# krzyz/topo-renderer

Hardware: AMD Instinct MI355X
Metric: panorama Mpix/s (higher is better)
Workload: dtype f32; 1 GPU; c4: 10x10 deg COP90-shaped mosaic (100 tiles of 1200x1200 f32), 16384x4096 panorama = 8 sectors of 2048x4096, view_mode 0; frames_in_flight=1

## Files before the change

topo-renderer_amd/__init__.py:

```python
from __future__ import annotations

import ctypes as C
import math
import os
import subprocess

import numpy as np

from . import panorama, synth

_HERE = os.path.dirname(os.path.abspath(__file__))
LIB_PATH = os.environ.get("TOPO_HIP_LIB") or os.path.join(_HERE, "libtopo_hip.so")
HEADER_PATH = os.path.join(os.path.dirname(_HERE), "include", "topo_hip.h")
TEST_HEADER_PATH = os.path.join(os.path.dirname(_HERE), "include", "topo_hip_test.h")

TOPO_OK = 0
TOPO_ERR_INVALID, TOPO_ERR_UNSUPPORTED, TOPO_ERR_HIP, TOPO_ERR_NOT_FOUND, TOPO_ERR_CAPACITY = -1, -2, -3, -4, -5
FORMAT_RGBA8_UNORM_SRGB, FORMAT_BGRA8_UNORM_SRGB, FORMAT_RGBA8_UNORM, FORMAT_BGRA8_UNORM = 1, 2, 3, 4
TIMING_SLOTS = 9
TIMING_NAMES = ("clear", "cull", "raster", "occlusion", "raster_big", "resolve", "total", "load", "load_tables")

NEAR, FAR = 50.0, 500000.0
N_SECTORS = 8
HORIZON_SKY, HORIZON_INCOMPLETE = -1, -2
HORIZON_DTYPE = np.dtype([("row", "<i4"), ("depth", "<f4"), ("lat_deg", "<i4"), ("lon_deg", "<i4"), ("cell_x", "<u4"), ("cell_y", "<u4"),
                          ("fan", "<u4"), ("_reserved", "<u4")])


class TopoError(RuntimeError):
    def __init__(self, code, msg):
        super().__init__(f"topo_hip error {code}: {msg}")
        self.code = code


def build(verbose: bool = False) -> str:
    subprocess.check_call(["make", "-C", os.path.join(_HERE, "csrc"), "all"] + ([] if verbose else ["-s"]))
    return LIB_PATH


_lib = None


def _preload_torch_hip_runtime():
    import importlib.util
    try:
        spec = importlib.util.find_spec("torch")
    except (ImportError, ValueError):
        spec = None
    if spec and spec.submodule_search_locations:
        cand = os.path.join(list(spec.submodule_search_locations)[0], "lib", "libamdhip64.so")
        if os.path.exists(cand):
            C.CDLL(cand, mode=C.RTLD_GLOBAL)


def lib():
    global _lib
    if _lib is None:
        if not os.path.exists(LIB_PATH):
            raise ImportError(f"{LIB_PATH} is missing -- run `python -c 'import __graft_entry__ as g; g.build()'` "
                              "(there is no Python/CPU fallback for the render path)")
        _preload_torch_hip_runtime()
        L = C.CDLL(LIB_PATH)
        vp, u32, i32, f32, sz = C.c_void_p, C.c_uint32, C.c_int32, C.c_float, C.c_size_t
        sigs = {
            "topo_create": (C.c_int, [C.POINTER(vp), C.c_int, u32, u32, u32]),
            "topo_destroy": (None, [vp]),
            "topo_last_error": (C.c_char_p, [vp]),
            "topo_add_terrain": (C.c_int, [vp, i32, i32, vp, u32, u32, vp, vp, vp]),
            "topo_add_terrain_device": (C.c_int, [vp, i32, i32, vp, u32, u32, vp, vp, vp]),
            "topo_unload_terrain": (C.c_int, [vp, i32, i32]),
            "topo_update": (C.c_int, [vp, u32, u32, vp, vp]),
            "topo_render": (C.c_int, [vp, vp, sz, vp, sz]),
            "topo_recompute_normals": (C.c_int, [vp]),
            "topo_render_views_device": (C.c_int, [vp, u32, vp, u32, u32, vp, sz, sz, vp, sz, sz]),
            "topo_set_stream": (C.c_int, [vp, vp]),
            "topo_synchronize": (C.c_int, [vp]),
            "topo_set_normals_lds_rows": (C.c_int, [vp, C.c_int]),
            "topo_debug_set_queue_caps": (C.c_int, [vp, u32, u32]),
            "topo_debug_far_phase_launched": (C.c_int, [vp, vp]),
            "topo_pin_host_buffer": (C.c_int, [vp, vp, sz]),
            "topo_unpin_host_buffer": (C.c_int, [vp, vp]),
            "topo_get_timings": (C.c_int, [vp, vp]),
            "topo_get_timing_history": (C.c_int, [vp, C.c_uint32, vp, vp]),
            "topo_get_counters": (C.c_int, [vp, vp]),
            "topo_set_occlusion_split": (C.c_int, [vp, f32]),
            "topo_set_timing_slots": (C.c_int, [vp, u32]),
            "topo_read_normals": (C.c_int, [vp, i32, i32, vp]),
            "topo_read_tile_tables": (C.c_int, [vp, i32, i32, vp, vp, vp, vp]),
            "topo_probe_sincos": (C.c_int, [vp, vp, vp, vp, sz]),
            "topo_probe_div": (C.c_int, [vp, i32, vp, vp, vp, sz]),
            "topo_set_pipeline_depth": (C.c_int, [vp, i32]),
            "topo_join": (C.c_int, [vp]),
            "topo_frame_status": (C.c_int, [vp, vp]),
            "topo_overlay_lines": (C.c_int, [vp, vp, u32, vp, u32, f32, vp, sz]),
            "topo_overlay_lines_device": (C.c_int, [vp, vp, u32, vp, u32, f32, vp, sz]),
            "topo_overlay_glyphs": (C.c_int, [vp, vp, u32, C.c_float, vp, u32, u32, vp, sz]),
            "topo_overlay_glyphs_device": (C.c_int, [vp, vp, u32, C.c_float, vp, u32, u32, vp, sz]),
            "topo_change_location_plan": (None, [f32, f32, f32, vp, u32, vp, u32, vp, vp, u32, vp]),
            "topo_change_location": (C.c_int, [vp, f32, f32, f32, vp, u32, vp, vp]),
            "topo_comm_unique_id": (C.c_int, [vp]),
            "topo_comm_init": (C.c_int, [C.POINTER(vp), C.c_int, vp, C.c_int, C.c_int]),
            "topo_comm_from_nccl": (C.c_int, [C.POINTER(vp), vp, C.c_int, C.c_int]),
            "topo_comm_destroy": (None, [vp]),
            "topo_panorama_sector_range": (None, [C.c_int, C.c_int, vp, vp]),
            "topo_panorama_slots": (u32, [C.c_int, u32, u32, vp, u32]),
            "topo_render_panorama": (C.c_int, [vp, vp, vp, f32, f32, u32, u32, f32, f32, i32, vp, vp]),
            "topo_render_batch": (C.c_int, [vp, u32, vp, vp, vp, f32, u32, u32, i32, vp, vp]),
            "topo_visible_peaks": (C.c_int, [vp, u32, vp, vp, vp]),
            "topo_visible_peaks_device": (C.c_int, [vp, vp, u32, u32, vp, sz, u32, vp, vp, vp]),
            "topo_camera_uniforms": (None, [vp, f32, f32, f32, f32, f32, f32, f32, i32, vp]),
            "topo_terrain_uniforms": (None, [vp, vp, vp, u32, u32, vp]),
            "topo_geometry_transform": (None, [f32, f32, f32, vp]),
            "topo_dist_from_depth": (f32, [f32]),
            "topo_pad_256": (u32, [u32]),
            "topo_synth_tile": (None, [i32, i32, u32, u32, u32, vp]),
            "topo_locations_range": (u32, [f32, f32, f32, vp, u32]),
            "topo_coordinate_transform": (C.c_int, [vp, u32, vp, u32, vp, vp, vp, vp]),
            "topo_geotiff_info": (C.c_int, [vp, sz, vp, vp, vp, vp, vp]),
            "topo_sector_fov_y": (f32, [u32, u32, u32]),
            "topo_panorama_uniforms": (None, [vp, f32, f32, u32, u32, f32, f32, i32, u32, vp]),
            "topo_render_device": (C.c_int, [vp, vp, sz, vp, sz]),
            "topo_geotiff_decode": (C.c_int, [vp, vp, sz, vp, sz]),
            "topo_add_terrain_geotiff": (C.c_int, [vp, i32, i32, vp, sz]),
            "topo_to_model": (None, [vp, vp, vp, f32, f32, vp]),
            "topo_to_raster": (None, [vp, vp, vp, f32, f32, vp]),
            "topo_height_value_at": (C.c_int, [vp, u32, u32, vp, vp, vp, C.c_double, C.c_double, vp]),
            "topo_viewshed_enable": (C.c_int, [vp, i32]),
            "topo_viewshed_reset": (C.c_int, [vp]),
            "topo_viewshed_read": (C.c_int, [vp, i32, i32, vp, sz, vp]),
            "topo_debug_viewshed_stats": (C.c_int, [vp, vp]),
            "topo_horizon_shape": (C.c_int, [vp, vp, vp, vp]),
            "topo_horizon_read": (C.c_int, [vp, u32, u32, vp, sz]),
            "topo_horizon_device": (C.c_int, [vp, u32, u32, vp, sz]),
            "topo_pixel_angles": (None, [vp, u32, u32, u32, vp, vp]),
        }
        for name, (res, args) in sigs.items():
            fn = getattr(L, name)
            fn.restype = res
            fn.argtypes = args
        L._topo_symbols = tuple(sigs)
        _lib = L
    return _lib


def _p(a):
    return a.ctypes.data_as(C.c_void_p)



def camera_uniforms(eye, yaw, pitch, fov_y, width, height, sun_theta_deg, sun_phi_deg, view_mode=0) -> np.ndarray:
    out = np.zeros(40, dtype=np.float32)
    e = np.ascontiguousarray(eye, dtype=np.float32)
    lib().topo_camera_uniforms(_p(e), yaw, pitch, fov_y, width, height, sun_theta_deg, sun_phi_deg, view_mode, _p(out))
    return out


def terrain_uniforms(raster_point, model_point, pixel_scale, w, h) -> np.ndarray:
    out = np.zeros(24, dtype=np.float32)
    rp, mp, ps = (np.ascontiguousarray(a, dtype=np.float32) for a in (raster_point, model_point, pixel_scale))
    lib().topo_terrain_uniforms(_p(rp), _p(mp), _p(ps), w, h, _p(out))
    return out


def geometry_transform(h, lon_deg, lat_deg) -> np.ndarray:
    out = np.zeros(3, dtype=np.float32)
    lib().topo_geometry_transform(h, lon_deg, lat_deg, _p(out))
    return out


def dist_from_depth(d: float) -> float:
    return float(lib().topo_dist_from_depth(d))


def pad_256(n: int) -> int:
    return int(lib().topo_pad_256(n))


def synth_tile(lat_deg, lon_deg, w=1200, h=1200, seed=synth.SEED_DEFAULT) -> np.ndarray:
    out = np.empty((h, w), dtype=np.float32)
    lib().topo_synth_tile(lat_deg, lon_deg, w, h, seed & 0xFFFFFFFF, _p(out))
    return out


def locations_range(latitude: float, longitude: float, range_dist: float = 100_000.0):
    buf = np.zeros((4096, 2), np.int32)
    n = int(lib().topo_locations_range(latitude, longitude, range_dist, _p(buf), 4096))
    return [(int(a), int(b)) for a, b in buf[:min(n, 4096)]]


def change_location_plan(latitude: float, longitude: float, loaded, range_dist: float = 100_000.0):
    ld = np.ascontiguousarray(np.array(list(loaded), dtype=np.int32).reshape(-1, 2))
    un, rq = np.zeros((4096, 2), np.int32), np.zeros((4096, 2), np.int32)
    nu, nr = C.c_uint32(), C.c_uint32()
    lib().topo_change_location_plan(latitude, longitude, range_dist, _p(ld) if len(ld) else None, len(ld), _p(un), 4096, C.byref(nu), _p(rq), 4096, C.byref(nr))
    return [(int(a), int(b)) for a, b in un[:nu.value]], [(int(a), int(b)) for a, b in rq[:nr.value]]


class CoordinateTransform:

    def __init__(self, raster_point, model_point, pixel_scale):
        self.raster_point = np.asarray(raster_point, np.float32)
        self.model_point = np.asarray(model_point, np.float32)
        self.pixel_scale = np.asarray(pixel_scale, np.float32)

    @classmethod
    def from_geo_tag_data(cls, pixel_scale_data, tie_points_data, model_transformation_data=None):
        arr = lambda v: None if v is None else np.ascontiguousarray(v, dtype=np.float64)
        ps, tp, mt = arr(pixel_scale_data), arr(tie_points_data), arr(model_transformation_data)
        rp, mp, sc = (np.zeros(2, np.float32) for _ in range(3))
        ptr = lambda a: None if a is None else _p(a)
        rc = lib().topo_coordinate_transform(ptr(ps), 0 if ps is None else ps.size, ptr(tp), 0 if tp is None else tp.size, ptr(mt),
                                             _p(rp), _p(mp), _p(sc))
        if rc != 0:
            raise TopoError(rc, "IncorrectGeoTags" if rc == -2 else "IncorrectGeoTagData")
        return cls(rp, mp, sc)

    def to_model(self, x, y):
        out = np.zeros(2, np.float32)
        lib().topo_to_model(_p(self.raster_point), _p(self.model_point), _p(self.pixel_scale), x, y, _p(out))
        return float(out[0]), float(out[1])

    def to_raster(self, lon, lat):
        out = np.zeros(2, np.float32)
        lib().topo_to_raster(_p(self.raster_point), _p(self.model_point), _p(self.pixel_scale), lon, lat, _p(out))
        return float(out[0]), float(out[1])

    def height_value_at(self, heights: np.ndarray, longitude: float, latitude: float):
        hts = np.ascontiguousarray(heights, dtype=np.float32)
        h, w = hts.shape
        out = np.zeros(1, np.float32)
        rc = lib().topo_height_value_at(_p(hts), w, h, _p(self.raster_point), _p(self.model_point), _p(self.pixel_scale),
                                        float(longitude), float(latitude), _p(out))
        return None if rc != 0 else float(out[0])


def geotiff_info(data: bytes):
    buf = np.frombuffer(data, np.uint8)
    w, h = C.c_uint32(), C.c_uint32()
    rp, mp, sc = (np.zeros(2, np.float32) for _ in range(3))
    rc = lib().topo_geotiff_info(_p(buf), buf.size, C.byref(w), C.byref(h), _p(rp), _p(mp), _p(sc))
    if rc != 0:
        raise TopoError(rc, "GeoTIFF container or geo tags not usable")
    return int(w.value), int(h.value), CoordinateTransform(rp, mp, sc)


def pixel_angles(view_uniforms, width: int, height: int, xy) -> np.ndarray:
    u = np.ascontiguousarray(view_uniforms).view(np.uint8)
    if u.nbytes != 160:
        raise ValueError("uniforms must be 160 bytes")
    pts = np.ascontiguousarray(xy, dtype=np.float32).reshape(-1, 2)
    out = np.zeros((len(pts), 2), np.float64)
    lib().topo_pixel_angles(_p(u), width, height, len(pts), _p(pts), _p(out))
    return out


def post_uniforms(width, height, pixelize_n=100.0) -> np.ndarray:
    return np.array([width, height, pixelize_n, 0.0], dtype=np.float32)


def sector_fov_y(sector_w: int, sector_h: int, n_sectors: int = N_SECTORS) -> float:
    return 2.0 * math.atan(math.tan(math.pi / n_sectors) * sector_h / sector_w)


def panorama_uniforms(eye, yaw0, sector_w, sector_h, sun_theta_deg, sun_phi_deg, view_mode=0,
                      n_sectors: int = N_SECTORS, pitch: float = 0.0):
    out = np.zeros((n_sectors, 40), dtype=np.float32)
    e = np.ascontiguousarray(eye, dtype=np.float32)
    lib().topo_panorama_uniforms(_p(e), yaw0, pitch, sector_w, sector_h, sun_theta_deg, sun_phi_deg, view_mode, n_sectors, _p(out))
    return [out[k].copy() for k in range(n_sectors)]



def comm_unique_id() -> np.ndarray:
    out = np.zeros(128, np.uint8)
    rc = lib().topo_comm_unique_id(_p(out))
    if rc != TOPO_OK:
        raise TopoError(rc, lib().topo_last_error(None).decode())
    return out


class Comm:

    def __init__(self, rank: int = 0, world: int = 1, unique_id=None, device: int = 0, nccl_comm: int = 0):
        h = C.c_void_p()
        if nccl_comm:
            rc = lib().topo_comm_from_nccl(C.byref(h), C.c_void_p(nccl_comm), rank, world)
        else:
            uid = None if unique_id is None else np.ascontiguousarray(unique_id, dtype=np.uint8)
            rc = lib().topo_comm_init(C.byref(h), device, None if uid is None else _p(uid), rank, world)
        if rc != TOPO_OK:
            raise TopoError(rc, lib().topo_last_error(None).decode())
        self._h, self.rank, self.world = h, rank, world

    def close(self):
        if getattr(self, "_h", None):
            lib().topo_comm_destroy(self._h)
            self._h = None

    def __del__(self):
        try:
            self.close()
        except Exception:
            pass


def panorama_slots(world: int, sector_w: int, sector_h: int):
    n = lib().topo_panorama_slots(world, sector_w, sector_h, None, 0)
    out = np.zeros((max(1, n), 3), np.uint32)
    lib().topo_panorama_slots(world, sector_w, sector_h, _p(out), n)
    return [tuple(int(v) for v in row) for row in out[:n]]


def panorama_sector_range(rank: int, world: int):
    a, b = C.c_uint32(), C.c_uint32()
    lib().topo_panorama_sector_range(rank, world, C.byref(a), C.byref(b))
    return range(a.value, a.value + b.value)



class TerrainRenderer:

    def __init__(self, width: int, height: int, device: int = 0, color_format: int = FORMAT_RGBA8_UNORM_SRGB):
        h = C.c_void_p()
        rc = lib().topo_create(C.byref(h), device, width, height, color_format)
        if rc != TOPO_OK:
            raise TopoError(rc, lib().topo_last_error(None).decode())
        self._h = h
        self.size = (width, height)
        self.tile_size = None

    def close(self):
        if getattr(self, "_h", None):
            lib().topo_destroy(self._h)
            self._h = None

    def __del__(self):
        try:
            self.close()
        except Exception:
            pass

    def _check(self, rc):
        if rc != TOPO_OK:
            raise TopoError(rc, lib().topo_last_error(self._h).decode())

    def add_terrain(self, lat_deg, lon_deg, heights, raster_point, model_point, pixel_scale):
        hts = np.ascontiguousarray(heights, dtype=np.float32)
        h, w = hts.shape
        rp, mp, ps = (np.ascontiguousarray(a, dtype=np.float32) for a in (raster_point, model_point, pixel_scale))
        self._check(lib().topo_add_terrain(self._h, lat_deg, lon_deg, _p(hts), w, h, _p(rp), _p(mp), _p(ps)))
        self.tile_size = (w, h)

    def add_terrain_device(self, lat_deg, lon_deg, heights_ptr: int, w, h, raster_point, model_point, pixel_scale):
        rp, mp, ps = (np.ascontiguousarray(a, dtype=np.float32) for a in (raster_point, model_point, pixel_scale))
        self._check(lib().topo_add_terrain_device(self._h, lat_deg, lon_deg, C.c_void_p(heights_ptr), w, h, _p(rp), _p(mp), _p(ps)))
        self.tile_size = (w, h)

    def unload_terrain(self, lat_deg, lon_deg):
        self._check(lib().topo_unload_terrain(self._h, lat_deg, lon_deg))

    def update(self, width, height, uniforms: np.ndarray, post: np.ndarray):
        u = np.ascontiguousarray(uniforms).view(np.uint8)
        pu = np.ascontiguousarray(post, dtype=np.float32)
        if u.nbytes != 160 or pu.nbytes != 16:
            raise ValueError("uniforms must be 160 bytes and post uniforms 16 bytes")
        self._check(lib().topo_update(self._h, width, height, _p(u), _p(pu)))
        self.size = (width, height)

    def render(self, want_depth=True, padded_depth=False):
        w, h = self.size
        rgba = np.empty((h, w, 4), np.uint8)
        if not want_depth:
            self._check(lib().topo_render(self._h, _p(rgba), w * 4, None, 0))
            return rgba, None
        pitch = pad_256(4 * w) if padded_depth else 4 * w
        depth = np.zeros((h, pitch // 4), np.float32)
        self._check(lib().topo_render(self._h, _p(rgba), w * 4, _p(depth), pitch))
        return rgba, (depth if padded_depth else depth[:, :w])

    def render_into(self, rgba: np.ndarray, depth: np.ndarray = None):
        self._check(lib().topo_render(self._h, _p(rgba), rgba.strides[0], _p(depth) if depth is not None else None,
                                      depth.strides[0] if depth is not None else 0))

    def pin_host_buffer(self, a: np.ndarray):
        self._check(lib().topo_pin_host_buffer(self._h, _p(a), a.nbytes))

    def unpin_host_buffer(self, a: np.ndarray):
        self._check(lib().topo_unpin_host_buffer(self._h, _p(a)))

    def decode_geotiff(self, data: bytes) -> np.ndarray:
        w, h, _ = geotiff_info(data)
        buf = np.frombuffer(data, np.uint8)
        out = np.empty((h, w), np.float32)
        self._check(lib().topo_geotiff_decode(self._h, _p(buf), buf.size, _p(out), out.size))
        return out

    def add_terrain_geotiff(self, lat_deg: int, lon_deg: int, data: bytes):
        buf = np.frombuffer(data, np.uint8)
        self._check(lib().topo_add_terrain_geotiff(self._h, lat_deg, lon_deg, _p(buf), buf.size))
        w, h, _ = geotiff_info(data)
        self.tile_size = (w, h)

    def render_device(self, rgba_ptr: int, rgba_pitch: int, depth_ptr: int = 0, depth_pitch: int = 0):
        self._check(lib().topo_render_device(self._h, C.c_void_p(rgba_ptr), rgba_pitch, C.c_void_p(depth_ptr) if depth_ptr else None, depth_pitch))

    def recompute_normals(self):
        self._check(lib().topo_recompute_normals(self._h))

    def overlay_lines(self, vertices, indices, rgba: np.ndarray, line_width: float = 0.5) -> np.ndarray:
        v = np.ascontiguousarray(vertices)
        ix = np.ascontiguousarray(indices, dtype=np.uint32)
        assert rgba.dtype == np.uint8 and rgba.flags.c_contiguous
        self._check(lib().topo_overlay_lines(self._h, _p(v), v.nbytes // 32, _p(ix), ix.size, line_width, _p(rgba), rgba.strides[0]))
        return rgba

    def overlay_lines_device(self, vertices, indices, rgba_ptr: int, rgba_pitch: int, line_width: float = 0.5):
        v = np.ascontiguousarray(vertices)
        ix = np.ascontiguousarray(indices, dtype=np.uint32)
        self._check(lib().topo_overlay_lines_device(self._h, _p(v), v.nbytes // 32, _p(ix), ix.size, line_width, C.c_void_p(rgba_ptr), rgba_pitch))

    def overlay_glyphs(self, glyphs, atlas: np.ndarray, rgba: np.ndarray, depth: float = 100.0 / 4096.0) -> np.ndarray:
        g = np.ascontiguousarray(glyphs)
        a = np.ascontiguousarray(atlas, dtype=np.uint8)
        assert rgba.dtype == np.uint8 and rgba.flags.c_contiguous
        self._check(lib().topo_overlay_glyphs(self._h, _p(g), g.nbytes // 28, depth, _p(a), a.shape[1], a.shape[0], _p(rgba), rgba.strides[0]))
        return rgba

    def overlay_glyphs_device(self, glyphs, atlas: np.ndarray, rgba_ptr: int, rgba_pitch: int, depth: float = 100.0 / 4096.0):
        g = np.ascontiguousarray(glyphs)
        a = np.ascontiguousarray(atlas, dtype=np.uint8)
        self._check(lib().topo_overlay_glyphs_device(self._h, _p(g), g.nbytes // 28, depth, _p(a), a.shape[1], a.shape[0], C.c_void_p(rgba_ptr), rgba_pitch))

    def change_location(self, latitude: float, longitude: float, range_dist: float = 100_000.0):
        rq = np.zeros((4096, 2), np.int32)
        nr, nu = C.c_uint32(), C.c_uint32()
        self._check(lib().topo_change_location(self._h, latitude, longitude, range_dist, _p(rq), 4096, C.byref(nr), C.byref(nu)))
        return [(int(a), int(b)) for a, b in rq[:nr.value]], int(nu.value)

    def render_panorama(self, comm, eye, yaw0, sector_w, sector_h, sun_theta_deg, sun_phi_deg, strip_ptr: int, depth_ptr: int = 0,
                        view_mode: int = 0, pitch: float = 0.0):
        e = np.ascontiguousarray(eye, dtype=np.float32)
        self._check(lib().topo_render_panorama(self._h, comm._h if comm is not None else None, _p(e), yaw0, pitch, sector_w, sector_h,
                                               sun_theta_deg, sun_phi_deg, view_mode, C.c_void_p(strip_ptr),
                                               C.c_void_p(depth_ptr) if depth_ptr else None))

    def render_batch(self, eyes, yaw0s, suns_theta_phi_deg, sector_w, sector_h, rgba_ptr: int, depth_ptr: int = 0, view_mode: int = 0,
                     pitch: float = 0.0):
        e = np.ascontiguousarray(eyes, dtype=np.float32).reshape(-1, 3)
        y = np.ascontiguousarray(yaw0s, dtype=np.float32).reshape(-1)
        sn = np.ascontiguousarray(suns_theta_phi_deg, dtype=np.float32).reshape(-1, 2)
        assert len(e) == len(y) == len(sn)
        self._check(lib().topo_render_batch(self._h, len(e), _p(e), _p(y), _p(sn), pitch, sector_w, sector_h, view_mode,
                                            C.c_void_p(rgba_ptr), C.c_void_p(depth_ptr) if depth_ptr else None))

    def render_views_device(self, uniforms_list, width, height, rgba_ptr: int, rgba_view_stride: int, rgba_pitch: int,
                            depth_ptr: int = 0, depth_view_stride: int = 0, depth_pitch: int = 0):
        if isinstance(uniforms_list, np.ndarray) and uniforms_list.dtype == np.uint8 and uniforms_list.ndim == 2:
            us = np.ascontiguousarray(uniforms_list)
            assert us.shape[1] == 160
        else:
            us = np.ascontiguousarray(np.stack([np.ascontiguousarray(u).view(np.uint8).reshape(160) for u in uniforms_list]))
        self._check(lib().topo_render_views_device(self._h, len(us), _p(us), width, height,
                                                   C.c_void_p(rgba_ptr), rgba_view_stride, rgba_pitch,
                                                   C.c_void_p(depth_ptr) if depth_ptr else None, depth_view_stride, depth_pitch))

    def set_stream(self, hip_stream: int):
        self._check(lib().topo_set_stream(self._h, C.c_void_p(hip_stream) if hip_stream else None))

    def set_pipeline_depth(self, depth: int):
        self._check(lib().topo_set_pipeline_depth(self._h, depth))

    def join(self):
        self._check(lib().topo_join(self._h))

    def synchronize(self):
        self._check(lib().topo_synchronize(self._h))

    def frame_status(self) -> dict:
        out = np.zeros(4, np.uint32)
        self._check(lib().topo_frame_status(self._h, _p(out)))
        return {"status": int(out[0]), "big_overflow": bool(out[0] & 1), "rare_overflow": bool(out[0] & 2), "bounds_violation": bool(out[0] & 4),
                "bounds_site": int(out[1]), "bounds_value": int(out[2]) | (int(out[3]) << 32)}

    def set_normals_lds_rows(self, rows: int):
        self._check(lib().topo_set_normals_lds_rows(self._h, rows))

    def debug_set_queue_caps(self, big_cap: int, rare_cap: int):
        self._check(lib().topo_debug_set_queue_caps(self._h, big_cap, rare_cap))

    def debug_far_phase_launched(self) -> bool:
        out = np.zeros(1, np.int32)
        self._check(lib().topo_debug_far_phase_launched(self._h, _p(out)))
        return bool(out[0])

    def timings(self) -> dict:
        out = np.zeros(TIMING_SLOTS, np.float32)
        self._check(lib().topo_get_timings(self._h, _p(out)))
        return {k: float(v) for k, v in zip(TIMING_NAMES, out) if k != "_"}

    def timing_history(self, n_frames: int) -> list:
        out, n = np.zeros((max(1, n_frames), 7), np.float32), C.c_uint32(0)
        self._check(lib().topo_get_timing_history(self._h, n_frames, _p(out), C.byref(n)))
        return [{k: float(v) for k, v in zip(TIMING_NAMES[:7], row)} for row in out[:n.value]]

    def counters(self) -> dict:
        out = np.zeros(6, np.uint32)
        self._check(lib().topo_get_counters(self._h, _p(out)))
        return {"blocks_rastered": int(out[0]) + int(out[5]), "big_items": int(out[1]), "status": int(out[2]), "rare_items": int(out[3]),
                "near_blocks": int(out[0]), "far_tested": int(out[4]), "far_survived": int(out[5])}

    def set_timing_slots(self, names=None, total=True):
        mask = 0x3F if names is None else sum(1 << TIMING_NAMES.index(n) for n in names)
        if not total:
            mask |= 0x80
        self._check(lib().topo_set_timing_slots(self._h, mask))

    def set_occlusion_split(self, metres: float):
        self._check(lib().topo_set_occlusion_split(self._h, metres))

    def read_tile_tables(self, lat_deg, lon_deg) -> dict:
        w, h = self.tile_size
        n = C.c_uint32(0)
        self._check(lib().topo_read_tile_tables(self._h, lat_deg, lon_deg, None, None, None, C.byref(n)))
        minmax, trig, bounds = np.empty((n.value, 2), np.float32), np.empty((w + h, 2), np.float32), np.empty(n.value * 17, np.float64)
        self._check(lib().topo_read_tile_tables(self._h, lat_deg, lon_deg, _p(minmax), _p(trig), _p(bounds), C.byref(n)))
        return {"minmax": minmax, "trig": trig, "bounds": bounds}

    def read_normals(self, lat_deg, lon_deg) -> np.ndarray:
        w, h = self.tile_size
        out = np.empty((h, w, 4), np.uint8)
        self._check(lib().topo_read_normals(self._h, lat_deg, lon_deg, _p(out)))
        return out

    def visible_peaks(self, peaks_xyz: np.ndarray):
        pk = np.ascontiguousarray(peaks_xyz, dtype=np.float32).reshape(-1, 3)
        n = pk.shape[0]
        vis = np.zeros(n, np.uint8)
        xy = np.zeros((n, 2), np.uint32)
        self._check(lib().topo_visible_peaks(self._h, n, _p(pk), _p(vis), _p(xy)))
        return vis.astype(bool), xy

    def visible_peaks_device(self, uniforms, width, height, depth_ptr, depth_pitch, n, peaks_ptr, visible_ptr, xy_ptr):
        u = np.ascontiguousarray(uniforms).view(np.uint8)
        self._check(lib().topo_visible_peaks_device(self._h, _p(u), width, height, C.c_void_p(depth_ptr), depth_pitch, n,
                                                    C.c_void_p(peaks_ptr), C.c_void_p(visible_ptr), C.c_void_p(xy_ptr)))

    def viewshed_enable(self, on: bool = True):
        self._check(lib().topo_viewshed_enable(self._h, 1 if on else 0))

    def viewshed_reset(self):
        self._check(lib().topo_viewshed_reset(self._h))

    def viewshed(self, lat_deg, lon_deg) -> np.ndarray:
        if self.tile_size is None:
            raise TopoError(TOPO_ERR_NOT_FOUND, "no tile loaded")
        w, h = self.tile_size
        out = np.zeros((h - 1, w - 1), np.uint8)
        n = C.c_uint64(0)
        self._check(lib().topo_viewshed_read(self._h, lat_deg, lon_deg, _p(out), w - 1, C.byref(n)))
        if int(out.sum()) != n.value:
            raise TopoError(TOPO_ERR_INVALID, f"viewshed count {n.value} differs from the mask's {int(out.sum())} cells")
        return out.astype(bool)

    def debug_viewshed_stats(self) -> dict:
        out = np.zeros(3, np.uint64)
        self._check(lib().topo_debug_viewshed_stats(self._h, _p(out)))
        return {"terrain_keys": int(out[0]), "updates": int(out[1]), "atomics": int(out[2])}

    def horizon_shape(self):
        n, w, h = C.c_uint32(), C.c_uint32(), C.c_uint32()
        self._check(lib().topo_horizon_shape(self._h, C.byref(n), C.byref(w), C.byref(h)))
        return int(n.value), int(w.value), int(h.value)

    def horizon(self, first_view: int = 0, n_views: int = None) -> np.ndarray:
        total, w, _ = self.horizon_shape()
        n = total - first_view if n_views is None else n_views
        out = np.zeros((max(n, 0), w), HORIZON_DTYPE)
        self._check(lib().topo_horizon_read(self._h, first_view, n, _p(out) if out.size else None, w))
        return out

    def horizon_device(self, out_ptr: int, first_view: int = 0, n_views: int = None, view_stride: int = None):
        total, w, _ = self.horizon_shape()
        n = total - first_view if n_views is None else n_views
        self._check(lib().topo_horizon_device(self._h, first_view, n, C.c_void_p(out_ptr), w if view_stride is None else view_stride))

    def probe_div(self, kind: int, x: np.ndarray, y: np.ndarray) -> np.ndarray:
        x = np.ascontiguousarray(x, dtype=np.float32)
        y = np.ascontiguousarray(y, dtype=np.float32)
        out = np.empty_like(x)
        self._check(lib().topo_probe_div(self._h, kind, _p(x), _p(y), _p(out), x.size))
        return out

    def probe_sincos(self, x: np.ndarray):
        x = np.ascontiguousarray(x, dtype=np.float32)
        s, c = np.empty_like(x), np.empty_like(x)
        self._check(lib().topo_probe_sincos(self._h, _p(x), _p(s), _p(c), x.size))
        return s, c
```

topo-renderer_amd/csrc/host_math.cpp:

```cpp
#include "host_math.hpp"

#include <algorithm>
#include <cmath>
#include <cstdlib>
#include <cstring>

#include "topo_math.h"

namespace topo {

namespace {

inline float rs_to_radians(float d) { return d * 0.017453292519943295f; }

struct V3 { float x, y, z; };
inline float vdot(V3 a, V3 b) { return (a.x * b.x + a.y * b.y) + a.z * b.z; }
inline V3 vcross(V3 a, V3 b) { return {a.y * b.z - a.z * b.y, a.z * b.x - a.x * b.z, a.x * b.y - a.y * b.x}; }
inline V3 vnormalize(V3 v) {
    const float r = 1.0f / sqrtf(vdot(v, v));
    return {v.x * r, v.y * r, v.z * r};
}

void euler_xyz_ex_a0(float b, float c, float m[9] ) {
    const float si = sinf(0.0f), ci = cosf(0.0f);
    const float sj = sinf(b), cj = cosf(b), sh = sinf(c), ch = cosf(c);
    const float cc = ci * ch, cs = ci * sh, sc = si * ch, ss = si * sh;
    m[0] = cj * ch;       m[1] = cj * sh;       m[2] = -sj;
    m[3] = sj * sc - cs;  m[4] = sj * ss + cc;  m[5] = cj * si;
    m[6] = sj * cc + ss;  m[7] = sj * cs - sc;  m[8] = cj * ci;
}

}

void terrain_rotation(float model_lon_deg, float model_lat_deg, float rot[9]) {
    euler_xyz_ex_a0(rs_to_radians(90.0f - model_lat_deg), rs_to_radians(model_lon_deg), rot);
}

void geometry_transform(float h, float lon_deg, float lat_deg, float out[3]) {
    const float r = kR0 + h;
    const float lon = rs_to_radians(lon_deg), lat = rs_to_radians(lat_deg);
    out[0] = r * cosf(lat) * cosf(lon);
    out[1] = r * cosf(lat) * sinf(lon);
    out[2] = r * sinf(lat);
}

void pixel_angles(const topo_uniforms* view, uint32_t w, uint32_t h, uint32_t n, const float* xy, double* az_el) {
    const float* f = view->camera_proj;
    double m[4][4], inv[4][8];
    for (int r = 0; r < 4; ++r)
        for (int c = 0; c < 4; ++c) m[r][c] = f[4 * c + r];
    for (int r = 0; r < 4; ++r)
        for (int c = 0; c < 8; ++c) inv[r][c] = c < 4 ? m[r][c] : (c - 4 == r ? 1.0 : 0.0);
    for (int c = 0; c < 4; ++c) {
        int piv = c;
        for (int r = c + 1; r < 4; ++r)
            if (std::fabs(inv[r][c]) > std::fabs(inv[piv][c])) piv = r;
        for (int k = 0; k < 8; ++k) std::swap(inv[c][k], inv[piv][k]);
        const double d = inv[c][c];
        for (int k = 0; k < 8; ++k) inv[c][k] /= d;
        for (int r = 0; r < 4; ++r)
            if (r != c) {
                const double s = inv[r][c];
                for (int k = 0; k < 8; ++k) inv[r][k] -= s * inv[c][k];
            }
    }
    auto unproject = [&](double nx, double ny, double nz, double out[3]) {
        double p[4];
        for (int r = 0; r < 4; ++r) p[r] = inv[r][4] * nx + inv[r][5] * ny + inv[r][6] * nz + inv[r][7];
        for (int k = 0; k < 3; ++k) out[k] = p[k] / p[3];
    };
    const double ex = view->camera_pos[0], ey = view->camera_pos[1], ez = view->camera_pos[2];
    const double el = std::sqrt(ex * ex + ey * ey + ez * ez);
    const double up[3] = {ex / el, ey / el, ez / el};
    const double eh = std::hypot(up[0], up[1]);
    const double east[3] = {eh > 0.0 ? -up[1] / eh : 0.0, eh > 0.0 ? up[0] / eh : 1.0, 0.0};
    const double north[3] = {up[1] * east[2] - up[2] * east[1], up[2] * east[0] - up[0] * east[2], up[0] * east[1] - up[1] * east[0]};
    const double kDeg = 180.0 / 3.14159265358979323846;
    for (uint32_t i = 0; i < n; ++i) {
        const double nx = 2.0 * xy[2 * i] / w - 1.0, ny = 1.0 - 2.0 * xy[2 * i + 1] / h;
        double p0[3], p1[3];
        unproject(nx, ny, 0.0, p0);
        unproject(nx, ny, 1.0, p1);
        const double d[3] = {p1[0] - p0[0], p1[1] - p0[1], p1[2] - p0[2]};
        const double de = d[0] * east[0] + d[1] * east[1] + d[2] * east[2];
        const double dn = d[0] * north[0] + d[1] * north[1] + d[2] * north[2];
        const double du = d[0] * up[0] + d[1] * up[1] + d[2] * up[2];
        double az = std::atan2(de, dn) * kDeg;
        if (az < 0.0) az += 360.0;
        az_el[2 * i] = az;
        az_el[2 * i + 1] = std::atan2(du, std::hypot(de, dn)) * kDeg;
    }
}

void camera_uniforms(const float eye_in[3], float yaw, float pitch, float fov_y, float width, float height,
                     float sun_theta_deg, float sun_phi_deg, int32_t view_mode, topo_uniforms* out) {
    memset(out, 0, sizeof *out);
    const V3 eye = {eye_in[0], eye_in[1], eye_in[2]};
    const V3 up = vnormalize(eye);
    const V3 from = {0.0f, -1.0f, 0.0f};
    float qx, qy, qz, qw;
    const float d = vdot(from, up);
    const float one_minus_eps = 1.0f - 2.0f * 1.1920929e-7f;
    if (d > one_minus_eps) {
        qx = qy = qz = 0.0f; qw = 1.0f;
    } else if (d < -one_minus_eps) {
        const float sign = copysignf(1.0f, from.z);
        const float a = -1.0f / (sign + from.z);
        const float b = from.x * from.y * a;
        const V3 axis = {b, sign + from.y * from.y * a, -from.y};
        const float s = sinf(3.14159265358979323846f * 0.5f), c = cosf(3.14159265358979323846f * 0.5f);
        qx = axis.x * s; qy = axis.y * s; qz = axis.z * s; qw = c;
    } else {
        const V3 c = vcross(from, up);
        const float w = 1.0f + d;
        const float l2 = (c.x * c.x + c.z * c.z) + (c.y * c.y + w * w);
        const float r = 1.0f / sqrtf(l2);
        qx = c.x * r; qy = c.y * r; qz = c.z * r; qw = w * r;
    }
    const V3 v = {cosf(yaw) * cosf(pitch), sinf(pitch), sinf(yaw) * cosf(pitch)};
    const V3 b = {qx, qy, qz};
    const float b2 = vdot(b, b);
    const float k0 = qw * qw - b2, k1 = vdot(v, b) * 2.0f, k2 = qw * 2.0f;
    const V3 bxv = vcross(b, v);
    const V3 f = {(v.x * k0 + b.x * k1) + bxv.x * k2, (v.y * k0 + b.y * k1) + bxv.y * k2, (v.z * k0 + b.z * k1) + bxv.z * k2};
    const V3 s = vnormalize(vcross(f, up));
    const V3 u = vcross(s, f);
    const float view[16] = {s.x, u.x, -f.x, 0.0f, s.y, u.y, -f.y, 0.0f, s.z, u.z, -f.z, 0.0f,
                            -vdot(eye, s), -vdot(eye, u), vdot(eye, f), 1.0f};
    const float aspect = width / height;
    const float sf = sinf(0.5f * fov_y), cf = cosf(0.5f * fov_y);
    const float hh = cf / sf, ww = hh / aspect, r = kFar / (kNear - kFar);
    const float proj[16] = {ww, 0, 0, 0, 0, hh, 0, 0, 0, 0, r, -1.0f, 0, 0, r * kNear, 0};
    for (int c = 0; c < 4; ++c)
        for (int rr = 0; rr < 4; ++rr) {
            float t = proj[rr] * view[c * 4 + 0];
            t = t + proj[4 + rr] * view[c * 4 + 1];
            t = t + proj[8 + rr] * view[c * 4 + 2];
            t = t + proj[12 + rr] * view[c * 4 + 3];
            out->camera_proj[c * 4 + rr] = t;
        }
    for (int c = 0; c < 3; ++c)
        for (int rr = 0; rr < 3; ++rr) out->normal_proj[c * 4 + rr] = view[c * 4 + rr];
    out->normal_proj[15] = 1.0f;
    out->camera_pos[0] = eye.x; out->camera_pos[1] = eye.y; out->camera_pos[2] = eye.z; out->camera_pos[3] = 0.0f;
    float m3[9];
    euler_xyz_ex_a0(rs_to_radians(90.0f - sun_phi_deg), rs_to_radians(sun_theta_deg), m3);
    out->sun_direction[0] = m3[6]; out->sun_direction[1] = m3[7]; out->sun_direction[2] = m3[8];
    out->view_mode = view_mode;
}

void panorama_uniforms(const float eye[3], float yaw0, float pitch, uint32_t sector_w, uint32_t sector_h, float sun_theta_deg, float sun_phi_deg,
                       int32_t view_mode, uint32_t n_sectors, topo_uniforms* out) {
    const double kPi = 3.14159265358979323846;
    const double fov = 2.0 * atan(tan(kPi / (double)n_sectors) * (double)sector_h / (double)sector_w);
    for (uint32_t k = 0; k < n_sectors; ++k)
        camera_uniforms(eye, (float)((double)yaw0 - (double)k * (2.0 * kPi / (double)n_sectors)), pitch, (float)fov, (float)sector_w,
                        (float)sector_h, sun_theta_deg, sun_phi_deg, view_mode, out + k);
}

uint32_t locations_range(float latitude, float longitude, float range_dist, int32_t* out, uint32_t cap) {
    int c_lat = (int)floorf(latitude);
    c_lat = c_lat < -90 ? c_lat : -90;
    c_lat = c_lat > 89 ? c_lat : 89;
    const int c_lon = ((int)(floorf(longitude) + 540.0f)) % 360 - 180;
    const float lat_cos = cosf(rs_to_radians(latitude));
    const float arc_factor = 0.5f * range_dist / kR0;
    const float arc_factor_sin = sinf(arc_factor);
    const float afs_sq = arc_factor_sin * arc_factor_sin;
    const float R2D = 57.29577951308232f;
    const float dlon = acosf(1.0f - afs_sq / lat_cos / lat_cos) * R2D;
    const float dlat = acosf(1.0f - afs_sq) * R2D;
    int lat_start = (int)floorf(latitude - dlat);
    lat_start = lat_start > -90 ? lat_start : -90;
    int lat_end = (int)floorf(latitude + dlat);
    lat_end = lat_end < 89 ? lat_end : 89;
    const int lon_start = (int)floorf(longitude - dlon), lon_end = (int)floorf(longitude + dlon);
    struct Item { int lat, lon, k0, k1; };
    std::vector<Item> v;
    for (int la = lat_start; la <= lat_end; ++la)
        for (int lo = lon_start; lo <= lon_end; ++lo) v.push_back({la, lo, std::abs(la - c_lat), std::abs(lo - c_lon)});
    std::stable_sort(v.begin(), v.end(), [](const Item& a, const Item& b) { return a.k0 != b.k0 ? a.k0 < b.k0 : a.k1 < b.k1; });
    uint32_t n = 0;
    for (const Item& it : v) {
        if (n < cap && out) { out[2 * n] = it.lat; out[2 * n + 1] = (it.lon + 540) % 360 - 180; }
        ++n;
    }
    return n;
}

void change_location_plan(float latitude, float longitude, float range_dist, const int32_t* loaded, uint32_t n_loaded,
                          std::vector<std::pair<int32_t, int32_t>>& unload, std::vector<std::pair<int32_t, int32_t>>& request) {
    const uint32_t n = locations_range(latitude, longitude, range_dist, nullptr, 0);
    std::vector<int32_t> want(2 * (size_t)n);
    locations_range(latitude, longitude, range_dist, want.data(), n);
    std::vector<bool> have(n, false);
    unload.clear();
    request.clear();
    for (uint32_t i = 0; i < n_loaded; ++i) {
        bool in_new = false;
        for (uint32_t k = 0; k < n; ++k)
            if (want[2 * k] == loaded[2 * i] && want[2 * k + 1] == loaded[2 * i + 1]) { in_new = true; have[k] = true; }
        if (!in_new) unload.emplace_back(loaded[2 * i], loaded[2 * i + 1]);
    }
    for (uint32_t k = 0; k < n; ++k) {
        bool dup = false;
        for (uint32_t j = 0; j < k && !dup; ++j) dup = want[2 * j] == want[2 * k] && want[2 * j + 1] == want[2 * k + 1];
        if (!have[k] && !dup) request.emplace_back(want[2 * k], want[2 * k + 1]);
    }
}

namespace {
inline float synth_hash(int64_t ix, int64_t iy, uint32_t seed) {
    uint32_t h = ((uint32_t)ix * 0x9E3779B1u) ^ ((uint32_t)iy * 0x85EBCA77u) ^ (seed * 0xC2B2AE3Du);
    h ^= h >> 15; h *= 0x2C1B3C6Du; h ^= h >> 12; h *= 0x297A2D39u; h ^= h >> 15;
    return (float)(h >> 8) * (1.0f / 16777216.0f);
}
}

void synth_tile(int32_t lat, int32_t lon, uint32_t w, uint32_t h, uint32_t seed, float* out) {
    static const int wl[5] = {512, 256, 128, 64, 32};
    static const float amp[5] = {1.0f, 0.5f, 0.25f, 0.125f, 0.0625f};
    const float norm = (float)(3000.0 / 1.9375);
    for (uint32_t y = 0; y < h; ++y) {
        const int64_t gy = (int64_t)(89 - lat) * h + y;
        for (uint32_t x = 0; x < w; ++x) {
            const int64_t gx = ((int64_t)lon + 180) * w + x;
            float acc = 0.0f;
            for (int o = 0; o < 5; ++o) {
                const int64_t cx = gx / wl[o], cy = gy / wl[o];
                const float fx = (float)(gx % wl[o]) / (float)wl[o], fy = (float)(gy % wl[o]) / (float)wl[o];
                const float ux = fx * fx * (3.0f - 2.0f * fx), uy = fy * fy * (3.0f - 2.0f * fy);
                const uint32_t s = seed + (uint32_t)o;
                const float v00 = synth_hash(cx, cy, s), v10 = synth_hash(cx + 1, cy, s);
                const float v01 = synth_hash(cx, cy + 1, s), v11 = synth_hash(cx + 1, cy + 1, s);
                const float a = v00 + ux * (v10 - v00), b = v01 + ux * (v11 - v01);
                const float v = a + uy * (b - a);
                acc = acc + amp[o] * v;
            }
            out[(size_t)y * w + x] = acc * norm;
        }
    }
}

}
```

topo-renderer_amd/csrc/host_math.hpp:

```cpp
#pragma once

#include <cstdint>
#include <utility>
#include <vector>

#include "../../include/topo_hip.h"

namespace topo {

void camera_uniforms(const float eye[3], float yaw, float pitch, float fov_y, float width, float height,
                     float sun_theta_deg, float sun_phi_deg, int32_t view_mode, topo_uniforms* out);
void panorama_uniforms(const float eye[3], float yaw0, float pitch, uint32_t sector_w, uint32_t sector_h, float sun_theta_deg, float sun_phi_deg,
                       int32_t view_mode, uint32_t n_sectors, topo_uniforms* out);
void geometry_transform(float h, float lon_deg, float lat_deg, float out[3]);
void pixel_angles(const topo_uniforms* view, uint32_t w, uint32_t h, uint32_t n, const float* xy, double* az_el);
void terrain_rotation(float model_lon_deg, float model_lat_deg, float rot3x3_colmajor[9]);
uint32_t locations_range(float latitude, float longitude, float range_dist, int32_t* out_lat_lon, uint32_t cap);
void change_location_plan(float latitude, float longitude, float range_dist, const int32_t* loaded, uint32_t n_loaded,
                          std::vector<std::pair<int32_t, int32_t>>& unload, std::vector<std::pair<int32_t, int32_t>>& request);
void synth_tile(int32_t lat, int32_t lon, uint32_t w, uint32_t h, uint32_t seed, float* out);

}
```

topo-renderer_amd/csrc/kernels_frame.h:

```cpp
#pragma once

#include "kernels_common.h"

namespace topo {
namespace {

__device__ __forceinline__ void clear_body(uint64_t* __restrict__ vis, uint8_t* __restrict__ dirty, size_t n, uint32_t* __restrict__ counters,
                                           uint32_t* __restrict__ zero, uint32_t block, uint32_t n_blocks) {
    if (block == 0)
        for (uint32_t i = threadIdx.x; i < kCounterWords; i += 256) zero[i] = 0;
    const uint32_t lane = threadIdx.x & 63;
    const size_t nseg = (n + 63) >> 6, wave = (size_t)block * 4 + (threadIdx.x >> 6), nwave = (size_t)n_blocks * 4;
    for (size_t g = wave * 64; g < nseg; g += nwave * 64) {
        const bool mine = g + lane < nseg && dirty[g + lane] != 0;
        uint64_t todo = __ballot(mine);
        if (mine) dirty[g + lane] = 0;
        while (todo) {
            const size_t seg = g + (size_t)__builtin_ctzll(todo);
            todo &= todo - 1;
            if (TOPO_CHK(counters, seg * 64 + lane < ((n + 63) & ~(size_t)63), 3u, seg * 64 + lane))
                vis[seg * 64 + lane] = kVisClear;
        }
    }
}
__global__ __launch_bounds__(256) void k_clear(uint64_t* __restrict__ vis, uint8_t* __restrict__ dirty, size_t n, uint32_t* __restrict__ counters,
                                               uint32_t* __restrict__ zero) {
    clear_body(vis, dirty, n, counters, zero, blockIdx.x, gridDim.x);
}


__device__ __forceinline__ void clip_plane(const float* m, int pl, double out[5]) {
    double a, b, cc, d;
    const int row = pl >> 1;
    const double sgn = (pl & 1) ? -1.0 : 1.0;
    if (pl == 4) {
        a = m[2]; b = m[6]; cc = m[10]; d = m[14];
    } else {
        a = (double)m[3] + sgn * (double)m[row];
        b = (double)m[7] + sgn * (double)m[4 + row];
        cc = (double)m[11] + sgn * (double)m[8 + row];
        d = (double)m[15] + sgn * (double)m[12 + row];
    }
    out[0] = a; out[1] = b; out[2] = cc; out[3] = d;
    out[4] = sqrt(a * a + b * b + cc * cc);
}

__device__ __forceinline__ void emit_near(const FrameParams& P, uint32_t view, uint32_t rank, uint32_t blk) {
    if (P.split_m > 0.0f) {
        const uint32_t by = blk / P.bx_count;
        const uint32_t cell_rows = min(kBCY, P.tile_h - 1 - by * kBCY);
        const uint32_t strip = P.near_strip, n = (cell_rows + strip - 1) / strip;
        const uint32_t base = atomicAdd(&P.counters[kCtrWork], n);
        for (uint32_t k = 0; k < n; ++k)
            if (base + k < P.near_cap && TOPO_CHK(P.counters, blk < (1u << 24) && strip * k < 16u, 4u, blk))
                P.work[base + k] = WorkItem{(view << 16) | rank, blk | ((strip * k) << 24) | (min(strip, cell_rows - strip * k) << 28)};
        return;
    }
    const uint32_t slot = atomicAdd(&P.counters[kCtrWork], 1u);
    if (slot < P.near_cap) P.work[slot] = WorkItem{(view << 16) | rank, blk};
}

__device__ __forceinline__ void cull_body(const FrameParams& P, uint32_t block) {
    const uint32_t blocks_per_tile = P.bx_count * P.by_count;
    const size_t total = (size_t)P.n_views * P.n_tiles * blocks_per_tile;
    const size_t gid0 = (size_t)block * blockDim.x, gid = gid0 + threadIdx.x;
    __shared__ double s_plane[2][6][5];
    __shared__ uint32_t s_far[256], s_nfar;
    const uint32_t view0 = (uint32_t)(gid0 / ((size_t)blocks_per_tile * P.n_tiles));
    if (threadIdx.x < 12 && view0 + threadIdx.x / 6 < P.n_views) clip_plane(P.views[view0 + threadIdx.x / 6].proj, threadIdx.x % 6, s_plane[threadIdx.x / 6][threadIdx.x % 6]);
    if (threadIdx.x == 0) s_nfar = 0;
    __syncthreads();
    if (gid < total) {
        const uint32_t blk = (uint32_t)(gid % blocks_per_tile);
        const uint32_t rank = (uint32_t)((gid / blocks_per_tile) % P.n_tiles);
        const uint32_t view = (uint32_t)(gid / ((size_t)blocks_per_tile * P.n_tiles));
        const TileDev& t = P.tiles[rank];
        const double hmin = (double)t.block_minmax[2 * blk], hmax = (double)t.block_minmax[2 * blk + 1];
        const double* bs = t.block_bounds + (size_t)blk * 4;
        const double c[3] = {bs[0], bs[1], bs[2]}, radius = bs[3];
        const float* m = P.views[view].proj;
        bool keep = true;
        for (int pl = 0; pl < 6 && keep; ++pl) {
            double own[5];
            const double* q = s_plane[view - view0 < 2 ? view - view0 : 0][pl];
            if (view - view0 >= 2) {
                clip_plane(m, pl, own);
                q = own;
            }
            const double dist = q[0] * c[0] + q[1] * c[1] + q[2] * c[2] + q[3];
            if (dist < -radius * q[4]) keep = false;
        }
        const bool sane = hmin <= hmax;
        if (!sane) keep = true;
        if (keep) {
            const double wn = sqrt((double)m[3] * m[3] + (double)m[7] * m[7] + (double)m[11] * m[11]);
            const double w_near = ((double)m[3] * c[0] + (double)m[7] * c[1] + (double)m[11] * c[2] + (double)m[15]) - radius * wn;
            const double sagitta = t.block_bounds[(size_t)blocks_per_tile * 16 + blk];
            if (sane && P.split_m > 0.0f && w_near > (double)P.split_m && sagitta <= 1.0) {
                const uint32_t fslot = atomicAdd(&s_nfar, 1u);
                if (TOPO_CHK(P.counters, fslot < 256u, 5u, fslot)) s_far[fslot] = threadIdx.x;
            }
            else emit_near(P, view, rank, blk);
        }
    }
    __syncthreads();
    for (uint32_t i = threadIdx.x; i < s_nfar; i += blockDim.x) {
        const size_t g = gid0 + s_far[i];
        const uint32_t blk = (uint32_t)(g % blocks_per_tile);
        const uint32_t rank = (uint32_t)((g / blocks_per_tile) % P.n_tiles);
        const uint32_t view = (uint32_t)(g / ((size_t)blocks_per_tile * P.n_tiles));
        const TileDev& t = P.tiles[rank];
        const double hmin = (double)t.block_minmax[2 * blk], hmax = (double)t.block_minmax[2 * blk + 1];
        const double* bb = t.block_bounds + (size_t)blocks_per_tile * 4 + (size_t)blk * 12;
        const float* m = P.views[view].proj;
        double bxlo = 1e30, bxhi = -1e30, bylo = 1e30, byhi = -1e30, wmin = 1e30, zclip_at_wmin = 0.0;
        const double hs[2] = {hmin - 1.0, hmax + 2.0 + t.block_bounds[(size_t)blocks_per_tile * 16 + blk]};
#pragma unroll 1
        for (int k = 0; k < 8; ++k) {
            const double R = (double)kR0 + (k < 4 ? hs[0] : hs[1]);
            const double px = R * bb[3 * (k & 3)], py = R * bb[3 * (k & 3) + 1], pz = R * bb[3 * (k & 3) + 2];
            const double cx = (double)m[0] * px + (double)m[4] * py + (double)m[8] * pz + (double)m[12];
            const double cy = (double)m[1] * px + (double)m[5] * py + (double)m[9] * pz + (double)m[13];
            const double cz = (double)m[2] * px + (double)m[6] * py + (double)m[10] * pz + (double)m[14];
            const double cw = (double)m[3] * px + (double)m[7] * py + (double)m[11] * pz + (double)m[15];
            const double icw = 1.0 / cw;
            const double sx = (cx * icw * 0.5 + 0.5) * (double)P.W, sy = (0.5 - cy * icw * 0.5) * (double)P.H;
            bxlo = sx < bxlo ? sx : bxlo; bxhi = sx > bxhi ? sx : bxhi;
            bylo = sy < bylo ? sy : bylo; byhi = sy > byhi ? sy : byhi;
            if (cw < wmin) { wmin = cw; zclip_at_wmin = cz; }
        }
        const double zmin = (zclip_at_wmin - 8.0) / wmin;
        if (!(wmin > 1000.0 && zmin > 0.0 && zmin < 1.0)) {
            emit_near(P, view, rank, blk);
            continue;
        }
        const int32_t ix0 = max((int32_t)floor(bxlo) - 2, 0), ix1 = min((int32_t)ceil(bxhi) + 2, P.W - 1);
        const int32_t iy0 = max((int32_t)floor(bylo) - 2, 0), iy1 = min((int32_t)ceil(byhi) + 2, P.H - 1);
        if (ix0 > ix1 || iy0 > iy1) continue;
        float zf = (float)zmin;
        if ((double)zf > zmin) zf = bits_f(f_bits(zf) - 1u);
        const uint32_t q = block % kFarLists, slot = atomicAdd(&P.counters[far_list_counter(q)], 1u);
        if (TOPO_CHK(P.counters, slot < P.far_sub_cap, 5u, slot)) {
            FarItem fi;
            fi.view_rank = (view << 16) | rank; fi.block = blk;
            fi.x0 = (uint16_t)ix0; fi.x1 = (uint16_t)ix1; fi.y0 = (uint16_t)iy0; fi.y1 = (uint16_t)iy1;
            fi.zmin_bits = f_bits(zf);
            P.far[(size_t)q * P.far_sub_cap + slot] = fi;
        }
    }
}

__global__ __launch_bounds__(256) void k_cull(FrameParams P) { cull_body(P, blockIdx.x); }
struct ClearCullArgs {
    FrameParams P;
    uint32_t n_cull_blocks, n_clear_blocks;
    uint32_t* zero;
    ViewPack pack;
    uint32_t pack_words;
};
__global__ __launch_bounds__(256) void k_clear_cull(FrameParams P, uint32_t n_cull_blocks, uint32_t n_clear_blocks, uint32_t* __restrict__ zero, ViewPack pack,
                                                    uint32_t pack_words) {
    if (pack_words) {
        const auto src = kernarg<uint32_t>(offsetof(ClearCullArgs, pack));
        if (blockIdx.x == 0 && threadIdx.x < pack_words) const_cast<uint32_t*>(reinterpret_cast<const uint32_t*>(P.views))[threadIdx.x] = src[threadIdx.x];
        P.views = (const ViewDev*)(const void*)src;
    }
    const uint32_t total = n_cull_blocks + n_clear_blocks;
    const uint32_t before = (uint32_t)((uint64_t)blockIdx.x * n_clear_blocks / total), upto = (uint32_t)((uint64_t)(blockIdx.x + 1u) * n_clear_blocks / total);
    if (upto > before) clear_body(P.vis, P.dirty, (size_t)P.n_views * P.W * P.H, P.counters, zero, before, n_clear_blocks);
    else cull_body(P, blockIdx.x - before);
}

#ifndef TOPO_OCC_ROWS
#define TOPO_OCC_ROWS 4
#endif
constexpr uint32_t kOccRows = TOPO_OCC_ROWS;
__global__ __launch_bounds__(256) void k_occlusion(FrameParams P) {
    if (blockIdx.x == 0 && threadIdx.x == 0) {
        P.counters[kCtrBigStart] = P.counters[kCtrBig];
        P.counters[kCtrRareStart] = P.counters[kCtrRare];
    }
    const uint32_t lane = threadIdx.x & 63;
    const uint32_t wave_global = blockIdx.x * 4 + __builtin_amdgcn_readfirstlane(threadIdx.x >> 6), wave_count = gridDim.x * 4;
    static_assert(kFarLists == 64, "one sub-list per lane");
    uint32_t incl = min(P.counters[far_list_counter(lane)], P.far_sub_cap);
#pragma unroll
    for (int o = 1; o < 64; o <<= 1) {
        const uint32_t up = (uint32_t)__shfl_up((int)incl, o);
        if ((int)lane >= o) incl += up;
    }
    const uint32_t count = (uint32_t)__shfl((int)incl, 63);
    if (blockIdx.x == 0 && threadIdx.x == 0) P.counters[kCtrFarTested] = count;
    auto entry = [&](uint32_t g) -> const FarItem& {
        const uint32_t q = (uint32_t)__popcll(__ballot(incl <= g));
        const uint32_t start = q ? (uint32_t)__shfl((int)incl, (int)q - 1) : 0u;
        return P.far[(size_t)q * P.far_sub_cap + (g - start)];
    };
    if (count == 0) return;
    FarItem fi_next = entry(wave_global < count ? wave_global : 0u);
    for (uint32_t item = wave_global; item < count; item += wave_count) {
        const FarItem fi = fi_next;
        fi_next = entry(item + wave_count < count ? item + wave_count : item);
        const uint64_t* vis = P.vis + (size_t)(fi.view_rank >> 16) * P.W * P.H;
        bool visible = false;
        for (uint32_t x = fi.x0; x <= fi.x1 && !visible; x += 64) {
            const uint32_t px = min(x + lane, (uint32_t)fi.x1);
            for (uint32_t y = fi.y0; y <= fi.y1; y += kOccRows) {
                uint32_t d[kOccRows];
#pragma unroll
                for (uint32_t k = 0; k < kOccRows; ++k) {
                    const size_t at = (size_t)min(y + k, (uint32_t)fi.y1) * P.W + px;
                    d[k] = TOPO_CHK(P.counters, at < (size_t)P.W * P.H && (fi.view_rank >> 16) < P.n_views, 6u, at) ? (uint32_t)(vis[at] >> 32) : 0u;
                }
                bool open = false;
#pragma unroll
                for (uint32_t k = 0; k < kOccRows; ++k) open |= d[k] >= fi.zmin_bits;
                if (__any(open)) { visible = true; break; }
            }
        }
        if (visible && lane == 0) {
            const uint32_t blk = fi.block, by = blk / P.bx_count;
            const uint32_t cell_rows = min(kBCY, P.tile_h - 1 - by * kBCY);
            const uint32_t strip = P.near_strip, n = (cell_rows + strip - 1) / strip;
            const uint32_t base = atomicAdd(&P.counters[kCtrFarSurvived], n);
            for (uint32_t k = 0; k < n; ++k)
                if (base + k < P.near_cap)
                    P.work2[base + k] = WorkItem{fi.view_rank, blk | ((strip * k) << 24) | (min(strip, cell_rows - strip * k) << 28)};
        }
    }
}



__device__ __forceinline__ void raster_box(const TriSetup& ts, const Vis& vis, int32_t W, uint32_t id,
                                           int32_t px0, int32_t px1, int32_t py0, int32_t py1) {
    for (int32_t py = py0; py <= py1; ++py)
        for (int32_t px = px0; px <= px1; ++px) {
            float z, b[3];
            if (triangle_pixel(ts, px, py, z, b)) vis_min(vis, (size_t)py * W + px, vis_key(z, id));
        }
}

__device__ bool enqueue_big(const FrameParams& P, uint32_t view, uint32_t id, const SVert& s0, const SVert& s1, const SVert& s2,
                            int32_t px0, int32_t px1, int32_t py0, int32_t py1) {
    const int32_t rx0 = px0 >> 6, rx1 = px1 >> 6, ry0 = py0 >> 6, ry1 = py1 >> 6;
    const uint32_t n = (uint32_t)((rx1 - rx0 + 1) * (ry1 - ry0 + 1));
    const uint32_t base = atomicAdd(&P.counters[kCtrBig], n);
    BigItem it;
    it.view = view;
    it.id = id;
    it.X[0] = s0.X; it.X[1] = s1.X; it.X[2] = s2.X;
    it.Y[0] = s0.Y; it.Y[1] = s1.Y; it.Y[2] = s2.Y;
    it.z[0] = s0.z; it.z[1] = s1.z; it.z[2] = s2.z;
    if (base >= P.big_cap || n > P.big_cap - base) {
        atomicOr(&P.counters[kCtrStatus], kStatusBigOverflow);
        it.id = kNoTri;
        it.region = 0;
        for (uint32_t k = base; k < P.big_cap && k - base < n; ++k) P.big[k] = it;
        return false;
    }
    uint32_t k = base;
    for (int32_t ry = ry0; ry <= ry1; ++ry)
        for (int32_t rx = rx0; rx <= rx1; ++rx) {
            it.region = ((uint32_t)ry << 16) | (uint32_t)rx;
            if (TOPO_CHK(P.counters, k < P.big_cap && rx >= 0 && ry >= 0 && rx * 64 < P.W && ry * 64 < P.H, 7u, k)) P.big[k] = it;
            ++k;
        }
    return true;
}

__device__ __forceinline__ void enqueue_rare(const FrameParams& P, uint32_t view, uint32_t draw) {
    const uint32_t slot = atomicAdd(&P.counters[kCtrRare], 1u);
    if (slot < P.rare_cap) P.rare[slot] = RareItem{view, draw};
    else atomicOr(&P.counters[kCtrStatus], kStatusRareOverflow);
}

#ifndef TOPO_FRAG_CAP
#define TOPO_FRAG_CAP 128
#endif
constexpr uint32_t kFragCap = TOPO_FRAG_CAP;
struct FragList {
    uint32_t count;
    uint32_t pix[kFragCap];
    uint64_t key[kFragCap];
};

#ifndef TOPO_INLANE_ROWS
#define TOPO_INLANE_ROWS 5
#endif
#ifndef TOPO_INLANE_COLS
#define TOPO_INLANE_COLS 24
#endif
constexpr int32_t kInlaneRows = TOPO_INLANE_ROWS, kInlaneCols = TOPO_INLANE_COLS;

__device__ __forceinline__ void frag_push(FragList& fl, const Vis& vis, uint32_t pix, uint64_t key) {
    const uint32_t slot = atomicAdd(&fl.count, 1u);
    if (slot < kFragCap) {
        fl.pix[slot] = pix;
        fl.key[slot] = key;
    } else {
        vis_min(vis, pix, key);
    }
}

constexpr uint32_t kTriCap = 128;
struct TriList {
    int32_t X0[kTriCap], Y0[kTriCap], X1[kTriCap], Y1[kTriCap], X2[kTriCap], Y2[kTriCap];
    float z0[kTriCap], z1[kTriCap], z2[kTriCap];
    uint32_t id[kTriCap];
};

__device__ __forceinline__ bool classify_small(const FrameParams& P, const SVert& s0, const SVert& s1, const SVert& s2, uint32_t view,
                                               uint32_t id) {
    const int32_t X0 = s0.X, Y0 = s0.Y, X1 = s1.X, Y1 = s1.Y, X2 = s2.X, Y2 = s2.Y;
    const int32_t mnx = min(X0, min(X1, X2)), mxx = max(X0, max(X1, X2));
    const int32_t mny = min(Y0, min(Y1, Y2)), mxy = max(Y0, max(Y1, Y2));
    if ((mxx - mnx) >= (1 << 14) || (mxy - mny) >= (1 << 14)) {
        enqueue_rare(P, view, id >> 1);
        return false;
    }
    const int32_t area2 = __mul24(X1 - X0, Y2 - Y0) - __mul24(Y1 - Y0, X2 - X0);
    if (area2 >= 0) return false;
    const int32_t px0 = max((mnx + 127) >> 8, 0), px1 = min((mxx - 128) >> 8, P.W - 1);
    const int32_t py0 = max((mny + 127) >> 8, 0), py1 = min((mxy - 128) >> 8, P.H - 1);
    if (px0 > px1 || py0 > py1) return false;
    if (py1 - py0 >= kInlaneRows || px1 - px0 >= kInlaneCols) {
        if (!enqueue_big(P, view, id, s0, s1, s2, px0, px1, py0, py1)) enqueue_rare(P, view, id >> 1);
        return false;
    }
    return true;
}


__device__ __forceinline__ uint32_t tri_push(TriList& tl, uint32_t n, bool push, const SVert& s0, const SVert& s1, const SVert& s2,
                                             uint32_t id, uint32_t* vis_counters) {
    const uint64_t mask = __ballot(push);
    if (push) {
        const uint32_t slot = n + __popcll(mask & ((1ull << (threadIdx.x & 63)) - 1ull));
        if (!TOPO_CHK(vis_counters, slot < kTriCap, 8u, slot)) return n;
        tl.X0[slot] = s0.X; tl.Y0[slot] = s0.Y; tl.X1[slot] = s1.X; tl.Y1[slot] = s1.Y; tl.X2[slot] = s2.X; tl.Y2[slot] = s2.Y;
        tl.z0[slot] = s0.z; tl.z1[slot] = s1.z; tl.z2[slot] = s2.z;
        tl.id[slot] = id;
    }
    return n + (uint32_t)__popcll(mask);
}

__device__ __forceinline__ uint32_t tri_drain(TriList& tl, FragList& fl, const Vis& vis, int32_t W, int32_t H, uint32_t n,
                                              bool flush) {
    const uint32_t lane = threadIdx.x & 63;
    const uint32_t take = min(n, 64u), base = n - take;
    if (lane < take) {
        const uint32_t e = base + lane;
        raster_rows(W, H, tl.X0[e], tl.Y0[e], tl.X1[e], tl.Y1[e], tl.X2[e], tl.Y2[e], tl.z0[e], tl.z1[e], tl.z2[e], tl.id[e],
                    [&](uint32_t pix, uint64_t key) { frag_push(fl, vis, pix, key); });
    }
    const uint32_t nfrag = min(fl.count, kFragCap);
    if (nfrag >= 64 || (flush && nfrag > 0)) {
        for (uint32_t f = lane; f < nfrag; f += 64) vis_min(vis, fl.pix[f], fl.key[f]);
        if (lane == 0) fl.count = 0;
    }
    return base;
}

__device__ __forceinline__ SVert shfl_down1(const SVert& v) {
    SVert o;
    o.X = __shfl_down(v.X, 1);
    o.Y = __shfl_down(v.Y, 1);
    o.z = __shfl_down(v.z, 1);
    o.flag = __shfl_down(v.flag, 1);
    return o;
}

#ifndef TOPO_RASTER_WAVES
#define TOPO_RASTER_WAVES 5
#endif
__global__ __launch_bounds__(256, TOPO_RASTER_WAVES) void k_raster(FrameParams P, int phase) {
    __shared__ FragList s_fl[4];
    __shared__ TriList s_tl[4];
    const WorkItem* __restrict__ work = phase == 0 ? P.work : P.work2;
    uint32_t count = P.counters[phase == 0 ? kCtrWork : kCtrFarSurvived];
    const uint32_t cap = P.near_cap;
    if (count > cap) count = cap;
    const uint32_t lane = threadIdx.x & 63, wave = __builtin_amdgcn_readfirstlane(threadIdx.x >> 6);
    FragList& fl = s_fl[wave];
    TriList& tl = s_tl[wave];
    uint32_t ntri = 0;
    const uint32_t wave_global = blockIdx.x * 4 + wave, wave_count = gridDim.x * 4;
    for (uint32_t item = wave_global; item < count; item += wave_count) {
        const auto wi_c = const_space(work + item);
        const WorkItem wi = {wi_c->view_rank, wi_c->block};
        const uint32_t view_idx = wi.view_rank >> 16, rank = wi.view_rank & 0xFFFFu;
        TileDev t;
        {
            const auto tc = const_space(P.tiles + rank);
            t.heights = tc->heights;
            t.raster_x = tc->raster_x; t.raster_y = tc->raster_y;
            t.model_x = tc->model_x; t.model_y = tc->model_y;
            t.scale_x = tc->scale_x; t.scale_y = tc->scale_y;
        }
        const auto view_proj = const_space(P.views[view_idx].proj);
        const uint32_t blk_id = wi.block & 0xFFFFFFu, strip_first = (wi.block >> 24) & 15u, strip_rows = wi.block >> 28;
        const uint32_t bx = blk_id % P.bx_count, by = blk_id / P.bx_count;
        const uint32_t x0 = bx * kBCX, y0 = by * kBCY + strip_first;
        const uint32_t nrows = min(strip_rows ? strip_rows + 1 : kVY, P.tile_h - y0);
        const uint32_t ncx = min(kBCX, P.tile_w - 1 - x0);
        const uint32_t vx = x0 + lane;
        const bool vcol = lane < kVX && vx < P.tile_w;
        const Vis vis = view_vis(P, view_idx);
        float proj[16];
#pragma unroll
        for (int q = 0; q < 16; ++q) proj[q] = view_proj[q];
        if (lane == 0) fl.count = 0;
        float slo, clo, lat_s = 0.0f, lat_c = 0.0f;
        sincos_f(vertex_lon(t, vcol ? vx : x0), slo, clo);
        if (lane < nrows) sincos_f(vertex_lat(t, y0 + lane), lat_s, lat_c);
        const auto hcol = TOPO_GLOBAL_F32(t.heights) + (size_t)y0 * P.tile_w + (vcol ? vx : x0);
        (void)TOPO_CHK(P.counters, rank < P.n_tiles && view_idx < P.n_views && y0 + nrows <= P.tile_h && (vcol ? vx : x0) < P.tile_w && nrows >= 1u, 9u,
                       ((uint64_t)y0 << 32) | x0);
        float h0 = hcol[0];
        float h1 = nrows > 1 ? hcol[(size_t)1 * P.tile_w] : 0.0f;
        float h2 = nrows > 2 ? hcol[(size_t)2 * P.tile_w] : 0.0f;
        float h3 = nrows > 3 ? hcol[(size_t)3 * P.tile_w] : 0.0f;
        SVert prev;
        prev.X = 0; prev.Y = 0; prev.z = 0.0f; prev.flag = kVtxNear;
        for (uint32_t r = 0; r < nrows; ++r) {
            const float h = h0;
            h0 = h1; h1 = h2; h2 = h3;
            if (r + 4 < nrows) h3 = hcol[(size_t)(r + 4) * P.tile_w];
            const float sla = __shfl(lat_s, (int)r), cla = __shfl(lat_c, (int)r);
            SVert cur;
            cur.X = 0; cur.Y = 0; cur.z = 0.0f; cur.flag = kVtxNear;
            if (vcol) {
                const f3 p = world_from_sincos(h, sla, cla, slo, clo);
                float clip[4];
                mat4_point(proj, p.x, p.y, p.z, clip);
                clip_to_screen(clip, (float)P.W, (float)P.H, cur);
            }
            if (r > 0) {
                const SVert cc = shfl_down1(prev), d = shfl_down1(cur);
                bool live = lane < ncx;
                if (live && (prev.flag | cur.flag | cc.flag | d.flag) == kVtxOk) {
                    const int32_t qx0 = min(min(prev.X, cur.X), min(cc.X, d.X)), qx1 = max(max(prev.X, cur.X), max(cc.X, d.X));
                    const int32_t qy0 = min(min(prev.Y, cur.Y), min(cc.Y, d.Y)), qy1 = max(max(prev.Y, cur.Y), max(cc.Y, d.Y));
                    const int32_t bx0 = max((qx0 + 127) >> 8, 0), bx1 = min((qx1 - 128) >> 8, P.W - 1);
                    const int32_t by0 = max((qy0 + 127) >> 8, 0), by1 = min((qy1 - 128) >> 8, P.H - 1);
                    live = bx0 <= bx1 && by0 <= by1;
                }
                const SVert &a = prev, &b = cur;
                const uint32_t i = x0 + lane, j = y0 + r - 1;
                const bool even = ((i + j) & 1u) == 0;
                const uint32_t tri0 = (i * (P.tile_h - 1) + j) * 2;
#pragma unroll
                for (uint32_t k = 0; k < 2; ++k) {
                    const SVert& s0 = k == 0 ? a : d;
                    const SVert& s1 = k == 0 ? b : cc;
                    const SVert& s2 = k == 0 ? (even ? d : cc) : (even ? a : b);
                    const uint32_t draw = rank * P.tris_per_tile + tri0 + k;
                    bool push = false;
                    if (live) {
                        const int fg = s0.flag | s1.flag | s2.flag;
                        if (fg == kVtxOk) {
                            push = classify_small(P, s0, s1, s2, view_idx, draw << 1);
                        } else if (fg & kVtxNear) {
                            const int nnear = (s0.flag == kVtxNear) + (s1.flag == kVtxNear) + (s2.flag == kVtxNear);
                            if (nnear != 3) enqueue_rare(P, view_idx, draw);
                        }
                    }
                    ntri = tri_push(tl, ntri, push, s0, s1, s2, draw << 1, P.counters);
                    if (ntri >= 64) ntri = tri_drain(tl, fl, vis, P.W, P.H, ntri, false);
                }
            }
            prev = cur;
        }
// ... 130 lines not shown
```

topo-renderer_amd/csrc/terrain_renderer.cpp:

```cpp
#include "terrain_renderer.hpp"

#include "geotiff.hpp"

#include <algorithm>
#include <atomic>
#include <thread>
#include <cmath>
#include <cstdio>
#include <cstring>

namespace topo {

namespace {

struct Switches {
    static int env(const char* name, int unset) { return getenv(name) ? atoi(getenv(name)) : unset; }
    const bool views_by_copy = env("TOPO_VIEWS_BY_COPY", 0) != 0;
    const bool views_in_cull = env("TOPO_VIEWS_IN_CULL", 1) != 0;
    const bool status_by_copy = env("TOPO_STATUS_BY_COPY", 0) != 0;
    const bool far_skip = env("TOPO_FAR_SKIP", 1) != 0;
    const bool events_by_marker = env("TOPO_EVENTS_BY_MARKER", 0) != 0;
    const bool fuse_clear_cull = env("TOPO_FUSE_CLEAR_CULL", 1) != 0;
    const int near_strip = env("TOPO_NEAR_STRIP", 0);
};
const Switches& switches() { static const Switches s; return s; }

bool is_linear(uint32_t format) { return format == TOPO_FORMAT_RGBA8_UNORM || format == TOPO_FORMAT_BGRA8_UNORM; }
bool is_bgra(uint32_t format) { return format == TOPO_FORMAT_BGRA8_UNORM_SRGB || format == TOPO_FORMAT_BGRA8_UNORM; }

constexpr int kTimingSlots = 6;
constexpr uint32_t kStagesOfSlot[kTimingSlots] = {1u << kStClear, 1u << kStCull, (1u << kStRasterNear) | (1u << kStRasterFar), 1u << kStOcclusion,
                                                  (1u << kStRareBigNear) | (1u << kStRareBigFar), 1u << kStResolve};
constexpr uint32_t stage_events(int stage) { return 3u << stage; }
constexpr uint32_t kLastEvent = 1u << kNumStages, kTotalEvents = 1u | kLastEvent;

}

int TerrainRenderer::fail(int code, const std::string& msg) {
    err_ = msg;
    return code;
}

int TerrainRenderer::hip_fail(hipError_t e, const char* what) {
    err_ = std::string(what) + ": " + hipGetErrorString(e);
    return TOPO_ERR_HIP;
}

int TerrainRenderer::bind_device() {
    TOPO_HIP_TRY(hipSetDevice(device_));
    return TOPO_OK;
}

int TerrainRenderer::create(TerrainRenderer** out, int device, uint32_t w, uint32_t h, uint32_t format, std::string* err) {
    *out = nullptr;
    if (w == 0 || h == 0) { *err = "target size must be non-zero"; return TOPO_ERR_INVALID; }
    if (format < TOPO_FORMAT_RGBA8_UNORM_SRGB || format > TOPO_FORMAT_BGRA8_UNORM) {
        *err = "colour format must be Rgba8UnormSrgb, Bgra8UnormSrgb, Rgba8Unorm or Bgra8Unorm";
        return TOPO_ERR_UNSUPPORTED;
    }
    int count = 0;
    hipError_t e = hipGetDeviceCount(&count);
    if (e != hipSuccess || count == 0) {
        *err = std::string("no HIP device: ") + (e != hipSuccess ? hipGetErrorString(e) : "device count is 0") +
               " (this library has no CPU fallback)";
        return TOPO_ERR_HIP;
    }
    if (device < 0 || device >= count) { *err = "hip_device out of range"; return TOPO_ERR_INVALID; }
    TerrainRenderer* r = new TerrainRenderer();
    r->device_ = device;
    r->W_ = w;
    r->H_ = h;
    r->format_ = format;
    if (r->init() != TOPO_OK) {
        *err = "HIP initialisation failed: " + r->err_;
        delete r;
        return TOPO_ERR_HIP;
    }
    *out = r;
    return TOPO_OK;
}

int TerrainRenderer::init() {
    TOPO_HIP_TRY(hipSetDevice(device_));
    TOPO_HIP_TRY(hipStreamCreate(&own_stream_.h));
    stream_ = own_stream_;
    for (auto& e : load_ev_) TOPO_HIP_TRY(hipEventCreate(&e.h));
    return init_ctx(ctx_[0], false);
}

TerrainRenderer::~TerrainRenderer() {
    (void)hipSetDevice(device_);
    if (stream_) (void)hipStreamSynchronize(stream_);
    for (auto& c : ctx_)
        if (c.stream) (void)hipStreamSynchronize(c.stream);
}

int TerrainRenderer::ensure(hipStream_t s, DeviceBuffer& b, size_t need) {
    if (need <= b.cap) return TOPO_OK;
    if (b.p) {
        TOPO_HIP_TRY(hipStreamSynchronize(s));
        TOPO_HIP_TRY(hipFree(b.p));
        b.p = nullptr;
        b.cap = 0;
    }
    TOPO_HIP_TRY(hipMalloc(&b.p, need));
    b.cap = need;
    return TOPO_OK;
}

int TerrainRenderer::ensure_pinned(PinnedBuffer& b, size_t need) {
    if (need <= b.cap) return TOPO_OK;
    b.reset();
    TOPO_HIP_TRY(hipHostMalloc(&b.p, need));
    b.cap = need;
    return TOPO_OK;
}

int TerrainRenderer::wait_all() {
    if (int rc = join()) return rc;
    TOPO_HIP_TRY(hipStreamSynchronize(stream_));
    return TOPO_OK;
}

Tile* TerrainRenderer::find(int lat, int lon) {
    auto it = tiles_.find(geo_key(lat, lon));
    return it == tiles_.end() ? nullptr : &it->second;
}

void TerrainRenderer::collect_jobs(const Tile& nt, const std::map<GeoKey, uint32_t>& rank, std::vector<EdgeJob>& edges,
                                   std::vector<CornerJob>& corners) {
    const int lat = nt.lat, lon = nt.lon;
    const uint32_t NONE = 0xFFFFFFFFu;
    auto loaded = [&](int la, int lo) -> uint32_t {
        Tile* t = find(la, lo);
        return (t && t != &nt && t->seq < nt.seq) ? rank.at(geo_key(la, lo)) : NONE;
    };
    const uint32_t me = rank.at(geo_key(lat, lon));
    const uint32_t left = loaded(lat, lon - 1), right = loaded(lat, lon + 1);
    const uint32_t top = loaded(lat + 1, lon), bottom = loaded(lat - 1, lon);
    const uint32_t top_left = loaded(lat + 1, lon - 1), top_right = loaded(lat + 1, lon + 1);
    const uint32_t bottom_left = loaded(lat - 1, lon - 1), bottom_right = loaded(lat - 1, lon + 1);
    if (left != NONE) edges.push_back(EdgeJob{left, me, me, 0});
    if (right != NONE) edges.push_back(EdgeJob{me, right, me, 0});
    if (top != NONE) edges.push_back(EdgeJob{top, me, me, 1});
    if (bottom != NONE) edges.push_back(EdgeJob{me, bottom, me, 1});
    if (top_left != NONE && top != NONE && left != NONE) corners.push_back(CornerJob{top_left, top, left, me, me});
    if (top != NONE && top_right != NONE && right != NONE) corners.push_back(CornerJob{top, top_right, me, right, me});
    if (left != NONE && bottom_left != NONE && bottom != NONE) corners.push_back(CornerJob{left, me, bottom_left, bottom, me});
    if (right != NONE && bottom != NONE && bottom_right != NONE) corners.push_back(CornerJob{me, right, bottom, bottom_right, me});
}

int TerrainRenderer::upload_seam_jobs(const std::vector<EdgeJob>& edges, const std::vector<CornerJob>& corners) {
    if (!edges.empty()) {
        if (int rc = ensure(stream_, d_edge_jobs_, edges.size() * sizeof(EdgeJob))) return rc;
        TOPO_HIP_TRY(hipMemcpyAsync(d_edge_jobs_.p, edges.data(), edges.size() * sizeof(EdgeJob), hipMemcpyHostToDevice, stream_));
    }
    if (!corners.empty()) {
        if (int rc = ensure(stream_, d_corner_jobs_, corners.size() * sizeof(CornerJob))) return rc;
        TOPO_HIP_TRY(hipMemcpyAsync(d_corner_jobs_.p, corners.data(), corners.size() * sizeof(CornerJob), hipMemcpyHostToDevice, stream_));
    }
    return TOPO_OK;
}
void TerrainRenderer::launch_seam_jobs(size_t n_edges, size_t n_corners) {
    launch_normals_border(d_tiles_.as<const TileDev>(), d_edge_jobs_.as<const EdgeJob>(), (uint32_t)n_edges, d_corner_jobs_.as<const CornerJob>(), (uint32_t)n_corners,
                          tile_w_, tile_h_, stream_);
}
int TerrainRenderer::run_seam_jobs(const std::vector<EdgeJob>& edges, const std::vector<CornerJob>& corners) {
    if (int rc = upload_seam_jobs(edges, corners)) return rc;
    launch_seam_jobs(edges.size(), corners.size());
    return TOPO_OK;
}

std::map<GeoKey, uint32_t> TerrainRenderer::ranks() const {
    std::map<GeoKey, uint32_t> r;
    uint32_t i = 0;
    for (const auto& kv : tiles_) r[kv.first] = i++;
    return r;
}

int TerrainRenderer::add_terrain(int32_t lat, int32_t lon, const float* heights, bool on_device, uint32_t w, uint32_t h,
                                 const float rp[2], const float mp[2], const float ps[2]) {
    if (!heights || !rp || !mp || !ps) return fail(TOPO_ERR_INVALID, "null argument");
    if (w < 3 || h < 3) return fail(TOPO_ERR_INVALID, "tile must be at least 3x3");
    if (w > 32768 || h > 32768) return fail(TOPO_ERR_INVALID, "tile too large");
    if (!tiles_.empty() && (w != tile_w_ || h != tile_h_))
        return fail(TOPO_ERR_INVALID, "mixed tile sizes are rejected (the reference caches one mesh: render_buffer.rs:12-15)");
    if (int rc = join()) return rc;
    const uint64_t tris = 2ull * (w - 1) * (h - 1);
    const size_t n_after = tiles_.size() + (find(lat, lon) ? 0 : 1);
    if (tris * n_after >= (1ull << 31) || n_after > 0xFFFFu) return fail(TOPO_ERR_CAPACITY, "draw-order id space exhausted");
    tile_w_ = w;
    tile_h_ = h;
    const size_t texels = (size_t)w * h;
    const uint32_t bxc = (w - 1 + kBCX - 1) / kBCX, byc = (h - 1 + kBCY - 1) / kBCY;
    Tile t;
    t.lat = lat;
    t.lon = lon;
    t.seq = next_seq_++;
    const size_t tile_floats = (size_t)bxc * byc * 2 + 2 * ((size_t)w + h);
    auto up256 = [](size_t n) { return (n + 255) & ~(size_t)255; };
    const size_t off_normals = up256(texels * 4), off_tables = off_normals + up256(texels * 4), off_bounds = off_tables + up256(tile_floats * sizeof(float));
    if (int rc = ensure(stream_, t.pool, off_bounds + (size_t)bxc * byc * 17 * sizeof(double))) return rc;
    t.d_heights = t.pool.as<float>();
    t.d_normals = reinterpret_cast<uint32_t*>(t.pool.as<uint8_t>() + off_normals);
    t.d_minmax = reinterpret_cast<float*>(t.pool.as<uint8_t>() + off_tables);
    if (const hipError_t e = hipMemcpyAsync(t.d_heights, heights, texels * 4, on_device ? hipMemcpyDeviceToDevice : hipMemcpyHostToDevice, stream_))
        return hip_fail(e, "tile upload");
    if (vs_ever_)
        if (int rc = alloc_mask(t)) return rc;
    t.dev.heights = t.d_heights;
    t.dev.normals = t.d_normals;
    t.dev.block_minmax = t.d_minmax;
    t.dev.trig_lon = t.d_minmax + (size_t)bxc * byc * 2;
    t.dev.trig_lat = t.dev.trig_lon + 2 * (size_t)w;
    t.dev.block_bounds = reinterpret_cast<const double*>(t.pool.as<uint8_t>() + off_bounds);
    t.dev.raster_x = rp[0]; t.dev.raster_y = rp[1];
    t.dev.model_x = mp[0]; t.dev.model_y = mp[1];
    t.dev.scale_x = ps[0]; t.dev.scale_y = ps[1];
    terrain_rotation(mp[0], mp[1], t.dev.rot);
    struct Retired {
        Tile tile;
        hipStream_t stream;
        ~Retired() { if (tile.pool.p) (void)hipStreamSynchronize(stream); }
    } old{Tile{}, stream_};
    if (Tile* ex = find(lat, lon)) { old.tile = std::move(*ex); tiles_.erase(geo_key(lat, lon)); }
    Tile& nt = tiles_[geo_key(lat, lon)] = std::move(t);
    table_dirty_ = true;
    ++tile_gen_;
    if (int rc = upload_tile_table()) return rc;
    {
        const std::map<GeoKey, uint32_t> rk = ranks();
        std::vector<EdgeJob> edges;
        std::vector<CornerJob> corners;
        collect_jobs(nt, rk, edges, corners);
        launch_load_kernels(rk.at(geo_key(lat, lon)), 1, nullptr);
        if (int rc = run_seam_jobs(edges, corners)) return rc;
    }
    TOPO_HIP_TRY(hipStreamSynchronize(stream_));
    {
        std::vector<double> sph((size_t)bxc * byc * 4);
        TOPO_HIP_TRY(hipMemcpy(sph.data(), nt.dev.block_bounds, sph.size() * sizeof(double), hipMemcpyDeviceToHost));
        double c[3] = {0.0, 0.0, 0.0}, r2 = 0.0;
        bool finite = true;
        for (size_t i = 0; i < sph.size(); i += 4) {
            finite = finite && std::isfinite(sph[i]) && std::isfinite(sph[i + 1]) && std::isfinite(sph[i + 2]) && std::isfinite(sph[i + 3]);
            for (int k = 0; k < 3; ++k) c[k] += sph[i + k];
        }
        for (int k = 0; k < 3; ++k) c[k] /= (double)(sph.size() / 4);
        for (size_t i = 0; i < sph.size() && finite; i += 4) {
            const double dx = sph[i] - c[0], dy = sph[i + 1] - c[1], dz = sph[i + 2] - c[2];
            r2 = std::max(r2, dx * dx + dy * dy + dz * dz);
        }
        nt.centres[0] = c[0]; nt.centres[1] = c[1]; nt.centres[2] = c[2];
        nt.centres[3] = finite ? std::sqrt(r2) : -1.0;
    }
    TOPO_HIP_TRY(hipGetLastError());
    return TOPO_OK;
}

void TerrainRenderer::launch_load_kernels(uint32_t first, uint32_t count, hipEvent_t mid) {
    const TileDev* tiles = d_tiles_.as<const TileDev>();
    if (normals_tables_fused(tile_w_, tile_h_, lds_rows_)) {
        launch_trig_tables(tiles, first, count, tile_w_, tile_h_, stream_);
        if (mid) (void)hipEventRecord(mid, stream_);
        launch_normals_tables(tiles, first, count, tile_w_, tile_h_, stream_);
        launch_block_bounds(tiles, first, count, tile_w_, tile_h_, stream_);
    } else {
        launch_block_tables(tiles, first, count, tile_w_, tile_h_, stream_);
        if (mid) (void)hipEventRecord(mid, stream_);
        launch_normals_interior(tiles, first, count, tile_w_, tile_h_, lds_rows_, stream_);
    }
}

int TerrainRenderer::unload_terrain(int32_t lat, int32_t lon) {
    Tile* t = find(lat, lon);
    if (!t) return TOPO_OK;
    if (int rc = wait_all()) return rc;
    tiles_.erase(geo_key(lat, lon));
    table_dirty_ = true;
    ++tile_gen_;
    return TOPO_OK;
}

int TerrainRenderer::recompute_normals() {
    if (int rc = join()) return rc;
    std::vector<Tile*> order;
    for (auto& kv : tiles_) order.push_back(&kv.second);
    std::sort(order.begin(), order.end(), [](Tile* a, Tile* b) { return a->seq < b->seq; });
    if (int rc = upload_tile_table()) return rc;
    const std::map<GeoKey, uint32_t> rk = ranks();
    std::vector<EdgeJob> edges;
    std::vector<CornerJob> corners;
    for (Tile* t : order) collect_jobs(*t, rk, edges, corners);
    if (int rc = ensure(stream_, d_edge_jobs_, (edges.size() + 1) * sizeof(EdgeJob))) return rc;
    if (int rc = ensure(stream_, d_corner_jobs_, (corners.size() + 1) * sizeof(CornerJob))) return rc;
    if (int rc = upload_seam_jobs(edges, corners)) return rc;
    TOPO_HIP_TRY(hipEventRecord(load_ev_[0], stream_));
    launch_load_kernels(0, (uint32_t)order.size(), load_ev_[2]);
    launch_seam_jobs(edges.size(), corners.size());
    TOPO_HIP_TRY(hipEventRecord(load_ev_[1], stream_));
    TOPO_HIP_TRY(hipStreamSynchronize(stream_));
    load_timed_ = true;
    TOPO_HIP_TRY(hipGetLastError());
    return TOPO_OK;
}

int TerrainRenderer::update(uint32_t w, uint32_t h, const topo_uniforms* u, const topo_post_uniforms* pu) {
    if (!u || !pu) return fail(TOPO_ERR_INVALID, "null argument");
    if (w == 0 || h == 0) return fail(TOPO_ERR_INVALID, "target size must be non-zero");
    if (pu->pixelize_n < 99.99999f && !(pu->pixelize_n >= 1.0f)) return fail(TOPO_ERR_INVALID, "pixelize_n must be at least 1");
    if (pu->pixelize_n < 99.99999f && !(pu->viewport[0] >= 1.0f && pu->viewport[1] >= 1.0f)) return fail(TOPO_ERR_INVALID, "viewport must be at least 1 x 1");
    W_ = w;
    H_ = h;
    uniforms_ = *u;
    post_ = *pu;
    have_uniforms_ = true;
    return TOPO_OK;
}

int TerrainRenderer::upload_tile_table() {
    if (!table_dirty_) return TOPO_OK;
    std::vector<TileDev> table;
    for (auto& kv : tiles_) table.push_back(kv.second.dev);
    if (!table.empty()) {
        if (int rc = ensure(stream_, d_tiles_, table.size() * sizeof(TileDev))) return rc;
        TOPO_HIP_TRY(hipStreamSynchronize(stream_));
        TOPO_HIP_TRY(hipMemcpy(d_tiles_.p, table.data(), table.size() * sizeof(TileDev), hipMemcpyHostToDevice));
        if (vs_ever_) {
            std::vector<uint32_t*> masks;
            for (auto& kv : tiles_) masks.push_back(kv.second.mask.as<uint32_t>());
            if (int rc = ensure(stream_, d_vs_table_, masks.size() * sizeof(uint32_t*))) return rc;
            TOPO_HIP_TRY(hipMemcpy(d_vs_table_.p, masks.data(), masks.size() * sizeof(uint32_t*), hipMemcpyHostToDevice));
        }
    }
    table_dirty_ = false;
    return TOPO_OK;
}

int TerrainRenderer::init_ctx(FrameCtx& c, bool own_stream) {
    for (auto& f : c.timed_frames)
        for (auto& e : f.ev)
            if (!e) TOPO_HIP_TRY(hipEventCreate(&e.h));
    if (!c.done) TOPO_HIP_TRY(hipEventCreateWithFlags(&c.done.h, hipEventDisableTiming));
    if (own_stream && !c.stream) TOPO_HIP_TRY(hipStreamCreateWithFlags(&c.stream.h, hipStreamNonBlocking));
    return TOPO_OK;
}

int TerrainRenderer::join() {
    if (int rc = bind_device()) return rc;
    for (auto& c : ctx_)
        if (c.pending) {
            if (c.last_stream) TOPO_HIP_TRY(hipStreamSynchronize(c.last_stream));
            c.pending = false;
        }
    return TOPO_OK;
}

bool TerrainRenderer::fold_frames(FrameCtx& c, uint64_t end) {
    bool overflow = false;
    for (; c.checked < end; ++c.checked) {
        const uint32_t* w = c.status_words(c.checked);
        last_status_[0] |= w[kCtrStatus];
        if (w[kCtrStatus] & kStatusBounds) record_bounds(w);
        overflow |= (w[kCtrStatus] & kStatusRareOverflow) != 0;
    }
    return overflow;
}

void TerrainRenderer::record_bounds(const uint32_t* w) {
    last_status_[0] |= kStatusBounds;
    last_status_[1] = w[kCtrBoundsTag]; last_status_[2] = w[kCtrBoundsLo]; last_status_[3] = w[kCtrBoundsHi];
}

bool TerrainRenderer::fold_idle() {
    bool overflow = false;
    for (auto& c : ctx_)
        if (!c.pending && c.h_status.p) overflow |= fold_frames(c);
    return overflow;
}

bool TerrainRenderer::fold_latest(FrameCtx& c, bool retry) {
    overflow_pending_ |= fold_frames(c, c.submitted - 1);
    const bool overflow = (c.latest_status()[kCtrStatus] & kStatusRareOverflow) != 0;
    if (overflow && retry) ++c.checked;
    else (void)fold_frames(c);
    return overflow;
}

int TerrainRenderer::check_frames() {
    const bool overflow = fold_idle() | overflow_pending_;
    overflow_pending_ = false;
    if (overflow) return fail(TOPO_ERR_CAPACITY, "rare-triangle queue overflowed: a frame is incomplete (raise the queue capacity or render fewer views per submission)");
    return TOPO_OK;
}

int TerrainRenderer::set_pipeline_depth(int depth) {
    if (depth < 1 || depth > kMaxPipeline) return fail(TOPO_ERR_INVALID, "pipeline depth must be 1..4");
    if (int rc = wait_all()) return rc;
    for (int i = 0; i < depth; ++i)
        if (int rc = init_ctx(ctx_[i], depth > 1)) return rc;
    pipeline_depth_ = depth;
    next_ctx_ = last_ctx_ = 0;
    return TOPO_OK;
}

static const char* submission_error(uint32_t n, uint32_t w, uint32_t h) {
    if (n > 0xFFFFu) return "too many views";
    if (w == 0 || h == 0 || w > 65536 || h > 65536) return "bad target size";
    return nullptr;
}

int TerrainRenderer::render_views_device(uint32_t n, const topo_uniforms* views, uint32_t w, uint32_t h, const OutputParams& out) {
    if (n == 0 || !views || !out.rgba) return fail(TOPO_ERR_INVALID, "null/empty argument");
    if (const char* e = submission_error(n, w, h)) return fail(TOPO_ERR_INVALID, e);
    if (int rc = bind_device()) return rc;
    if (table_dirty_)
        if (int rc = join()) return rc;
    if (int rc = upload_tile_table()) return rc;
    FrameCtx& c = ctx_[next_ctx_];
    last_ctx_ = next_ctx_;
    next_ctx_ = (next_ctx_ + 1) % pipeline_depth_;
    if (pipeline_depth_ == 1) return render_frame(c, stream_, n, views, w, h, out);
    TOPO_HIP_TRY(hipEventRecord(c.done, stream_));
    TOPO_HIP_TRY(hipStreamWaitEvent(c.stream, c.done, 0));
    return render_frame(c, c.stream, n, views, w, h, out);
}

static bool far_phase_empty(const topo_uniforms* views, uint32_t n, const std::map<GeoKey, Tile>& tiles, float* split_m) {
    double bound = 0.0;
    for (uint32_t i = 0; i < n && bound >= 0.0; ++i) {
        const float* m = views[i].camera_proj;
        const double wn = std::sqrt((double)m[3] * m[3] + (double)m[7] * m[7] + (double)m[11] * m[11]);
        for (const auto& kv : tiles) {
            const double* s = kv.second.centres;
            const double w_far = (double)m[3] * s[0] + (double)m[7] * s[1] + (double)m[11] * s[2] + (double)m[15] + s[3] * wn;
            if (!(s[3] >= 0.0) || !(w_far < 1e30)) { bound = -1.0; break; }
            bound = std::max(bound, w_far);
        }
    }
    if (!(bound >= 0.0 && bound + 2.0 < (double)*split_m * (4.0 / 3.0))) return false;
    *split_m = std::max(*split_m, (float)(bound + 2.0));
    return true;
}

static bool fused_clear_cull(const FrameParams& p) { return switches().fuse_clear_cull && p.n_tiles != 0; }

int TerrainRenderer::render_frame(FrameCtx& c, hipStream_t stream, uint32_t n, const topo_uniforms* views, uint32_t w, uint32_t h,
                                  const OutputParams& out, const ResolveSlot* slots, uint32_t n_slots,
                                  const std::function<int(uint32_t, hipStream_t)>* after_slot) {
    if (n == 0) return fail(TOPO_ERR_INVALID, "null/empty argument");
    if (const char* e = submission_error(n, w, h)) return fail(TOPO_ERR_INVALID, e);
    latest_ctx_ = -1;
    FrameParams p{};
    if (int rc = grow_frame_buffers(c, stream, n, w, h, p)) return rc;
    ViewPack pack{};
    bool pack_in_cull = false;
    if (int rc = stage_views(c, stream, views, p, pack, &pack_in_cull)) return rc;
    fill_params(c, p);
    last_blocks_tested_ = p.work_cap;
    last_far_phase_ = p.split_m > 0.0f && !(switches().far_skip && far_phase_empty(views, n, tiles_, &p.split_m));
    if (int rc = queue_frame(c, stream, p, pack_in_cull ? &pack : nullptr, last_far_phase_, out, slots, n_slots, after_slot)) return rc;
    record_submission(c, p);
    TOPO_HIP_TRY(hipGetLastError());
    return TOPO_OK;
}

int TerrainRenderer::grow_frame_buffers(FrameCtx& c, hipStream_t stream, uint32_t n, uint32_t w, uint32_t h, FrameParams& p) {
    p.n_views = n;
    p.n_tiles = (uint32_t)tiles_.size();
    p.W = (int32_t)w;
    p.H = (int32_t)h;
    p.bx_count = p.n_tiles ? (tile_w_ - 1 + kBCX - 1) / kBCX : 0;
    p.by_count = p.n_tiles ? (tile_h_ - 1 + kBCY - 1) / kBCY : 0;
    const size_t pixels = (size_t)n * w * h;
    const size_t work_cap = (size_t)n * p.n_tiles * p.bx_count * p.by_count;
    p.big_cap = big_cap_cfg_ ? big_cap_cfg_ : (1u << 22);
    p.rare_cap = rare_cap_cfg_ ? rare_cap_cfg_ : (rare_cap_auto_ ? (uint32_t)rare_cap_auto_ : (1u << 22));
    if (work_cap >= (1ull << 30)) return fail(TOPO_ERR_CAPACITY, "too many raster blocks in one submission");
    if (pixels >= (1ull << 32)) return fail(TOPO_ERR_CAPACITY, "more than 2^32 pixels in one submission");
    const size_t vis_keys = (pixels + 63) & ~(size_t)63;
    if (vis_keys * 8 > c.d_vis.cap) {
        if (int rc = ensure(stream, c.d_vis, vis_keys * 8)) return rc;
        if (int rc = ensure(stream, c.d_dirty, vis_keys / 64 + 64)) return rc;
        TOPO_HIP_TRY(hipMemsetAsync(c.d_dirty.p, 1, c.d_dirty.cap, stream));
    }
    if (int rc = ensure(stream_, d_views_, sizeof(ViewDev) * kMaxViewsPerSlot * kViewSlots)) return rc;
    const int strip_env = switches().near_strip;
    p.near_strip = strip_env >= 1 && strip_env <= 15 ? (uint32_t)strip_env : (work_cap <= 64 * 1024 ? 1u : 2u);
    const size_t near_cap = (size_t)((kBCY + p.near_strip - 1) / p.near_strip) * work_cap;
    if (int rc = ensure(stream, c.d_work, (near_cap ? near_cap : 1) * sizeof(WorkItem))) return rc;
    if (int rc = ensure(stream, c.d_work2, (near_cap ? near_cap : 1) * sizeof(WorkItem))) return rc;
    const size_t far_sub_cap = ((work_cap + 255) / 256 + kFarLists - 1) / kFarLists * 256;
    if (int rc = ensure(stream, c.d_far, (far_sub_cap ? far_sub_cap * kFarLists : 1) * sizeof(FarItem))) return rc;
    if (int rc = ensure(stream, c.d_big, p.big_cap * sizeof(BigItem))) return rc;
    if (int rc = ensure(stream, c.d_rare, p.rare_cap * sizeof(RareItem))) return rc;
    if (!c.d_counters.p) {
        if (int rc = ensure(stream, c.d_counters, 2 * kCounterWords * sizeof(uint32_t))) return rc;
        TOPO_HIP_TRY(hipMemsetAsync(c.d_counters.p, 0, 2 * kCounterWords * sizeof(uint32_t), stream));
    }
    if (int rc = ensure_pinned(c.h_status, kStatusRing * kStatusWords * sizeof(uint32_t))) return rc;
    if (c.submitted - c.checked == kStatusRing) {
        if (c.last_stream) TOPO_HIP_TRY(hipStreamSynchronize(c.last_stream));
        overflow_pending_ |= fold_frames(c);
    }
    c.last_stream = stream;
    c.pending = pipeline_depth_ > 1;
    p.work_cap = (uint32_t)work_cap;
    p.far_sub_cap = (uint32_t)far_sub_cap;
    p.near_cap = (uint32_t)near_cap;
    return TOPO_OK;
}

int TerrainRenderer::stage_views(FrameCtx& c, hipStream_t stream, const topo_uniforms* views, FrameParams& p, ViewPack& pack, bool* pack_in_cull) {
    const uint32_t n = p.n_views;
    if (n > kMaxViewsPerSlot) return fail(TOPO_ERR_INVALID, "too many views in one submission");
    static_assert(kViewSlots % kMaxPipeline == 0, "every frame context has its own share of the slots");
    const int slot = (int)(&c - ctx_) * (kViewSlots / kMaxPipeline) + (int)(c.frames % (kViewSlots / kMaxPipeline));
    ViewDev* d_slot = d_views_.as<ViewDev>() + (size_t)slot * kMaxViewsPerSlot;
    p.views = d_slot;
    auto fill_views = [&](ViewDev* vd) {
        for (uint32_t i = 0; i < n; ++i) {
            memcpy(vd[i].proj, views[i].camera_proj, sizeof vd[i].proj);
            vd[i].cam_x = views[i].camera_pos[0];
            vd[i].cam_y = views[i].camera_pos[1];
            memcpy(vd[i].sun, views[i].sun_direction, sizeof vd[i].sun);
            vd[i].view_mode = views[i].view_mode;
        }
    };
    const bool packed = n <= kPackViews && !switches().views_by_copy;
    *pack_in_cull = packed && fused_clear_cull(p) && switches().views_in_cull;
    if (packed) {
        fill_views(pack.v);
        if (!*pack_in_cull) launch_put_views(pack, n, d_slot, stream);
        return TOPO_OK;
    }
    if (!view_ev_[kViewSlots - 1]) {
        if (int rc = ensure_pinned(h_views_, sizeof(ViewDev) * kMaxViewsPerSlot * kViewSlots)) return rc;
        for (auto& e : view_ev_)
            if (!e) TOPO_HIP_TRY(hipEventCreateWithFlags(&e.h, hipEventDisableTiming));
    }
    if (view_used_[slot]) TOPO_HIP_TRY(hipEventSynchronize(view_ev_[slot]));
    ViewDev* vd = h_views_.as<ViewDev>() + (size_t)slot * kMaxViewsPerSlot;
    fill_views(vd);
    TOPO_HIP_TRY(hipMemcpyAsync(d_slot, vd, n * sizeof(ViewDev), hipMemcpyHostToDevice, stream));
    TOPO_HIP_TRY(hipEventRecord(view_ev_[slot], stream));
    view_used_[slot] = true;
    return TOPO_OK;
}

void TerrainRenderer::fill_params(FrameCtx& c, FrameParams& p) {
    p.tiles = d_tiles_.as<const TileDev>();
    p.vis = c.d_vis.as<uint64_t>();
    p.dirty = c.d_dirty.as<uint8_t>();
    p.work = c.d_work.as<WorkItem>();
    p.counters = c.d_counters.as<uint32_t>() + (c.frames & 1u) * kCounterWords;
#ifdef TOPO_BOUNDS_CHECK
    p.status_out = nullptr;
#else
    p.status_out = switches().status_by_copy ? nullptr : c.status_words(c.submitted);
#endif
    p.big = c.d_big.as<BigItem>();
    p.rare = c.d_rare.as<RareItem>();
    p.far = c.d_far.as<FarItem>();
    p.work2 = c.d_work2.as<WorkItem>();
    p.split_m = occlusion_split_m_;
    p.tile_w = tile_w_;
    p.tile_h = tile_h_;
    p.tris_per_tile = p.n_tiles ? 2u * (tile_w_ - 1) * (tile_h_ - 1) : 8u;
    p.div_tris = fastdiv_make(p.tris_per_tile);
    p.div_hm1 = fastdiv_make(p.n_tiles ? tile_h_ - 1 : 2u);
    p.rblocks_x = ((uint32_t)p.W + kResolveBlockW - 1) / kResolveBlockW;
    p.rblocks_view = p.rblocks_x * (((uint32_t)p.H + kResolveBlockH - 1) / kResolveBlockH);
    p.div_rblocks_x = fastdiv_make(p.rblocks_x > 1 ? p.rblocks_x : 2u);
    p.div_rblocks_view = fastdiv_make(p.rblocks_view > 1 ? p.rblocks_view : 2u);
    float thresh[256];
    for (int i = 0; i < 256; ++i) thresh[i] = bits_f(TOPO_SRGB_THRESH_BITS[i]);
    p.linear_target = is_linear(format_) ? 1u : 0u;
    p.bgra = is_bgra(format_) ? 1u : 0u;
    p.sky_c8 = (p.linear_target ? to_unorm8(0.0f) | (to_unorm8(0.71f) << 8) | (to_unorm8(0.885f) << 16)
                                : srgb_encode(thresh, 0.0f) | (srgb_encode(thresh, 0.71f) << 8) | (srgb_encode(thresh, 0.885f) << 16)) |
               (to_unorm8(1.0f) << 24);
}

int TerrainRenderer::queue_frame(FrameCtx& c, hipStream_t stream, FrameParams& p, const ViewPack* pack_in_cull, bool far_phase, const OutputParams& out,
                                 const ResolveSlot* slots, uint32_t n_slots, const std::function<int(uint32_t, hipStream_t)>* after_slot) {
    const uint32_t n = p.n_views, w = (uint32_t)p.W, h = (uint32_t)p.H;
    uint32_t* const counters_next = c.d_counters.as<uint32_t>() + ((c.frames & 1u) ^ 1u) * kCounterWords;
    uint32_t ev_need = timing_total_ ? kTotalEvents : 0u;
    for (int sl = 0; sl < kTimingSlots; ++sl)
        for (int st = 0; st < kNumStages; ++st)
            if ((timing_slots_ & (1u << sl)) && (kStagesOfSlot[sl] & (1u << st))) ev_need |= stage_events(st);
    const bool pixelize = post_.pixelize_n < 99.99999f;
    const bool own_times = !switches().events_by_marker && !pixelize && (ev_need & ~(kTotalEvents | stage_events(kStResolve))) == 0;
    FrameCtx::TimedFrame& tf = c.timed_frames[c.frames++ % kEvRing];
    tf.recorded = ev_need;
    tf.slots = timing_slots_;
    tf.frame = ++frame_seq_;
    auto mark = [&](int i, bool may_be_own = false) { return (ev_need >> i & 1u) && !(may_be_own && own_times) ? hipEventRecord(tf.ev[i], stream) : hipSuccess; };
    auto own = [&](int i) -> hipEvent_t { return (ev_need >> i & 1u) && own_times ? (hipEvent_t)tf.ev[i] : nullptr; };
    TOPO_HIP_TRY(mark(kStClear, true));
    const hipEvent_t ev_first = own(kStClear);
    const bool fuse = fused_clear_cull(p);
    if (fuse) launch_clear_cull(p, counters_next, stream, ev_first, pack_in_cull, n);
    else launch_clear(p, counters_next, stream, ev_first);
    TOPO_HIP_TRY(mark(kStCull));
    if (!fuse) launch_cull(p, stream);
    TOPO_HIP_TRY(mark(kStRasterNear));
    launch_raster(p, 0, stream);
    TOPO_HIP_TRY(mark(kStRareBigNear));
    launch_raster_rare(p, stream);
    launch_raster_big(p, stream);
    TOPO_HIP_TRY(mark(kStOcclusion));
    if (far_phase) launch_occlusion(p, stream);
    TOPO_HIP_TRY(mark(kStRasterFar));
    if (far_phase) launch_raster(p, 1, stream);
    TOPO_HIP_TRY(mark(kStRareBigFar));
    if (far_phase) {
        launch_raster_rare(p, stream);
        launch_raster_big(p, stream);
    }
    TOPO_HIP_TRY(mark(kStResolve, true));
    const hipEvent_t ev_rstart = own(kStResolve), ev_rstop = own(kNumStages);
    OutputParams kout = out;
    if (pixelize) {
        if (n_slots) return fail(TOPO_ERR_UNSUPPORTED, "the pixelise branch is not available on the slot-by-slot (multi-GPU) path");
        const size_t img = (size_t)w * h * 4;
        if (int rc = ensure(stream, c.d_pre_rgba, img * n)) return rc;
        if (!out.depth)
            if (int rc = ensure(stream, c.d_pre_depth, img * n)) return rc;
        kout.rgba = c.d_pre_rgba.as<uint8_t>();
        kout.rgba_view_stride = img;
        kout.rgba_pitch = (size_t)w * 4;
        if (!out.depth) { kout.depth = c.d_pre_depth.as<float>(); kout.depth_view_stride = img; kout.depth_pitch = (size_t)w * 4; }
        p.post_off = 1;
    }
    if (n_slots == 0) {
        p.rblock_first = 0;
        p.rblock_count = p.rblocks_view * n;
        launch_resolve(p, kout, stream, ev_rstart, ev_rstop);
        if (pixelize)
            launch_post_pixelize(n, (int32_t)w, (int32_t)h, post_.viewport[0] >= 1.0f ? post_.viewport[0] : (float)w, post_.viewport[1] >= 1.0f ? post_.viewport[1] : (float)h,
                                 post_.pixelize_n, c.d_pre_rgba.as<const uint8_t>(), out, kout.depth, kout.depth_view_stride, kout.depth_pitch, p.linear_target, p.bgra, stream);
    } else {
        for (uint32_t i = 0; i < n_slots; ++i) {
            if ((uint64_t)slots[i].block_first + slots[i].block_count > (uint64_t)p.rblocks_view * n) return fail(TOPO_ERR_INVALID, "resolve slot outside the frame");
            p.rblock_first = slots[i].block_first;
            p.rblock_count = slots[i].block_count;
            launch_resolve(p, out, stream, i == 0 ? ev_rstart : nullptr, i + 1 == n_slots ? ev_rstop : nullptr);
            if (after_slot)
                if (int rc = (*after_slot)(i, stream)) return rc;
        }
    }
    if (vs_on_)
        launch_viewshed(p, d_vs_table_.as<uint32_t* const>(), d_vs_stats_.as<unsigned long long>(), stream);
    TOPO_HIP_TRY(mark(kNumStages, true));
    if (!p.status_out) TOPO_HIP_TRY(hipMemcpyAsync(c.status_words(c.submitted), p.counters, kStatusWords * sizeof(uint32_t), hipMemcpyDeviceToHost, stream));
    return TOPO_OK;
}

void TerrainRenderer::record_submission(FrameCtx& c, const FrameParams& p) {
    ++c.submitted;
    c.timed = true;
    c.sub.n_views = p.n_views;
    c.sub.tile_gen = tile_gen_;
    HorizonParams& q = c.sub.query;
    q.vis = p.vis;
    q.dirty = p.dirty;
    q.counters = p.counters;
    q.W = (uint32_t)p.W;
    q.H = (uint32_t)p.H;
    q.n_keys = (size_t)p.n_views * q.W * q.H;
    q.n_tiles = p.n_tiles;
    q.tris_per_tile = p.tris_per_tile;
    q.hm1 = p.n_tiles ? tile_h_ - 1 : 2u;
    q.div_tris = p.div_tris;
    q.div_hm1 = p.div_hm1;
    latest_ctx_ = (int)(&c - ctx_);
}


int TerrainRenderer::alloc_mask(Tile& t) {
    DeviceBuffer m;
    if (int rc = ensure(stream_, m, mask_bytes())) return rc;
    TOPO_HIP_TRY(hipMemsetAsync(m.p, 0, mask_bytes(), stream_));
    t.mask = std::move(m);
    return TOPO_OK;
}

int TerrainRenderer::viewshed_enable(bool on) {
    if (int rc = bind_device()) return rc;
    if (on && !vs_ever_) {
        if (int rc = join()) return rc;
        const size_t stats = (size_t)kViewshedStatSlots * 4 * sizeof(unsigned long long);
        if (!d_vs_stats_.p) {
            if (int rc = ensure(stream_, d_vs_stats_, stats)) return rc;
            TOPO_HIP_TRY(hipMemsetAsync(d_vs_stats_.p, 0, stats, stream_));
        }
        for (auto& kv : tiles_)
            if (!kv.second.mask.p)
                if (int rc = alloc_mask(kv.second)) return rc;
        vs_ever_ = true;
        table_dirty_ = true;
    }
    vs_on_ = on;
    return TOPO_OK;
}

int TerrainRenderer::viewshed_reset() {
    if (int rc = bind_device()) return rc;
    if (!vs_ever_) return TOPO_OK;
    if (int rc = join()) return rc;
    for (auto& kv : tiles_) TOPO_HIP_TRY(hipMemsetAsync(kv.second.mask.p, 0, mask_bytes(), stream_));
    TOPO_HIP_TRY(hipMemsetAsync(d_vs_stats_.p, 0, (size_t)kViewshedStatSlots * 4 * sizeof(unsigned long long), stream_));
    return TOPO_OK;
}

int TerrainRenderer::viewshed_read(int32_t lat, int32_t lon, uint8_t* mask_out, size_t pitch, uint64_t* n_visible) {
    if (!mask_out) return fail(TOPO_ERR_INVALID, "mask_out is null");
    Tile* t = find(lat, lon);
    if (!t) return fail(TOPO_ERR_NOT_FOUND, "no such tile");
    if (!vs_ever_) return fail(TOPO_ERR_INVALID, "viewshed accumulation was never enabled");
    const uint32_t wm1 = tile_w_ - 1, hm1 = tile_h_ - 1;
    if (pitch < wm1) return fail(TOPO_ERR_INVALID, "pitch smaller than a row");
    if (int rc = wait_all()) return rc;
    std::vector<uint32_t> words(mask_bytes() / 4);
    TOPO_HIP_TRY(hipMemcpy(words.data(), t->mask.p, mask_bytes(), hipMemcpyDeviceToHost));
    uint64_t count = 0;
    for (uint32_t x = 0, bit = 0; x < wm1; ++x)
        for (uint32_t y = 0; y < hm1; ++y, ++bit) {
            const uint8_t v = (uint8_t)((words[bit >> 5] >> (bit & 31u)) & 1u);
            mask_out[(size_t)y * pitch + x] = v;
            count += v;
        }
    if (n_visible) *n_visible = count;
    return TOPO_OK;
}

int TerrainRenderer::viewshed_stats(uint64_t out[3]) {
    if (!out) return fail(TOPO_ERR_INVALID, "null argument");
    out[0] = out[1] = out[2] = 0;
    if (!vs_ever_) return TOPO_OK;
    if (int rc = wait_all()) return rc;
    std::vector<unsigned long long> s((size_t)kViewshedStatSlots * 4);
    TOPO_HIP_TRY(hipMemcpy(s.data(), d_vs_stats_.p, s.size() * sizeof(s[0]), hipMemcpyDeviceToHost));
    for (size_t i = 0; i < s.size(); i += 4)
        for (int k = 0; k < 3; ++k) out[k] += s[i + k];
    return TOPO_OK;
}


static_assert(sizeof(HorizonPoint) == sizeof(topo_horizon_point) && sizeof(topo_horizon_point) == 32, "horizon record layout");

int TerrainRenderer::horizon_shape(uint32_t* n_views, uint32_t* w, uint32_t* h) {
    if (!n_views || !w || !h) return fail(TOPO_ERR_INVALID, "null argument");
    if (latest_ctx_ < 0) return fail(TOPO_ERR_INVALID, "no submission to query");
    const FrameCtx::Submission& s = ctx_[latest_ctx_].sub;
    *n_views = s.n_views;
    *w = s.query.W;
    *h = s.query.H;
    return TOPO_OK;
}

int TerrainRenderer::horizon_prepare(uint32_t first, uint32_t n, size_t view_stride, FrameCtx** out_c, hipStream_t* out_s) {
    if (latest_ctx_ < 0) return fail(TOPO_ERR_INVALID, "no submission to query");
    FrameCtx& c = ctx_[latest_ctx_];
    if (c.sub.tile_gen != tile_gen_) return fail(TOPO_ERR_INVALID, "tiles were added or unloaded since the latest submission: its draw order is gone");
    if (n == 0 || first >= c.sub.n_views || n > c.sub.n_views - first) return fail(TOPO_ERR_INVALID, "views outside the latest submission");
    if (view_stride < c.sub.query.W) return fail(TOPO_ERR_INVALID, "view stride smaller than a view's width");
    if (int rc = bind_device()) return rc;
    *out_c = &c;
    *out_s = c.last_stream ? c.last_stream : stream_;
    return TOPO_OK;
}

int TerrainRenderer::horizon_launch(FrameCtx& c, uint32_t first, uint32_t n, HorizonPoint* out, size_t view_stride, hipStream_t s) {
    if (hz_ll_gen_ != tile_gen_) {
        if (int rc = wait_all()) return rc;
        hz_ll_.clear();
        for (const auto& kv : tiles_) {
            hz_ll_.push_back(kv.second.lat);
            hz_ll_.push_back(kv.second.lon);
        }
        if (int rc = ensure(stream_, d_hz_ll_, (hz_ll_.size() + 2) * sizeof(int32_t))) return rc;
        if (!hz_ll_.empty()) TOPO_HIP_TRY(hipMemcpyAsync(d_hz_ll_.p, hz_ll_.data(), hz_ll_.size() * sizeof(int32_t), hipMemcpyHostToDevice, s));
        hz_ll_gen_ = tile_gen_;
    }
#ifdef TOPO_BOUNDS_CHECK
    if (!d_hz_check_.p) {
        if (int rc = ensure(s, d_hz_check_, kStatusWords * sizeof(uint32_t))) return rc;
        TOPO_HIP_TRY(hipMemsetAsync(d_hz_check_.p, 0, kStatusWords * sizeof(uint32_t), s));
    }
#endif
    HorizonParams p = c.sub.query;
    p.check = d_hz_check_.as<uint32_t>();
    p.tile_ll = d_hz_ll_.as<const int32_t>();
    p.out = out;
    p.view_stride = view_stride;
    p.first_view = first;
    p.n_views = n;
    launch_horizon(p, s);
    TOPO_HIP_TRY(hipGetLastError());
    return TOPO_OK;
}

int TerrainRenderer::horizon_fold_check() {
#ifdef TOPO_BOUNDS_CHECK
    if (!d_hz_check_.p) return TOPO_OK;
    uint32_t w[kStatusWords];
    TOPO_HIP_TRY(hipMemcpy(w, d_hz_check_.p, sizeof w, hipMemcpyDeviceToHost));
    if (w[kCtrStatus] & kStatusBounds) {
        record_bounds(w);
        TOPO_HIP_TRY(hipMemset(d_hz_check_.p, 0, sizeof w));
    }
#endif
    return TOPO_OK;
}

int TerrainRenderer::horizon_read(uint32_t first, uint32_t n, topo_horizon_point* out, size_t view_stride) {
    if (!out) return fail(TOPO_ERR_INVALID, "null argument");
    FrameCtx* c = nullptr;
    hipStream_t s = nullptr;
    if (int rc = horizon_prepare(first, n, view_stride, &c, &s)) return rc;
    const size_t row = (size_t)c->sub.query.W * sizeof(HorizonPoint);
    if (int rc = ensure(s, d_hz_out_, row * n)) return rc;
    if (int rc = horizon_launch(*c, first, n, d_hz_out_.as<HorizonPoint>(), c->sub.query.W, s)) return rc;
    TOPO_HIP_TRY(hipMemcpy2DAsync(out, view_stride * sizeof(topo_horizon_point), d_hz_out_.p, row, row, n, hipMemcpyDeviceToHost, s));
    TOPO_HIP_TRY(hipStreamSynchronize(s));
    c->pending = false;
    const bool overflow = fold_latest(*c, false);
    if (int rc = horizon_fold_check()) return rc;
    if (overflow)
        return fail(TOPO_ERR_CAPACITY, "rare-triangle queue overflowed: the latest submission is incomplete, and so is its horizon");
    return TOPO_OK;
}

int TerrainRenderer::horizon_device(uint32_t first, uint32_t n, topo_horizon_point* out_dev, size_t view_stride) {
    if (!out_dev) return fail(TOPO_ERR_INVALID, "null argument");
    if ((uintptr_t)out_dev % 16 != 0) return fail(TOPO_ERR_INVALID, "out_dev must be 16-byte aligned");
    FrameCtx* c = nullptr;
    hipStream_t s = nullptr;
    if (int rc = horizon_prepare(first, n, view_stride, &c, &s)) return rc;
    if (int rc = horizon_launch(*c, first, n, (HorizonPoint*)out_dev, view_stride, s)) return rc;
    if (s != stream_) c->pending = true;
    return TOPO_OK;
}

int TerrainRenderer::render_device(uint8_t* rgba_dev, size_t rgba_pitch, float* depth_dev, size_t depth_pitch) {
    if (!rgba_dev) return fail(TOPO_ERR_INVALID, "rgba_dev is null");
    if (!have_uniforms_) return fail(TOPO_ERR_INVALID, "topo_update has not been called");
    if (rgba_pitch < (size_t)W_ * 4 || (depth_dev && depth_pitch < (size_t)W_ * 4)) return fail(TOPO_ERR_INVALID, "pitch smaller than a row");
    return render_views_device(1, &uniforms_, W_, H_, image_output(rgba_dev, rgba_pitch, depth_dev, depth_pitch, H_));
}

int TerrainRenderer::render(uint8_t* rgba, size_t rgba_pitch, float* depth, size_t depth_pitch) {
    if (!rgba) return fail(TOPO_ERR_INVALID, "rgba_out is null");
    if (!have_uniforms_) return fail(TOPO_ERR_INVALID, "topo_update has not been called");
    if (rgba_pitch < (size_t)W_ * 4 || (depth && depth_pitch < (size_t)W_ * 4)) return fail(TOPO_ERR_INVALID, "pitch smaller than a row");
    if (int rc = bind_device()) return rc;
    const size_t row = (size_t)W_ * 4;
    if (int rc = ensure(stream_, d_out_rgba_, row * H_)) return rc;
    if (depth)
        if (int rc = ensure(stream_, d_out_depth_, row * H_)) return rc;
    const OutputParams o = image_output(d_out_rgba_.as<uint8_t>(), row, depth ? d_out_depth_.as<float>() : nullptr, row, H_);
    if (int rc = wait_all()) return rc;
    overflow_pending_ |= fold_idle();
    for (int attempt = 0;; ++attempt) {
        if (int rc = render_views_device(1, &uniforms_, W_, H_, o)) return rc;
        if (int rc = wait_all()) return rc;
        FrameCtx& fc = ctx_[last_ctx_];
        const bool retry = rare_cap_cfg_ == 0 && attempt < 3;
        if (!fold_latest(fc, retry)) break;
        if (!retry) return fail(TOPO_ERR_CAPACITY, "rare-triangle queue overflowed: frame incomplete");
        const uint32_t wanted = fc.latest_status()[kCtrRare];
        rare_cap_auto_ = (uint64_t)wanted + wanted / 4u + 1024u;
        if (rare_cap_auto_ > (1ull << 28)) return fail(TOPO_ERR_CAPACITY, "rare-triangle queue would exceed 2^28 entries");
    }
    if (int rc = download(rgba, rgba_pitch, d_out_rgba_.as<const uint8_t>(), row)) return rc;
    if (depth)
        if (int rc = download((uint8_t*)depth, depth_pitch, d_out_depth_.as<const uint8_t>(), row)) return rc;
    have_depth_ = depth != nullptr;
    depth_w_ = W_;
    depth_h_ = H_;
    return TOPO_OK;
}

int TerrainRenderer::download(uint8_t* dst, size_t dst_pitch, const uint8_t* src_dev, size_t row) {
    const size_t span = dst_pitch * (H_ - 1) + row;
    for (const auto& pin : pinned_)
        if (dst >= pin.as<uint8_t>() && dst + span <= pin.as<uint8_t>() + pin.cap) {
            TOPO_HIP_TRY(hipMemcpy2DAsync(dst, dst_pitch, src_dev, row, row, H_, hipMemcpyDeviceToHost, stream_));
            TOPO_HIP_TRY(hipStreamSynchronize(stream_));
            return TOPO_OK;
        }
    const size_t total = row * H_;
    if (int rc = ensure_pinned(h_stage_, total)) return rc;
    uint8_t* const stage = h_stage_.as<uint8_t>();
    constexpr int kSlices = 8;
    for (auto& e : stage_ev_)
        if (!e) TOPO_HIP_TRY(hipEventCreateWithFlags(&e.h, hipEventDisableTiming));
    const uint32_t rows_per = (H_ + kSlices - 1) / kSlices;
    int n_slices = 0;
    for (uint32_t r0 = 0; r0 < H_; r0 += rows_per, ++n_slices) {
        const uint32_t rows = std::min(rows_per, H_ - r0);
        TOPO_HIP_TRY(hipMemcpyAsync(stage + (size_t)r0 * row, src_dev + (size_t)r0 * row, (size_t)rows * row, hipMemcpyDeviceToHost, stream_));
        TOPO_HIP_TRY(hipEventRecord(stage_ev_[n_slices], stream_));
    }
    const unsigned hw = std::thread::hardware_concurrency();
    const int n_threads = (int)std::min<size_t>(std::max(1u, std::min(hw ? hw : 4u, 8u)), std::max<size_t>(1, total >> 20));
    std::atomic<int> failed{0};
// ... 410 lines not shown
```

topo-renderer_amd/csrc/terrain_renderer.hpp:

```cpp
#pragma once

#include <hip/hip_runtime.h>

#include <cstdint>
#include <functional>
#include <map>
#include <string>
#include <tuple>
#include <utility>
#include <vector>

#include "../../include/topo_hip.h"
#include "host_math.hpp"
#include "topo_kernels.h"

namespace topo {

constexpr uint32_t kPanoramaSectors = 8;
struct Comm;

using GeoKey = std::tuple<int, int, int, int>;
inline GeoKey geo_key(int lat, int lon) {
    return GeoKey(lat < 0 ? -lat : lat, lat > 0 ? 1 : 0, lon < 0 ? -lon : lon, lon > 0 ? 1 : 0);
}

#define TOPO_HIP_TRY(expr)                                   \
    do {                                                     \
        hipError_t e_ = (expr);                              \
        if (e_ != hipSuccess) return hip_fail(e_, #expr);    \
    } while (0)

template <hipError_t (*Free)(void*)>
struct Block {
    void* p = nullptr;
    size_t cap = 0;
    Block() = default;
    Block(Block&& o) noexcept : p(std::exchange(o.p, nullptr)), cap(std::exchange(o.cap, 0)) {}
    Block& operator=(Block&& o) noexcept { if (this != &o) { reset(); p = std::exchange(o.p, nullptr); cap = std::exchange(o.cap, 0); } return *this; }
    ~Block() { reset(); }
    void reset() { if (p) (void)Free(p); p = nullptr; cap = 0; }
    template <class T> T* as() const { return static_cast<T*>(p); }
};
using DeviceBuffer = Block<hipFree>;
using PinnedBuffer = Block<hipHostFree>;
using HostRegistration = Block<hipHostUnregister>;

template <class H, hipError_t (*Destroy)(H)>
struct Handle {
    H h = nullptr;
    Handle() = default;
    Handle(Handle&& o) noexcept : h(std::exchange(o.h, nullptr)) {}
    Handle& operator=(Handle&& o) noexcept { if (this != &o) { reset(); h = std::exchange(o.h, nullptr); } return *this; }
    ~Handle() { reset(); }
    void reset() { if (h) (void)Destroy(h); h = nullptr; }
    operator H() const { return h; }
};
using Event = Handle<hipEvent_t, hipEventDestroy>;
using Stream = Handle<hipStream_t, hipStreamDestroy>;

inline OutputParams image_output(uint8_t* rgba, size_t rgba_pitch, float* depth, size_t depth_pitch, uint32_t rows) {
    return OutputParams{rgba, rgba_pitch * rows, rgba_pitch, depth, depth_pitch * rows, depth_pitch};
}

struct Tile {
    int lat = 0, lon = 0;
    uint64_t seq = 0;
    DeviceBuffer pool;
    float* d_heights = nullptr;
    uint32_t* d_normals = nullptr;
    float* d_minmax = nullptr;
    double centres[4] = {0.0, 0.0, 0.0, -1.0};
    TileDev dev{};
    DeviceBuffer mask;
};

enum Stage { kStClear, kStCull, kStRasterNear, kStRareBigNear, kStOcclusion, kStRasterFar, kStRareBigFar, kStResolve, kNumStages };

class TerrainRenderer {
   public:
    static int create(TerrainRenderer** out, int device, uint32_t w, uint32_t h, uint32_t format, std::string* err);
    ~TerrainRenderer();

    int add_terrain(int32_t lat, int32_t lon, const float* heights, bool heights_on_device, uint32_t w, uint32_t h,
                    const float rp[2], const float mp[2], const float ps[2]);
    int unload_terrain(int32_t lat, int32_t lon);
    bool last_far_phase() const { return last_far_phase_; }
    int update(uint32_t w, uint32_t h, const topo_uniforms* u, const topo_post_uniforms* pu);
    int render(uint8_t* rgba, size_t rgba_pitch, float* depth, size_t depth_pitch);
    int render_views_device(uint32_t n, const topo_uniforms* views, uint32_t w, uint32_t h, const OutputParams& out);
    int render_device(uint8_t* rgba_dev, size_t rgba_pitch, float* depth_dev, size_t depth_pitch);
    int render_panorama(Comm* comm, const float eye[3], float yaw0, float pitch, uint32_t sector_w, uint32_t sector_h, float sun_theta_deg,
                        float sun_phi_deg, int32_t view_mode, uint8_t* strip_dev, float* depth_dev);
    int render_batch(uint32_t n_viewpoints, const float* eyes, const float* yaw0s, const float* sun_theta_phi_deg, float pitch, uint32_t sector_w,
                     uint32_t sector_h, int32_t view_mode, uint8_t* rgba_dev, float* depth_dev);
    int recompute_normals();
    int overlay_lines_device(const void* vertices, uint32_t n_vertices, const uint32_t* indices, uint32_t n_indices, float line_width, uint8_t* rgba_dev,
                             size_t rgba_pitch);
    int overlay_glyphs(const void* glyphs, uint32_t n_glyphs, float depth, const uint8_t* atlas, uint32_t atlas_w, uint32_t atlas_h, uint8_t* rgba, size_t rgba_pitch);
    int overlay_glyphs_device(const void* glyphs, uint32_t n_glyphs, float depth, const uint8_t* atlas, uint32_t atlas_w, uint32_t atlas_h, uint8_t* rgba_dev,
                              size_t rgba_pitch);
    int overlay_lines(const void* vertices, uint32_t n_vertices, const uint32_t* indices, uint32_t n_indices, float line_width, uint8_t* rgba,
                      size_t rgba_pitch);
    int change_location(float latitude, float longitude, float range_dist, std::vector<std::pair<int32_t, int32_t>>& request, uint32_t* n_unloaded);

    int set_stream(hipStream_t s);
    int synchronize();
    int set_pipeline_depth(int depth);
    int join();
    int join_frames();
    int set_normals_lds_rows(int rows);
    int set_queue_caps(uint32_t big_cap, uint32_t rare_cap);
    int pin_host_buffer(void* p, size_t bytes);
    int unpin_host_buffer(void* p);
    int get_timings(float out[TOPO_TIMING_SLOTS]);
    int get_timing_history(uint32_t n_frames, float* out_ms, uint32_t* n_out);
    int get_counters(uint32_t out[6]);
    int frame_status(uint32_t out[4]);
    int set_occlusion_split(float metres);
    int set_timing_slots(uint32_t mask);
    int read_normals(int32_t lat, int32_t lon, uint8_t* out);
    int read_tile_tables(int32_t lat, int32_t lon, float* minmax_out, float* trig_out, double* bounds_out, uint32_t* n_blocks_out);
    int geotiff_to_device(const uint8_t* bytes, size_t n, DeviceBuffer& heights, uint32_t* w, uint32_t* h, float rp[2], float mp[2], float ps[2]);
    int geotiff_decode(const uint8_t* bytes, size_t n, float* heights_out, size_t capacity);
    int add_terrain_geotiff(int32_t lat, int32_t lon, const uint8_t* bytes, size_t n);
    int probe_sincos(const float* x, float* s, float* c, size_t n);
    int probe_div(int32_t kind, const float* x, const float* y, float* out, size_t n);
    int visible_peaks(uint32_t n, const float* peaks, uint8_t* visible, uint32_t* xy);
    int visible_peaks_device(const topo_uniforms* view, uint32_t w, uint32_t h, const float* depth_dev, size_t depth_pitch,
                             uint32_t n, const float* peaks_dev, uint8_t* visible_dev, uint32_t* xy_dev);

    int viewshed_enable(bool on);
    int viewshed_reset();
    int viewshed_read(int32_t lat, int32_t lon, uint8_t* mask_out, size_t pitch, uint64_t* n_visible);
    int viewshed_stats(uint64_t out[3]);

    int horizon_shape(uint32_t* n_views, uint32_t* w, uint32_t* h);
    int horizon_read(uint32_t first_view, uint32_t n_views, topo_horizon_point* out, size_t view_stride);
    int horizon_device(uint32_t first_view, uint32_t n_views, topo_horizon_point* out_dev, size_t view_stride);

    const char* last_error() const { return err_.c_str(); }

   private:
    TerrainRenderer() = default;
    int init();
    int fail(int code, const std::string& msg);
    int hip_fail(hipError_t e, const char* what);
    int bind_device();
    int ensure(hipStream_t s, DeviceBuffer& b, size_t need);
    int ensure_pinned(PinnedBuffer& b, size_t need);
    int wait_all();
    void collect_jobs(const Tile& nt, const std::map<GeoKey, uint32_t>& rank, std::vector<EdgeJob>& edges,
                      std::vector<CornerJob>& corners);
    int run_seam_jobs(const std::vector<EdgeJob>& edges, const std::vector<CornerJob>& corners);
    int upload_seam_jobs(const std::vector<EdgeJob>& edges, const std::vector<CornerJob>& corners);
    void launch_seam_jobs(size_t n_edges, size_t n_corners);
    void launch_load_kernels(uint32_t first, uint32_t count, hipEvent_t mid);
    std::map<GeoKey, uint32_t> ranks() const;
    Tile* find(int lat, int lon);
    int upload_tile_table();
    int overlay_upload(const void* a, size_t a_bytes, const void* b, size_t b_bytes, uint8_t** b_dev, bool* keys_fresh);
    template <class Draw> int overlay_host_image(uint8_t* rgba, size_t rgba_pitch, Draw draw);
    int alloc_mask(Tile& t);
    size_t mask_bytes() const { return (((size_t)(tile_w_ - 1) * (tile_h_ - 1) + 31) / 32) * 4; }

    int device_ = 0;
    uint32_t W_ = 0, H_ = 0;
    uint32_t format_ = TOPO_FORMAT_RGBA8_UNORM_SRGB;
    uint32_t tile_w_ = 0, tile_h_ = 0;
    topo_uniforms uniforms_{};
    topo_post_uniforms post_{{0.0f, 0.0f}, 100.0f, 0.0f};
    bool have_uniforms_ = false;
    std::map<GeoKey, Tile> tiles_;
    uint64_t next_seq_ = 1;
    bool table_dirty_ = true;
    int lds_rows_ = 0;
    uint32_t big_cap_cfg_ = 0, rare_cap_cfg_ = 0;
    uint64_t rare_cap_auto_ = 0;
    uint32_t timing_slots_ = 0x3Fu;
    bool timing_total_ = true;
    float occlusion_split_m_ = 90000.0f;

    Stream own_stream_;
    hipStream_t stream_ = nullptr;
    static constexpr int kEvRing = 32;
    static constexpr uint64_t kStatusRing = 64;
    uint64_t frame_seq_ = 0;
    Event load_ev_[3];
    bool load_timed_ = false;

    struct FrameCtx {
        Stream stream;
        struct TimedFrame {
            Event ev[kNumStages + 1];
            uint32_t recorded = 0, slots = 0;
            uint64_t frame = 0;
        } timed_frames[kEvRing];
        uint64_t frames = 0;
        Event done;
        hipStream_t last_stream = nullptr;
        bool timed = false, pending = false;
        PinnedBuffer h_status;
        uint64_t submitted = 0, checked = 0;
        uint32_t* status_words(uint64_t frame) const { return h_status.as<uint32_t>() + (frame % kStatusRing) * kStatusWords; }
        const uint32_t* latest_status() const { return status_words(submitted - 1); }
        DeviceBuffer d_vis, d_dirty;
        DeviceBuffer d_work, d_work2, d_far, d_big, d_rare, d_counters;
        DeviceBuffer d_pre_rgba, d_pre_depth;
        struct Submission {
            uint32_t n_views = 0;
            uint64_t tile_gen = 0;
            HorizonParams query{};
        } sub;
    };
    static constexpr int kMaxPipeline = 4;
    FrameCtx ctx_[kMaxPipeline];
    int pipeline_depth_ = 1, next_ctx_ = 0, last_ctx_ = 0;
    int init_ctx(FrameCtx& c, bool own_stream);
    int check_frames();
    uint32_t last_status_[4] = {};
    bool fold_frames(FrameCtx& c, uint64_t end);
    bool fold_frames(FrameCtx& c) { return fold_frames(c, c.submitted); }
    bool fold_idle();
    bool fold_latest(FrameCtx& c, bool retry);
    void record_bounds(const uint32_t* words);
    bool overflow_pending_ = false;
    struct ResolveSlot { uint32_t block_first, block_count; };
    int render_frame(FrameCtx& c, hipStream_t s, uint32_t n, const topo_uniforms* views, uint32_t w, uint32_t h, const OutputParams& out,
                     const ResolveSlot* slots = nullptr, uint32_t n_slots = 0, const std::function<int(uint32_t, hipStream_t)>* after_slot = nullptr);
    int grow_frame_buffers(FrameCtx& c, hipStream_t s, uint32_t n, uint32_t w, uint32_t h, FrameParams& p);
    int stage_views(FrameCtx& c, hipStream_t s, const topo_uniforms* views, FrameParams& p, ViewPack& pack, bool* pack_in_cull);
    void fill_params(FrameCtx& c, FrameParams& p);
    int queue_frame(FrameCtx& c, hipStream_t s, FrameParams& p, const ViewPack* pack_in_cull, bool far_phase, const OutputParams& out, const ResolveSlot* slots,
                    uint32_t n_slots, const std::function<int(uint32_t, hipStream_t)>* after_slot);
    void record_submission(FrameCtx& c, const FrameParams& p);
    int frame_durations(const FrameCtx::TimedFrame& f, float out[7]);

    DeviceBuffer d_tiles_, d_views_, d_edge_jobs_, d_corner_jobs_, d_out_rgba_, d_out_depth_;
    PinnedBuffer h_stage_;
    Event stage_ev_[8];
    std::vector<HostRegistration> pinned_;
    int download(uint8_t* dst, size_t dst_pitch, const uint8_t* src_dev, size_t row);
    static constexpr int kViewSlots = 16;
    static constexpr uint32_t kMaxViewsPerSlot = 64;
    PinnedBuffer h_views_;
    Event view_ev_[kViewSlots];
    bool view_used_[kViewSlots] = {};
    DeviceBuffer d_peaks_;
    DeviceBuffer d_proj_;
    DeviceBuffer d_overlay_geo_;
    DeviceBuffer d_overlay_keys_;
    uint32_t overlay_w_ = 0, overlay_h_ = 0;
    bool have_depth_ = false;
    uint32_t depth_w_ = 0, depth_h_ = 0;
    uint32_t last_blocks_tested_ = 0;
    bool last_far_phase_ = true;
    bool vs_on_ = false, vs_ever_ = false;
    DeviceBuffer d_vs_table_;
    DeviceBuffer d_vs_stats_;
    int latest_ctx_ = -1;
    uint64_t tile_gen_ = 0;
    std::vector<int32_t> hz_ll_;
    uint64_t hz_ll_gen_ = ~0ull;
    DeviceBuffer d_hz_ll_, d_hz_out_;
    DeviceBuffer d_hz_check_;
    int horizon_prepare(uint32_t first_view, uint32_t n_views, size_t view_stride, FrameCtx** c, hipStream_t* s);
    int horizon_launch(FrameCtx& c, uint32_t first_view, uint32_t n_views, HorizonPoint* out, size_t view_stride, hipStream_t s);
    int horizon_fold_check();

    std::string err_;
};

int comm_unique_id(uint8_t out[128], std::string* err);
int comm_init(Comm** out, int device, const uint8_t id128[128], int rank, int world, std::string* err);
int comm_from_nccl(Comm** out, void* nccl_comm, int rank, int world, std::string* err);
void comm_destroy(Comm* c);
void panorama_sector_range(int rank, int world, uint32_t* first, uint32_t* count);
uint32_t panorama_slots(int world, uint32_t sector_w, uint32_t sector_h, topo_panorama_slot* out, uint32_t cap);

}
```

topo-renderer_amd/csrc/topo_capi.cpp:

```cpp
#include <cmath>
#include <cstdint>
#include <cstring>
#include <new>
#include <string>
#include <utility>
#include <vector>

#include "../../include/topo_hip_test.h"
#include "geotiff.hpp"
#include "terrain_renderer.hpp"

struct topo_ctx {
    topo::TerrainRenderer* r = nullptr;
};

namespace {
thread_local std::string g_create_error;
}

#define TOPO_GUARD(ctx)                       \
    if (!(ctx) || !(ctx)->r) return TOPO_ERR_INVALID

extern "C" {

int topo_create(topo_ctx** out, int hip_device, uint32_t width, uint32_t height, uint32_t color_format) {
    if (!out) return TOPO_ERR_INVALID;
    *out = nullptr;
    topo::TerrainRenderer* r = nullptr;
    int rc;
    try {
        rc = topo::TerrainRenderer::create(&r, hip_device, width, height, color_format, &g_create_error);
    } catch (const std::exception& e) {
        g_create_error = e.what();
        return TOPO_ERR_HIP;
    }
    if (rc != TOPO_OK) return rc;
    topo_ctx* c = new (std::nothrow) topo_ctx();
    if (!c) { delete r; return TOPO_ERR_HIP; }
    c->r = r;
    *out = c;
    return TOPO_OK;
}

void topo_destroy(topo_ctx* ctx) {
    if (!ctx) return;
    delete ctx->r;
    delete ctx;
}

const char* topo_last_error(topo_ctx* ctx) {
    if (!ctx || !ctx->r) return g_create_error.c_str();
    return ctx->r->last_error();
}

#define TOPO_CALL(expr)                                         \
    try {                                                       \
        return (expr);                                          \
    } catch (const std::exception&) {                           \
        return TOPO_ERR_HIP;                                    \
    }

int topo_add_terrain(topo_ctx* ctx, int32_t lat, int32_t lon, const float* heights, uint32_t w, uint32_t h,
                     const float rp[2], const float mp[2], const float ps[2]) {
    TOPO_GUARD(ctx);
    TOPO_CALL(ctx->r->add_terrain(lat, lon, heights, false, w, h, rp, mp, ps));
}

int topo_add_terrain_device(topo_ctx* ctx, int32_t lat, int32_t lon, const float* heights_dev, uint32_t w, uint32_t h,
                            const float rp[2], const float mp[2], const float ps[2]) {
    TOPO_GUARD(ctx);
    TOPO_CALL(ctx->r->add_terrain(lat, lon, heights_dev, true, w, h, rp, mp, ps));
}

int topo_unload_terrain(topo_ctx* ctx, int32_t lat, int32_t lon) {
    TOPO_GUARD(ctx);
    TOPO_CALL(ctx->r->unload_terrain(lat, lon));
}

int topo_update(topo_ctx* ctx, uint32_t w, uint32_t h, const topo_uniforms* u, const topo_post_uniforms* pu) {
    TOPO_GUARD(ctx);
    TOPO_CALL(ctx->r->update(w, h, u, pu));
}

int topo_render(topo_ctx* ctx, uint8_t* rgba, size_t rgba_pitch, float* depth, size_t depth_pitch) {
    TOPO_GUARD(ctx);
    TOPO_CALL(ctx->r->render(rgba, rgba_pitch, depth, depth_pitch));
}

int topo_recompute_normals(topo_ctx* ctx) {
    TOPO_GUARD(ctx);
    TOPO_CALL(ctx->r->recompute_normals());
}

int topo_render_views_device(topo_ctx* ctx, uint32_t n_views, const topo_uniforms* views, uint32_t width, uint32_t height,
                             uint8_t* rgba_dev, size_t rgba_view_stride, size_t rgba_pitch, float* depth_dev,
                             size_t depth_view_stride, size_t depth_pitch) {
    TOPO_GUARD(ctx);
    topo::OutputParams o{};
    o.rgba = rgba_dev;
    o.rgba_view_stride = rgba_view_stride;
    o.rgba_pitch = rgba_pitch;
    o.depth = depth_dev;
    o.depth_view_stride = depth_view_stride;
    o.depth_pitch = depth_pitch;
    TOPO_CALL(ctx->r->render_views_device(n_views, views, width, height, o));
}

int topo_set_stream(topo_ctx* ctx, void* hip_stream) {
    TOPO_GUARD(ctx);
    TOPO_CALL(ctx->r->set_stream((hipStream_t)hip_stream));
}

int topo_synchronize(topo_ctx* ctx) {
    TOPO_GUARD(ctx);
    TOPO_CALL(ctx->r->synchronize());
}

int topo_set_normals_lds_rows(topo_ctx* ctx, int rows) {
    TOPO_GUARD(ctx);
    return ctx->r->set_normals_lds_rows(rows);
}

int topo_debug_set_queue_caps(topo_ctx* ctx, uint32_t big_cap, uint32_t rare_cap) {
    TOPO_GUARD(ctx);
    TOPO_CALL(ctx->r->set_queue_caps(big_cap, rare_cap));
}

int topo_debug_far_phase_launched(topo_ctx* ctx, int32_t* out) {
    TOPO_GUARD(ctx);
    if (!out) return TOPO_ERR_INVALID;
    *out = ctx->r->last_far_phase() ? 1 : 0;
    return TOPO_OK;
}

int topo_get_timings(topo_ctx* ctx, float out_ms[TOPO_TIMING_SLOTS]) {
    TOPO_GUARD(ctx);
    TOPO_CALL(ctx->r->get_timings(out_ms));
}

int topo_pin_host_buffer(topo_ctx* ctx, void* buffer, size_t bytes) {
    TOPO_GUARD(ctx);
    TOPO_CALL(ctx->r->pin_host_buffer(buffer, bytes));
}

int topo_unpin_host_buffer(topo_ctx* ctx, void* buffer) {
    TOPO_GUARD(ctx);
    TOPO_CALL(ctx->r->unpin_host_buffer(buffer));
}

int topo_get_timing_history(topo_ctx* ctx, uint32_t n_frames, float* out_ms, uint32_t* n_out) {
    TOPO_GUARD(ctx);
    if (!n_out) return TOPO_ERR_INVALID;
    TOPO_CALL(ctx->r->get_timing_history(n_frames, out_ms, n_out));
}

int topo_set_timing_slots(topo_ctx* ctx, uint32_t slot_mask) {
    TOPO_GUARD(ctx);
    TOPO_CALL(ctx->r->set_timing_slots(slot_mask));
}

int topo_set_occlusion_split(topo_ctx* ctx, float metres) {
    TOPO_GUARD(ctx);
    return ctx->r->set_occlusion_split(metres);
}

int topo_get_counters(topo_ctx* ctx, uint32_t out[6]) {
    TOPO_GUARD(ctx);
    TOPO_CALL(ctx->r->get_counters(out));
}

int topo_read_normals(topo_ctx* ctx, int32_t lat, int32_t lon, uint8_t* out) {
    TOPO_GUARD(ctx);
    TOPO_CALL(ctx->r->read_normals(lat, lon, out));
}

int topo_read_tile_tables(topo_ctx* ctx, int32_t lat, int32_t lon, float* minmax_out, float* trig_out, double* bounds_out, uint32_t* n_blocks_out) {
    TOPO_GUARD(ctx);
    TOPO_CALL(ctx->r->read_tile_tables(lat, lon, minmax_out, trig_out, bounds_out, n_blocks_out));
}

int topo_visible_peaks(topo_ctx* ctx, uint32_t n_peaks, const float* peaks_xyz, uint8_t* visible_out, uint32_t* xy_out) {
    TOPO_GUARD(ctx);
    TOPO_CALL(ctx->r->visible_peaks(n_peaks, peaks_xyz, visible_out, xy_out));
}

int topo_visible_peaks_device(topo_ctx* ctx, const topo_uniforms* view, uint32_t width, uint32_t height, const float* depth_dev,
                              size_t depth_pitch, uint32_t n_peaks, const float* peaks_xyz_dev, uint8_t* visible_dev,
                              uint32_t* xy_dev) {
    TOPO_GUARD(ctx);
    TOPO_CALL(ctx->r->visible_peaks_device(view, width, height, depth_dev, depth_pitch, n_peaks, peaks_xyz_dev, visible_dev, xy_dev));
}

int topo_probe_sincos(topo_ctx* ctx, const float* x, float* s, float* c, size_t n) {
    TOPO_GUARD(ctx);
    TOPO_CALL(ctx->r->probe_sincos(x, s, c, n));
}

int topo_set_pipeline_depth(topo_ctx* ctx, int32_t depth) {
    TOPO_GUARD(ctx);
    TOPO_CALL(ctx->r->set_pipeline_depth(depth));
}

int topo_join(topo_ctx* ctx) {
    TOPO_GUARD(ctx);
    TOPO_CALL(ctx->r->join_frames());
}

struct topo_comm {
    topo::Comm* c = nullptr;
};

int topo_comm_unique_id(uint8_t out_id[TOPO_COMM_ID_BYTES]) {
    if (!out_id) return TOPO_ERR_INVALID;
    try {
        return topo::comm_unique_id(out_id, &g_create_error);
    } catch (const std::exception& e) {
        g_create_error = e.what();
        return TOPO_ERR_HIP;
    }
}

int topo_comm_init(topo_comm** out, int hip_device, const uint8_t id[TOPO_COMM_ID_BYTES], int rank, int world) {
    if (!out || (world > 1 && !id)) return TOPO_ERR_INVALID;
    *out = nullptr;
    topo::Comm* c = nullptr;
    static const uint8_t zero[TOPO_COMM_ID_BYTES] = {};
    int rc;
    try {
        rc = topo::comm_init(&c, hip_device, id ? id : zero, rank, world, &g_create_error);
    } catch (const std::exception& e) {
        g_create_error = e.what();
        return TOPO_ERR_HIP;
    }
    if (rc != TOPO_OK) return rc;
    *out = new topo_comm();
    (*out)->c = c;
    return TOPO_OK;
}

int topo_comm_from_nccl(topo_comm** out, void* nccl_comm, int rank, int world) {
    if (!out) return TOPO_ERR_INVALID;
    *out = nullptr;
    topo::Comm* c = nullptr;
    if (int rc = topo::comm_from_nccl(&c, nccl_comm, rank, world, &g_create_error)) return rc;
    *out = new topo_comm();
    (*out)->c = c;
    return TOPO_OK;
}

void topo_comm_destroy(topo_comm* comm) {
    if (!comm) return;
    topo::comm_destroy(comm->c);
    delete comm;
}

void topo_panorama_sector_range(int rank, int world, uint32_t* first, uint32_t* count) {
    if (first && count && world >= 1 && rank >= 0 && rank < world) topo::panorama_sector_range(rank, world, first, count);
}

uint32_t topo_panorama_slots(int world, uint32_t sector_w, uint32_t sector_h, topo_panorama_slot* out, uint32_t cap) {
    if (world < 1 || topo::kPanoramaSectors % (uint32_t)world != 0 || sector_w == 0 || sector_h == 0) return 0;
    return topo::panorama_slots(world, sector_w, sector_h, out, cap);
}

int topo_render_panorama(topo_ctx* ctx, topo_comm* comm, const float eye[3], float yaw0, float pitch, uint32_t sector_w, uint32_t sector_h,
                         float sun_theta_deg, float sun_phi_deg, int32_t view_mode, uint8_t* strip_dev, float* depth_dev) {
    TOPO_GUARD(ctx);
    TOPO_CALL(ctx->r->render_panorama(comm ? comm->c : nullptr, eye, yaw0, pitch, sector_w, sector_h, sun_theta_deg, sun_phi_deg, view_mode,
                                      strip_dev, depth_dev));
}

int topo_render_batch(topo_ctx* ctx, uint32_t n_viewpoints, const float* eyes_xyz, const float* yaw0, const float* sun_theta_phi_deg,
                      float pitch, uint32_t sector_w, uint32_t sector_h, int32_t view_mode, uint8_t* rgba_dev, float* depth_dev) {
    TOPO_GUARD(ctx);
    TOPO_CALL(ctx->r->render_batch(n_viewpoints, eyes_xyz, yaw0, sun_theta_phi_deg, pitch, sector_w, sector_h, view_mode, rgba_dev, depth_dev));
}

static uint32_t put_pairs(const std::vector<std::pair<int32_t, int32_t>>& v, int32_t* out, uint32_t cap) {
    for (uint32_t i = 0; i < v.size() && i < cap && out; ++i) { out[2 * i] = v[i].first; out[2 * i + 1] = v[i].second; }
    return (uint32_t)v.size();
}

void topo_change_location_plan(float latitude, float longitude, float range_dist, const int32_t* loaded_lat_lon, uint32_t n_loaded,
                               int32_t* unload_out, uint32_t unload_cap, uint32_t* n_unload, int32_t* request_out, uint32_t request_cap,
                               uint32_t* n_request) {
    std::vector<std::pair<int32_t, int32_t>> unload, request;
    topo::change_location_plan(latitude, longitude, range_dist, loaded_lat_lon, loaded_lat_lon ? n_loaded : 0, unload, request);
    const uint32_t nu = put_pairs(unload, unload_out, unload_cap), nr = put_pairs(request, request_out, request_cap);
    if (n_unload) *n_unload = nu;
    if (n_request) *n_request = nr;
}

int topo_change_location(topo_ctx* ctx, float latitude, float longitude, float range_dist, int32_t* request_out, uint32_t request_cap,
                         uint32_t* n_request, uint32_t* n_unloaded) {
    TOPO_GUARD(ctx);
    try {
        std::vector<std::pair<int32_t, int32_t>> request;
        const int rc = ctx->r->change_location(latitude, longitude, range_dist, request, n_unloaded);
        if (rc != TOPO_OK) return rc;
        const uint32_t nr = put_pairs(request, request_out, request_cap);
        if (n_request) *n_request = nr;
        return TOPO_OK;
    } catch (const std::exception&) {
        return TOPO_ERR_HIP;
    }
}

int topo_overlay_lines(topo_ctx* ctx, const topo_overlay_vertex* vertices, uint32_t n_vertices, const uint32_t* indices, uint32_t n_indices,
                       float line_width, uint8_t* rgba, size_t rgba_pitch) {
    TOPO_GUARD(ctx);
    TOPO_CALL(ctx->r->overlay_lines(vertices, n_vertices, indices, n_indices, line_width, rgba, rgba_pitch));
}

int topo_overlay_lines_device(topo_ctx* ctx, const topo_overlay_vertex* vertices, uint32_t n_vertices, const uint32_t* indices, uint32_t n_indices,
                              float line_width, uint8_t* rgba_dev, size_t rgba_pitch) {
    TOPO_GUARD(ctx);
    TOPO_CALL(ctx->r->overlay_lines_device(vertices, n_vertices, indices, n_indices, line_width, rgba_dev, rgba_pitch));
}

int topo_overlay_glyphs(topo_ctx* ctx, const topo_glyph* glyphs, uint32_t n_glyphs, float depth, const uint8_t* atlas_mask, uint32_t atlas_w, uint32_t atlas_h,
                        uint8_t* rgba, size_t rgba_pitch) {
    TOPO_GUARD(ctx);
    TOPO_CALL(ctx->r->overlay_glyphs(glyphs, n_glyphs, depth, atlas_mask, atlas_w, atlas_h, rgba, rgba_pitch));
}

int topo_overlay_glyphs_device(topo_ctx* ctx, const topo_glyph* glyphs, uint32_t n_glyphs, float depth, const uint8_t* atlas_mask, uint32_t atlas_w,
                               uint32_t atlas_h, uint8_t* rgba_dev, size_t rgba_pitch) {
    TOPO_GUARD(ctx);
    TOPO_CALL(ctx->r->overlay_glyphs_device(glyphs, n_glyphs, depth, atlas_mask, atlas_w, atlas_h, rgba_dev, rgba_pitch));
}

int topo_viewshed_enable(topo_ctx* ctx, int32_t on) {
    TOPO_GUARD(ctx);
    TOPO_CALL(ctx->r->viewshed_enable(on != 0));
}

int topo_viewshed_reset(topo_ctx* ctx) {
    TOPO_GUARD(ctx);
    TOPO_CALL(ctx->r->viewshed_reset());
}

int topo_viewshed_read(topo_ctx* ctx, int32_t lat_deg, int32_t lon_deg, uint8_t* mask_out, size_t pitch, uint64_t* n_visible_out) {
    TOPO_GUARD(ctx);
    TOPO_CALL(ctx->r->viewshed_read(lat_deg, lon_deg, mask_out, pitch, n_visible_out));
}

int topo_debug_viewshed_stats(topo_ctx* ctx, uint64_t out[3]) {
    TOPO_GUARD(ctx);
    TOPO_CALL(ctx->r->viewshed_stats(out));
}

int topo_horizon_shape(topo_ctx* ctx, uint32_t* n_views, uint32_t* width, uint32_t* height) {
    TOPO_GUARD(ctx);
    TOPO_CALL(ctx->r->horizon_shape(n_views, width, height));
}

int topo_horizon_read(topo_ctx* ctx, uint32_t first_view, uint32_t n_views, topo_horizon_point* out, size_t view_stride) {
    TOPO_GUARD(ctx);
    TOPO_CALL(ctx->r->horizon_read(first_view, n_views, out, view_stride));
}

int topo_horizon_device(topo_ctx* ctx, uint32_t first_view, uint32_t n_views, topo_horizon_point* out_dev, size_t view_stride) {
    TOPO_GUARD(ctx);
    TOPO_CALL(ctx->r->horizon_device(first_view, n_views, out_dev, view_stride));
}

void topo_pixel_angles(const topo_uniforms* view, uint32_t width, uint32_t height, uint32_t n, const float* xy, double* az_el_out) {
    if (!view || !az_el_out || (n && !xy) || width == 0 || height == 0) return;
    topo::pixel_angles(view, width, height, n, xy, az_el_out);
}

int topo_frame_status(topo_ctx* ctx, uint32_t out[4]) {
    TOPO_GUARD(ctx);
    if (!out) return TOPO_ERR_INVALID;
    TOPO_CALL(ctx->r->frame_status(out));
}

int topo_probe_div(topo_ctx* ctx, int32_t kind, const float* x, const float* y, float* out, size_t n) {
    TOPO_GUARD(ctx);
    TOPO_CALL(ctx->r->probe_div(kind, x, y, out, n));
}

void topo_camera_uniforms(const float eye[3], float yaw, float pitch, float fov_y, float width, float height,
                          float sun_theta_deg, float sun_phi_deg, int32_t view_mode, topo_uniforms* out) {
    topo::camera_uniforms(eye, yaw, pitch, fov_y, width, height, sun_theta_deg, sun_phi_deg, view_mode, out);
}

float topo_sector_fov_y(uint32_t sector_w, uint32_t sector_h, uint32_t n_sectors) {
    return (float)(2.0 * atan(tan(3.14159265358979323846 / (double)n_sectors) * (double)sector_h / (double)sector_w));
}

void topo_panorama_uniforms(const float eye[3], float yaw0, float pitch, uint32_t sector_w, uint32_t sector_h, float sun_theta_deg,
                            float sun_phi_deg, int32_t view_mode, uint32_t n_sectors, topo_uniforms* out) {
    topo::panorama_uniforms(eye, yaw0, pitch, sector_w, sector_h, sun_theta_deg, sun_phi_deg, view_mode, n_sectors, out);
}

int topo_render_device(topo_ctx* ctx, uint8_t* rgba_dev, size_t rgba_pitch, float* depth_dev, size_t depth_pitch) {
    TOPO_GUARD(ctx);
    TOPO_CALL(ctx->r->render_device(rgba_dev, rgba_pitch, depth_dev, depth_pitch));
}

void topo_terrain_uniforms(const float rp[2], const float mp[2], const float ps[2], uint32_t w, uint32_t h, float out[24]) {
    memset(out, 0, 24 * sizeof(float));
    out[0] = rp[0]; out[1] = rp[1]; out[2] = mp[0]; out[3] = mp[1]; out[4] = ps[0]; out[5] = ps[1];
    out[6] = (float)w; out[7] = (float)h;
    float rot[9];
    topo::terrain_rotation(mp[0], mp[1], rot);
    for (int c = 0; c < 3; ++c)
        for (int r = 0; r < 3; ++r) out[8 + c * 4 + r] = rot[c * 3 + r];
    out[8 + 15] = 1.0f;
}

void topo_geometry_transform(float h, float lon_deg, float lat_deg, float out[3]) {
    topo::geometry_transform(h, lon_deg, lat_deg, out);
}

float topo_dist_from_depth(float depth) { return topo::kFar * topo::kNear / (topo::kFar - depth * (topo::kFar - topo::kNear)); }

uint32_t topo_pad_256(uint32_t size) { return ((size - 1) / 256 + 1) * 256; }

int topo_coordinate_transform(const double* pixel_scale, uint32_t n_pixel_scale, const double* tie_points, uint32_t n_tie_points,
                              const double* model_transformation, float rp[2], float mp[2], float ps[2]) {
    if (!rp || !mp || !ps) return TOPO_ERR_INVALID;
    if (model_transformation) return TOPO_ERR_UNSUPPORTED;
    if (!pixel_scale || !tie_points) return TOPO_ERR_UNSUPPORTED;
    if (n_pixel_scale != 3 || n_tie_points != 6) return TOPO_ERR_INVALID;
    rp[0] = (float)tie_points[0]; rp[1] = (float)tie_points[1];
    mp[0] = (float)tie_points[3]; mp[1] = (float)tie_points[4];
    ps[0] = (float)pixel_scale[0]; ps[1] = (float)pixel_scale[1];
    return TOPO_OK;
}

void topo_to_model(const float rp[2], const float mp[2], const float ps[2], float x, float y, float out[2]) {
    out[0] = (x - rp[0]) * ps[0] + mp[0];
    out[1] = (y - rp[1]) * -ps[1] + mp[1];
}

// ... 55 lines not shown
```

topo-renderer_amd/csrc/topo_kernels.h:

```cpp
#pragma once

#include <hip/hip_runtime.h>
#include <hip/hip_ext.h>

#include "topo_pipeline.h"

namespace topo {

constexpr uint32_t kBCX = 60, kBCY = 15;
constexpr uint32_t kVX = kBCX + 1, kVY = kBCY + 1;
#ifndef TOPO_RESOLVE_RPW
#define TOPO_RESOLVE_RPW 8
#endif
constexpr uint32_t kResolveBlockW = 64, kResolveBlockH = 4 * TOPO_RESOLVE_RPW;

struct WorkItem {
    uint32_t view_rank;
    uint32_t block;
};

struct FarItem {
    uint32_t view_rank;
    uint32_t block;
    uint16_t x0, x1, y0, y1;
    uint32_t zmin_bits;
};

struct BigItem {
    uint32_t view;
    uint32_t id;
    uint32_t region;
    int32_t X[3], Y[3];
    float z[3];
};

struct RareItem {
    uint32_t view;
    uint32_t draw;
};

struct FrameParams {
    const TileDev* tiles;
    const ViewDev* views;
    uint64_t* vis;
    uint8_t* dirty;
    WorkItem* work;
    uint32_t* counters;
    uint32_t* status_out;
    BigItem* big;
    RareItem* rare;
    FarItem* far;
    WorkItem* work2;
    uint32_t work_cap, big_cap, rare_cap;
    uint32_t far_sub_cap;
    uint32_t near_cap;
    uint32_t near_strip;
    float split_m;
    uint32_t n_views, n_tiles;
    int32_t W, H;
    uint32_t tile_w, tile_h;
    uint32_t bx_count, by_count;
    uint32_t tris_per_tile;
    FastDiv div_tris, div_hm1;
    uint32_t sky_c8;
    uint32_t linear_target;
    uint32_t bgra;
    uint32_t rblocks_x, rblocks_view;
    uint32_t post_off;
    uint32_t rblock_first, rblock_count;
    FastDiv div_rblocks_x, div_rblocks_view;
};

struct OutputParams {
    uint8_t* rgba;
    size_t rgba_view_stride, rgba_pitch;
    float* depth;
    size_t depth_view_stride, depth_pitch;
};

constexpr uint32_t kStatusBigOverflow = 1u;
constexpr uint32_t kStatusRareOverflow = 2u;
constexpr uint32_t kFarLists = 64;
constexpr uint32_t kStatusWords = 16;
constexpr uint32_t kCounterWords = kStatusWords + 16 * kFarLists;
constexpr uint32_t kStatusBounds = 4u;
constexpr uint32_t kCtrWork = 0, kCtrBig = 1;
constexpr uint32_t kCtrStatus = 2;
constexpr uint32_t kCtrRare = 3;
constexpr uint32_t kCtrFarTested = 4, kCtrFarSurvived = 5;
constexpr uint32_t kCtrBigStart = 6, kCtrRareStart = 7;
constexpr uint32_t kCtrBoundsTag = 8, kCtrBoundsLo = 9, kCtrBoundsHi = 10;
constexpr uint32_t far_list_counter(uint32_t q) { return kStatusWords + 16 * q; }

struct EdgeJob {
    uint32_t lt, rb;
    uint32_t uni;
    uint32_t top_bottom;
};
struct CornerJob {
    uint32_t lt, rt, lb, rb;
    uint32_t uni;
};

void launch_block_tables(const TileDev* tiles, uint32_t first, uint32_t count, uint32_t w, uint32_t h, hipStream_t s);
bool normals_tables_fused(uint32_t w, uint32_t h, int lds_rows);
void launch_trig_tables(const TileDev* tiles, uint32_t first, uint32_t count, uint32_t w, uint32_t h, hipStream_t s);
void launch_normals_tables(const TileDev* tiles, uint32_t first, uint32_t count, uint32_t w, uint32_t h, hipStream_t s);
void launch_block_bounds(const TileDev* tiles, uint32_t first, uint32_t count, uint32_t w, uint32_t h, hipStream_t s);
void launch_normals_interior(const TileDev* tiles, uint32_t first, uint32_t count, uint32_t w, uint32_t h, int lds_rows,
                             hipStream_t s);
void launch_normals_border(const TileDev* tiles, const EdgeJob* edges, uint32_t n_edges, const CornerJob* corners, uint32_t n_corners, uint32_t w,
                           uint32_t h, hipStream_t s);

constexpr uint32_t kPackViews = 8;
struct ViewPack { ViewDev v[kPackViews]; };
void launch_put_views(const ViewPack& pack, uint32_t n, ViewDev* dst, hipStream_t s);
void launch_clear(const FrameParams& p, uint32_t* zero, hipStream_t s, hipEvent_t start = nullptr);
void launch_clear_cull(const FrameParams& p, uint32_t* zero, hipStream_t s, hipEvent_t start = nullptr, const ViewPack* pack = nullptr, uint32_t n_pack_views = 0);
void launch_cull(const FrameParams& p, hipStream_t s);
void launch_raster(const FrameParams& p, int phase, hipStream_t s);
void launch_occlusion(const FrameParams& p, hipStream_t s);
void launch_raster_rare(const FrameParams& p, hipStream_t s);
void launch_raster_big(const FrameParams& p, hipStream_t s);
void launch_resolve(const FrameParams& p, const OutputParams& o, hipStream_t s, hipEvent_t start = nullptr, hipEvent_t stop = nullptr);

constexpr uint32_t kViewshedStatSlots = 1024;
void launch_viewshed(const FrameParams& p, uint32_t* const* masks, unsigned long long* stats, hipStream_t s);

struct HorizonPoint {
    int32_t row;
    float depth;
    int32_t lat, lon;
    uint32_t cell_x, cell_y, fan, reserved;
};
struct HorizonParams {
    const uint64_t* vis;
    const uint8_t* dirty;
    const uint32_t* counters;
    uint32_t* check;
    const int32_t* tile_ll;
    HorizonPoint* out;
    size_t view_stride;
    size_t n_keys;
    uint32_t first_view, n_views;
    uint32_t W, H;
    uint32_t n_tiles, tris_per_tile, hm1;
    FastDiv div_tris, div_hm1;
};
void launch_horizon(const HorizonParams& p, hipStream_t s);

void launch_overlay(const OverlayVertex* verts, const uint32_t* idx, uint32_t n_tris, uint32_t n_verts, float width, int32_t W, int32_t H, uint64_t* keys,
                    bool keys_fresh, uint8_t* rgba, size_t pitch, uint32_t linear_target, uint32_t bgra, hipStream_t s);

void launch_overlay_glyphs(const GlyphInstance* glyphs, uint32_t n_glyphs, float depth, const uint8_t* atlas, uint32_t aw, uint32_t ah, int32_t W, int32_t H,
                           uint64_t* keys, bool keys_fresh, uint8_t* rgba, size_t pitch, uint32_t linear_target, uint32_t bgra, hipStream_t s);
void launch_post_pixelize(uint32_t n_views, int32_t W, int32_t H, float vw, float vh, float pixelize_n, const uint8_t* pre_rgba, const OutputParams& out,
                          const float* depth, size_t depth_view_stride, size_t depth_pitch, uint32_t linear_target, uint32_t bgra, hipStream_t s);
void launch_visible_peaks(const float* proj16_dev, uint32_t w, uint32_t h, const float* depth, size_t depth_pitch, uint32_t n,
                          const float* peaks_xyz, uint8_t* visible, uint32_t* xy, hipStream_t s);

struct TiffSegDev {
    uint64_t byte_off;
    uint32_t row0;
    uint32_t x0, y0, w, h;
    uint32_t pad_;
};
void launch_tiff_rows(uint8_t* bytes, const TiffSegDev* segs, const uint32_t* row_seg, uint32_t n_rows, float* out, uint32_t W, uint32_t H,
                      uint32_t predictor, bool big_endian, hipStream_t s);
void launch_probe_sincos(const float* x, float* s, float* c, size_t n, hipStream_t st);
void launch_probe_div(int kind, const float* x, const float* y, float* out, size_t n, hipStream_t st);

}
```

topo-renderer_amd/csrc/topo_kernels.hip:

```cpp
#include <atomic>

#include "kernels_common.h"
#include "kernels_load.h"
#include "kernels_frame.h"
#include "kernels_resolve.h"
#include "kernels_query.h"
#include "kernels_overlay.h"
#include "kernels_tiff.h"

namespace topo {


template <typename K, typename... Args>
static inline void launch_timed(K kernel, dim3 grid, dim3 block, hipStream_t s, hipEvent_t start, hipEvent_t stop, const Args&... args) {
    if (start || stop) hipExtLaunchKernelGGL(kernel, grid, block, 0, s, start, stop, 0, args...);
    else hipLaunchKernelGGL(kernel, grid, block, 0, s, args...);
}

struct BlockGrid { uint32_t bxc, byc; };
static inline BlockGrid block_grid(uint32_t w, uint32_t h) { return {(w - 1 + kBCX - 1) / kBCX, (h - 1 + kBCY - 1) / kBCY}; }

template <int kSite, typename K>
static unsigned resident_grid(K kernel, unsigned fallback) {
    constexpr int kMaxDev = 64;
    static std::atomic<unsigned> cache[kMaxDev];
    int dev = 0, cus = 0, per_cu = 0;
    if (hipGetDevice(&dev) != hipSuccess || dev < 0 || dev >= kMaxDev) return fallback;
    if (unsigned g = cache[dev].load(std::memory_order_relaxed)) return g;
    if (hipDeviceGetAttribute(&cus, hipDeviceAttributeMultiprocessorCount, dev) != hipSuccess || cus <= 0) return fallback;
    if (hipOccupancyMaxActiveBlocksPerMultiprocessor(&per_cu, kernel, 256, 0) != hipSuccess || per_cu <= 0) return fallback;
    const unsigned g = (unsigned)(cus * per_cu);
    cache[dev].store(g, std::memory_order_relaxed);
    return g;
}


void launch_block_tables(const TileDev* tiles, uint32_t first, uint32_t count, uint32_t w, uint32_t h, hipStream_t s) {
    if (count == 0) return;
    const auto [bxc, byc] = block_grid(w, h);
    const uint32_t runs = (bxc + kTblBlocks - 1) / kTblBlocks * byc;
    hipLaunchKernelGGL(k_block_tables, dim3((runs + 3) / 4, count), dim3(256), 0, s, tiles, first, w, h, bxc, byc);
}

bool normals_tables_fused(uint32_t w, uint32_t h, int lds_rows) {
    static const bool off = getenv("TOPO_LOAD_FUSED") && atoi(getenv("TOPO_LOAD_FUSED")) == 0;
    return !off && lds_rows == 0 && w >= 4 * kBCX && w % (4 * kBCX) == 0 && h >= 3;
}
void launch_trig_tables(const TileDev* tiles, uint32_t first, uint32_t count, uint32_t w, uint32_t h, hipStream_t s) {
    if (count == 0) return;
    hipLaunchKernelGGL(k_trig_tables, dim3((w + h + 255) / 256, count), dim3(256), 0, s, tiles, first, w, h);
}
void launch_normals_tables(const TileDev* tiles, uint32_t first, uint32_t count, uint32_t w, uint32_t h, hipStream_t s) {
    if (count == 0) return;
    const auto [bxc, byc] = block_grid(w, h);
    const uint32_t pieces = (w / (4 * kBCX)) * ((h + kBCY - 1) / kBCY) * count;
    static const int shape = getenv("TOPO_FUSED_SHAPE") ? atoi(getenv("TOPO_FUSED_SHAPE")) : 44;
    const dim3 grid(((pieces + 7) / 8) * 8);
    switch (shape) {
        case 53: hipLaunchKernelGGL((k_normals_rolling<5, 3, true, 5>), grid, dim3(192), 0, s, tiles, first, count, (int)w, (int)h, bxc, byc); break;
        case 35: hipLaunchKernelGGL((k_normals_rolling<3, 5, true, 3>), grid, dim3(320), 0, s, tiles, first, count, (int)w, (int)h, bxc, byc); break;
        case 82: hipLaunchKernelGGL((k_normals_rolling<8, 2, true, 4>), grid, dim3(128), 0, s, tiles, first, count, (int)w, (int)h, bxc, byc); break;
        case 151: hipLaunchKernelGGL((k_normals_rolling<15, 1, true, 5>), grid, dim3(64), 0, s, tiles, first, count, (int)w, (int)h, bxc, byc); break;
        default: hipLaunchKernelGGL((k_normals_rolling<4, 4, true, 4>), grid, dim3(256), 0, s, tiles, first, count, (int)w, (int)h, bxc, byc); break;
    }
}
void launch_block_bounds(const TileDev* tiles, uint32_t first, uint32_t count, uint32_t w, uint32_t h, hipStream_t s) {
    if (count == 0) return;
    const auto [bxc, byc] = block_grid(w, h);
    if (count <= 4) hipLaunchKernelGGL(k_block_bounds<8>, dim3((bxc * byc + 31) / 32, count), dim3(256), 0, s, tiles, first, w, h, bxc, byc);
    else hipLaunchKernelGGL(k_block_bounds<1>, dim3((bxc * byc + 255) / 256, count), dim3(256), 0, s, tiles, first, w, h, bxc, byc);
}

void launch_normals_interior(const TileDev* tiles, uint32_t first, uint32_t count, uint32_t w, uint32_t h, int lds_rows,
                             hipStream_t s) {
    if (count == 0) return;
    const dim3 block(256);
    if (lds_rows == 0 && w % 4 == 0) {
        static const int shape = getenv("TOPO_ROLL_SHAPE") ? atoi(getenv("TOPO_ROLL_SHAPE")) : 41;
#define TOPO_ROLL(R, WV) hipLaunchKernelGGL((k_normals_rolling<R, WV, false>), dim3(((((w + 255) / 256) * (((h + (R)-1) / (R) + (WV)-1) / (WV)) * count + 7) / 8) * 8), dim3(64 * (WV)), 0, s, tiles, first, count, (int)w, (int)h, 0u, 0u)
        switch (shape) {
            case 44: TOPO_ROLL(4, 4); break;
            case 81: TOPO_ROLL(8, 1); break;
            case 84: TOPO_ROLL(8, 4); break;
            case 164: TOPO_ROLL(16, 4); break;
            case 484: TOPO_ROLL(48, 4); break;
            default: TOPO_ROLL(4, 1); break;
        }
#undef TOPO_ROLL
        return;
    }
#define TOPO_K1(R)                                                                                                                    \
    hipLaunchKernelGGL(k_normals_interior<R>, dim3(((((w + 127) / 128) * ((h + (R)-1) / (R)) * count + 7) / 8) * 8), block, 0, s, tiles, first, \
                       count, (int)w, (int)h)
    switch (lds_rows) {
        case 4: TOPO_K1(4); break;
        case 8: TOPO_K1(8); break;
        case 16: TOPO_K1(16); break;
        case 64: TOPO_K1(64); break;
        default: TOPO_K1(32); break;
    }
#undef TOPO_K1
}

void launch_normals_border(const TileDev* tiles, const EdgeJob* edges, uint32_t n_edges, const CornerJob* corners, uint32_t n_corners, uint32_t w,
                           uint32_t h, hipStream_t s) {
    const uint32_t chunks = (w + 63) / 64, blocks = chunks * n_edges + (n_corners + 63) / 64;
    if (blocks == 0) return;
    hipLaunchKernelGGL(k_normals_border, dim3(blocks), dim3(64), 0, s, tiles, edges, n_edges, chunks, corners, n_corners, (int)w, (int)h);
}

void launch_clear(const FrameParams& p, uint32_t* zero, hipStream_t s, hipEvent_t start) {
    const size_t n = (size_t)p.n_views * p.W * p.H;
    launch_timed(k_clear, dim3(2048), dim3(256), s, start, nullptr, p.vis, p.dirty, n, p.counters, zero);
}
void launch_put_views(const ViewPack& pack, uint32_t n, ViewDev* dst, hipStream_t s) {
    hipLaunchKernelGGL(k_put_views, dim3(1), dim3(256), 0, s, pack, n * (uint32_t)(sizeof(ViewDev) / 4), (uint32_t*)dst);
}

void launch_clear_cull(const FrameParams& p, uint32_t* zero, hipStream_t s, hipEvent_t start, const ViewPack* pack, uint32_t n_pack_views) {
    const size_t total = (size_t)p.n_views * p.n_tiles * p.bx_count * p.by_count;
    const unsigned n_cull = (unsigned)((total + 255) / 256), n_clear = 2048;
    static const ViewPack none{};
    const ViewPack& pk = pack ? *pack : none;
    const uint32_t words = pack ? n_pack_views * (uint32_t)(sizeof(ViewDev) / 4) : 0u;
    launch_timed(k_clear_cull, dim3(n_cull + n_clear), dim3(256), s, start, nullptr, p, n_cull, n_clear, zero, pk, words);
}

void launch_cull(const FrameParams& p, hipStream_t s) {
    const size_t total = (size_t)p.n_views * p.n_tiles * p.bx_count * p.by_count;
    if (total == 0) return;
    hipLaunchKernelGGL(k_cull, dim3((unsigned)((total + 255) / 256)), dim3(256), 0, s, p);
}

void launch_raster(const FrameParams& p, int phase, hipStream_t s) {
    if (p.n_tiles == 0) return;
    const unsigned grid = resident_grid<0>(k_raster, 256 * 5);
    hipLaunchKernelGGL(k_raster, dim3(grid), dim3(256), 0, s, p, phase);
}

void launch_occlusion(const FrameParams& p, hipStream_t s) {
    if (p.n_tiles == 0) return;
    const unsigned grid = resident_grid<1>(k_occlusion, 256 * 8);
    hipLaunchKernelGGL(k_occlusion, dim3(grid), dim3(256), 0, s, p);
}

void launch_raster_rare(const FrameParams& p, hipStream_t s) {
    if (p.n_tiles == 0) return;
    hipLaunchKernelGGL(k_raster_rare, dim3(256), dim3(256), 0, s, p);
}

void launch_raster_big(const FrameParams& p, hipStream_t s) {
    if (p.n_tiles == 0) return;
    const unsigned grid = resident_grid<2>(k_raster_big, 256 * 4);
    hipLaunchKernelGGL(k_raster_big, dim3(grid), dim3(256), 0, s, p);
}

void launch_resolve(const FrameParams& p, const OutputParams& o, hipStream_t s, hipEvent_t start, hipEvent_t stop) {
    const unsigned n_blocks = p.rblock_count;
    if (n_blocks == 0) return;
    unsigned resident = 4u * resident_grid<3>(k_resolve<true, false>, 256 * TOPO_RESOLVE_WGS);
    if (const char* e = getenv("TOPO_RESOLVE_GRID")) resident = (unsigned)atoi(e) ? (unsigned)atoi(e) : n_blocks;
    const dim3 grid(n_blocks < resident ? n_blocks : resident), block(256);
    const bool bgra = p.bgra && !p.post_off;
    auto launch = [&](auto kernel) { launch_timed(kernel, grid, block, s, start, stop, p, o); };
    if (!p.linear_target && !bgra) launch(k_resolve<true, false>);
    else if (!p.linear_target) launch(k_resolve<true, true>);
    else if (!bgra) launch(k_resolve<false, false>);
    else launch(k_resolve<false, true>);
}

void launch_viewshed(const FrameParams& p, uint32_t* const* masks, unsigned long long* stats, hipStream_t s) {
    if (p.n_tiles == 0) return;
    const size_t groups = (((size_t)p.n_views * p.W * p.H + 63) / 64 + 63) / 64;
    const unsigned grid = (unsigned)((groups + 3) / 4 < kViewshedStatSlots ? (groups + 3) / 4 : kViewshedStatSlots);
    hipLaunchKernelGGL(k_viewshed, dim3(grid), dim3(256), 0, s, p, masks, stats);
}

void launch_horizon(const HorizonParams& p, hipStream_t s) {
    const uint64_t waves = (uint64_t)((p.W + 63) / 64) * p.n_views;
    if (waves == 0) return;
    hipLaunchKernelGGL(k_horizon, dim3((unsigned)((waves + 3) / 4)), dim3(256), 0, s, p);
}

static void overlay_keys_init(uint64_t* keys, int32_t W, int32_t H, bool keys_fresh, hipStream_t s) {
    const size_t n = (size_t)W * H;
    if (keys_fresh) hipLaunchKernelGGL(k_overlay_init, dim3((unsigned)((n + 255) / 256)), dim3(256), 0, s, keys, n);
}

void launch_overlay(const OverlayVertex* verts, const uint32_t* idx, uint32_t n_tris, uint32_t n_verts, float width, int32_t W, int32_t H, uint64_t* keys,
                    bool keys_fresh, uint8_t* rgba, size_t pitch, uint32_t linear_target, uint32_t bgra, hipStream_t s) {
    overlay_keys_init(keys, W, H, keys_fresh, s);
    if (n_tris == 0) return;
    hipLaunchKernelGGL(k_overlay_raster, dim3((n_tris + 63) / 64), dim3(64), 0, s, verts, idx, n_tris, n_verts, width, W, H, keys);
    hipLaunchKernelGGL(k_overlay_resolve, dim3((W + 63) / 64, (H + 3) / 4), dim3(256), 0, s, verts, idx, width, W, H, keys, rgba, pitch, linear_target, bgra);
}

void launch_overlay_glyphs(const GlyphInstance* glyphs, uint32_t n_glyphs, float depth, const uint8_t* atlas, uint32_t aw, uint32_t ah, int32_t W, int32_t H,
                           uint64_t* keys, bool keys_fresh, uint8_t* rgba, size_t pitch, uint32_t linear_target, uint32_t bgra, hipStream_t s) {
    overlay_keys_init(keys, W, H, keys_fresh, s);
    if (n_glyphs == 0) return;
    hipLaunchKernelGGL(k_glyph_raster, dim3(n_glyphs), dim3(64), 0, s, glyphs, n_glyphs, depth, W, H, keys);
    hipLaunchKernelGGL(k_glyph_resolve, dim3(n_glyphs), dim3(64), 0, s, glyphs, n_glyphs, depth, atlas, aw, ah, W, H, keys, rgba, pitch, linear_target, bgra);
}

void launch_post_pixelize(uint32_t n_views, int32_t W, int32_t H, float vw, float vh, float pixelize_n, const uint8_t* pre_rgba, const OutputParams& out,
                          const float* depth, size_t depth_view_stride, size_t depth_pitch, uint32_t linear_target, uint32_t bgra, hipStream_t s) {
    hipLaunchKernelGGL(k_post_pixelize, dim3((W + 63) / 64, (H + 3) / 4, n_views), dim3(256), 0, s, W, H, vw, vh, pixelize_n, pre_rgba, out, depth, depth_view_stride,
                       depth_pitch, linear_target, bgra);
}

void launch_visible_peaks(const float* proj16_dev, uint32_t w, uint32_t h, const float* depth, size_t depth_pitch, uint32_t n,
                          const float* peaks_xyz, uint8_t* visible, uint32_t* xy, hipStream_t s) {
    if (n == 0) return;
    hipLaunchKernelGGL(k_visible_peaks, dim3((n + 255) / 256), dim3(256), 0, s, proj16_dev, w, h, depth, depth_pitch, n, peaks_xyz,
                       visible, xy);
}

void launch_tiff_rows(uint8_t* bytes, const TiffSegDev* segs, const uint32_t* row_seg, uint32_t n_rows, float* out, uint32_t W, uint32_t H,
                      uint32_t predictor, bool big_endian, hipStream_t s) {
    if (n_rows) hipLaunchKernelGGL(k_tiff_rows, dim3(n_rows), dim3(256), 0, s, bytes, segs, row_seg, out, W, H, predictor, big_endian ? 1 : 0);
}

void launch_probe_sincos(const float* x, float* s, float* c, size_t n, hipStream_t st) {
    hipLaunchKernelGGL(k_probe_sincos, dim3((unsigned)((n + 255) / 256)), dim3(256), 0, st, x, s, c, n);
}

void launch_probe_div(int kind, const float* x, const float* y, float* out, size_t n, hipStream_t st) {
    hipLaunchKernelGGL(k_probe_div, dim3((unsigned)((n + 255) / 256)), dim3(256), 0, st, kind, x, y, out, n);
}

}
```

Before: 88110 Mpix/s.

## Prefilter view-tile pairs on host and cull only surviving pairs

Adds a host-side frustum test of each tile's bounding sphere against each view's clip planes. The surviving view×tile pairs are passed as 16-bit codes in the kernel argument segment, and the cull kernel launches workgroups only for those pairs instead of every block of every tile in every view. The intent is to cut cull work and launch size when most tiles sit outside a sector's frustum. It adds host CPU work per frame and a larger kernel argument block, and if tiles do not divide evenly into 256-block workgroups it can leave some workgroups partly idle.

```diff
diff --git a/topo-renderer_amd/__init__.py b/topo-renderer_amd/__init__.py
--- a/topo-renderer_amd/__init__.py
+++ b/topo-renderer_amd/__init__.py
@@ -78,6 +78,8 @@
             "topo_set_normals_lds_rows": (C.c_int, [vp, C.c_int]),
             "topo_debug_set_queue_caps": (C.c_int, [vp, u32, u32]),
             "topo_debug_far_phase_launched": (C.c_int, [vp, vp]),
+            "topo_debug_set_tile_prefilter": (C.c_int, [vp, i32]),
+            "topo_debug_cull_pairs": (C.c_int, [vp, vp]),
             "topo_pin_host_buffer": (C.c_int, [vp, vp, sz]),
             "topo_unpin_host_buffer": (C.c_int, [vp, vp]),
             "topo_get_timings": (C.c_int, [vp, vp]),
@@ -493,6 +495,14 @@
         self._check(lib().topo_debug_far_phase_launched(self._h, _p(out)))
         return bool(out[0])
 
+    def debug_set_tile_prefilter(self, on: bool):
+        self._check(lib().topo_debug_set_tile_prefilter(self._h, 1 if on else 0))
+
+    def debug_cull_pairs(self) -> tuple:
+        out = np.zeros(2, np.uint32)
+        self._check(lib().topo_debug_cull_pairs(self._h, _p(out)))
+        return int(out[0]), int(out[1])
+
     def timings(self) -> dict:
         out = np.zeros(TIMING_SLOTS, np.float32)
         self._check(lib().topo_get_timings(self._h, _p(out)))
diff --git a/topo-renderer_amd/csrc/host_math.cpp b/topo-renderer_amd/csrc/host_math.cpp
--- a/topo-renderer_amd/csrc/host_math.cpp
+++ b/topo-renderer_amd/csrc/host_math.cpp
@@ -209,6 +209,42 @@
     }
 }
 
+uint32_t tile_prefilter(const topo_uniforms* views, uint32_t n_views, const double* spheres, uint32_t n_tiles, uint16_t* out, uint32_t cap) {
+    uint32_t kept = 0;
+    for (uint32_t v = 0; v < n_views; ++v) {
+        const float* m = views[v].camera_proj;
+        double q[6][5];
+        for (int pl = 0; pl < 6; ++pl) {
+            const int row = pl >> 1;
+            const double sgn = (pl & 1) ? -1.0 : 1.0;
+            double a, b, c, d;
+            if (pl == 4) {
+                a = m[2]; b = m[6]; c = m[10]; d = m[14];
+            } else {
+                a = (double)m[3] + sgn * (double)m[row];
+                b = (double)m[7] + sgn * (double)m[4 + row];
+                c = (double)m[11] + sgn * (double)m[8 + row];
+                d = (double)m[15] + sgn * (double)m[12 + row];
+            }
+            q[pl][0] = a; q[pl][1] = b; q[pl][2] = c; q[pl][3] = d;
+            q[pl][4] = std::sqrt(a * a + b * b + c * c);
+        }
+        for (uint32_t t = 0; t < n_tiles; ++t) {
+            const double* s = spheres + (size_t)t * kTileSphereDoubles;
+            bool outside = false;
+            if (s[3] >= 0.0 && s[4] >= 0.0) {
+                const double reach = s[3] + s[4] + 1.0;
+                for (int pl = 0; pl < 6 && !outside; ++pl)
+                    outside = q[pl][0] * s[0] + q[pl][1] * s[1] + q[pl][2] * s[2] + q[pl][3] < -reach * q[pl][4];
+            }
+            if (outside) continue;
+            if (kept < cap) out[kept] = (uint16_t)(v * n_tiles + t);
+            ++kept;
+        }
+    }
+    return kept;
+}
+
 namespace {
 inline float synth_hash(int64_t ix, int64_t iy, uint32_t seed) {
     uint32_t h = ((uint32_t)ix * 0x9E3779B1u) ^ ((uint32_t)iy * 0x85EBCA77u) ^ (seed * 0xC2B2AE3Du);
diff --git a/topo-renderer_amd/csrc/host_math.hpp b/topo-renderer_amd/csrc/host_math.hpp
--- a/topo-renderer_amd/csrc/host_math.hpp
+++ b/topo-renderer_amd/csrc/host_math.hpp
@@ -18,6 +18,8 @@
 uint32_t locations_range(float latitude, float longitude, float range_dist, int32_t* out_lat_lon, uint32_t cap);
 void change_location_plan(float latitude, float longitude, float range_dist, const int32_t* loaded, uint32_t n_loaded,
                           std::vector<std::pair<int32_t, int32_t>>& unload, std::vector<std::pair<int32_t, int32_t>>& request);
+constexpr uint32_t kTileSphereDoubles = 5;
+uint32_t tile_prefilter(const topo_uniforms* views, uint32_t n_views, const double* spheres, uint32_t n_tiles, uint16_t* out, uint32_t cap);
 void synth_tile(int32_t lat, int32_t lon, uint32_t w, uint32_t h, uint32_t seed, float* out);
 
 }
diff --git a/topo-renderer_amd/csrc/kernels_frame.h b/topo-renderer_amd/csrc/kernels_frame.h
--- a/topo-renderer_amd/csrc/kernels_frame.h
+++ b/topo-renderer_amd/csrc/kernels_frame.h
@@ -60,20 +60,47 @@
     if (slot < P.near_cap) P.work[slot] = WorkItem{(view << 16) | rank, blk};
 }
 
-__device__ __forceinline__ void cull_body(const FrameParams& P, uint32_t block) {
-    const uint32_t blocks_per_tile = P.bx_count * P.by_count;
-    const size_t total = (size_t)P.n_views * P.n_tiles * blocks_per_tile;
-    const size_t gid0 = (size_t)block * blockDim.x, gid = gid0 + threadIdx.x;
+struct CullMap {
+    uint32_t blocks_per_tile, wgs_per_pair;
+    size_t gid0;
+    uint32_t view, rank, blk0;
+    __device__ __forceinline__ CullMap(const FrameParams& P, uint32_t block, const_space_ptr<uint32_t> pairs, uint32_t wgs_per_pair_)
+        : blocks_per_tile(P.bx_count * P.by_count), wgs_per_pair(wgs_per_pair_), gid0((size_t)block * 256), view(0), rank(0), blk0(0) {
+        if (wgs_per_pair) {
+            const uint32_t pair = block / wgs_per_pair;
+            const uint32_t word = TOPO_CHK(P.counters, pair < kMaxCullPairs, 18u, pair) ? pairs[pair >> 1] : 0u;
+            uint32_t code = (word >> ((pair & 1u) * 16u)) & 0xFFFFu;
+            if (!TOPO_CHK(P.counters, code < P.n_views * P.n_tiles, 18u, code)) code = 0u;
+            view = code / P.n_tiles; rank = code % P.n_tiles;
+            blk0 = (block % wgs_per_pair) * 256u;
+        } else {
+            view = (uint32_t)(gid0 / ((size_t)blocks_per_tile * P.n_tiles));
+        }
+    }
+    __device__ __forceinline__ bool locate(const FrameParams& P, uint32_t t, uint32_t& v, uint32_t& r, uint32_t& b) const {
+        if (wgs_per_pair) {
+            v = view; r = rank; b = blk0 + t;
+            return b < blocks_per_tile;
+        }
+        const size_t g = gid0 + t;
+        b = (uint32_t)(g % blocks_per_tile);
+        r = (uint32_t)((g / blocks_per_tile) % P.n_tiles);
+        v = (uint32_t)(g / ((size_t)blocks_per_tile * P.n_tiles));
+        return g < (size_t)P.n_views * P.n_tiles * blocks_per_tile;
+    }
+};
+
+__device__ __forceinline__ void cull_body(const FrameParams& P, uint32_t block, const_space_ptr<uint32_t> pairs, uint32_t wgs_per_pair) {
+    const CullMap map(P, block, pairs, wgs_per_pair);
+    const uint32_t blocks_per_tile = map.blocks_per_tile;
     __shared__ double s_plane[2][6][5];
     __shared__ uint32_t s_far[256], s_nfar;
-    const uint32_t view0 = (uint32_t)(gid0 / ((size_t)blocks_per_tile * P.n_tiles));
+    const uint32_t view0 = map.view;
     if (threadIdx.x < 12 && view0 + threadIdx.x / 6 < P.n_views) clip_plane(P.views[view0 + threadIdx.x / 6].proj, threadIdx.x % 6, s_plane[threadIdx.x / 6][threadIdx.x % 6]);
     if (threadIdx.x == 0) s_nfar = 0;
     __syncthreads();
-    if (gid < total) {
-        const uint32_t blk = (uint32_t)(gid % blocks_per_tile);
-        const uint32_t rank = (uint32_t)((gid / blocks_per_tile) % P.n_tiles);
-        const uint32_t view = (uint32_t)(gid / ((size_t)blocks_per_tile * P.n_tiles));
+    uint32_t blk, rank, view;
+    if (map.locate(P, threadIdx.x, view, rank, blk)) {
         const TileDev& t = P.tiles[rank];
         const double hmin = (double)t.block_minmax[2 * blk], hmax = (double)t.block_minmax[2 * blk + 1];
         const double* bs = t.block_bounds + (size_t)blk * 4;
@@ -105,10 +132,7 @@
     }
     __syncthreads();
     for (uint32_t i = threadIdx.x; i < s_nfar; i += blockDim.x) {
-        const size_t g = gid0 + s_far[i];
-        const uint32_t blk = (uint32_t)(g % blocks_per_tile);
-        const uint32_t rank = (uint32_t)((g / blocks_per_tile) % P.n_tiles);
-        const uint32_t view = (uint32_t)(g / ((size_t)blocks_per_tile * P.n_tiles));
+        (void)map.locate(P, s_far[i], view, rank, blk);
         const TileDev& t = P.tiles[rank];
         const double hmin = (double)t.block_minmax[2 * blk], hmax = (double)t.block_minmax[2 * blk + 1];
         const double* bb = t.block_bounds + (size_t)blocks_per_tile * 4 + (size_t)blk * 12;
@@ -150,16 +174,29 @@
     }
 }
 
-__global__ __launch_bounds__(256) void k_cull(FrameParams P) { cull_body(P, blockIdx.x); }
+struct CullPairs { uint16_t code[kMaxCullPairs]; };
+struct CullArgs {
+    FrameParams P;
+    uint32_t wgs_per_pair;
+    CullPairs pairs;
+};
+__global__ __launch_bounds__(256) void k_cull(FrameParams P, uint32_t wgs_per_pair, CullPairs pairs) {
+    cull_body(P, blockIdx.x, kernarg<uint32_t>(offsetof(CullArgs, pairs)), wgs_per_pair);
+}
 struct ClearCullArgs {
     FrameParams P;
     uint32_t n_cull_blocks, n_clear_blocks;
     uint32_t* zero;
     ViewPack pack;
     uint32_t pack_words;
+    uint32_t wgs_per_pair;
+    CullPairs pairs;
 };
+static_assert(sizeof(ClearCullArgs) <= 3584 && sizeof(CullArgs) <= 3584, "a launch's argument segment holds 4 KB, the hidden arguments included");
+static_assert(offsetof(ClearCullArgs, pairs) % 4 == 0 && offsetof(CullArgs, pairs) % 4 == 0, "the pair list is read in words");
+static_assert(offsetof(ClearCullArgs, pack) == 232 && offsetof(ClearCullArgs, pairs) == 944 && offsetof(CullArgs, pairs) == 220, "the argument segment's layout");
 __global__ __launch_bounds__(256) void k_clear_cull(FrameParams P, uint32_t n_cull_blocks, uint32_t n_clear_blocks, uint32_t* __restrict__ zero, ViewPack pack,
-                                                    uint32_t pack_words) {
+                                                    uint32_t pack_words, uint32_t wgs_per_pair, CullPairs pairs) {
     if (pack_words) {
         const auto src = kernarg<uint32_t>(offsetof(ClearCullArgs, pack));
         if (blockIdx.x == 0 && threadIdx.x < pack_words) const_cast<uint32_t*>(reinterpret_cast<const uint32_t*>(P.views))[threadIdx.x] = src[threadIdx.x];
@@ -168,7 +205,7 @@
     const uint32_t total = n_cull_blocks + n_clear_blocks;
     const uint32_t before = (uint32_t)((uint64_t)blockIdx.x * n_clear_blocks / total), upto = (uint32_t)((uint64_t)(blockIdx.x + 1u) * n_clear_blocks / total);
     if (upto > before) clear_body(P.vis, P.dirty, (size_t)P.n_views * P.W * P.H, P.counters, zero, before, n_clear_blocks);
-    else cull_body(P, blockIdx.x - before);
+    else cull_body(P, blockIdx.x - before, kernarg<uint32_t>(offsetof(ClearCullArgs, pairs)), wgs_per_pair);
 }
 
 #ifndef TOPO_OCC_ROWS
diff --git a/topo-renderer_amd/csrc/terrain_renderer.cpp b/topo-renderer_amd/csrc/terrain_renderer.cpp
--- a/topo-renderer_amd/csrc/terrain_renderer.cpp
+++ b/topo-renderer_amd/csrc/terrain_renderer.cpp
@@ -21,6 +21,7 @@
     const bool far_skip = env("TOPO_FAR_SKIP", 1) != 0;
     const bool events_by_marker = env("TOPO_EVENTS_BY_MARKER", 0) != 0;
     const bool fuse_clear_cull = env("TOPO_FUSE_CLEAR_CULL", 1) != 0;
+    const bool tile_prefilter = env("TOPO_TILE_PREFILTER", 1) != 0;
     const int near_strip = env("TOPO_NEAR_STRIP", 0);
 };
 const Switches& switches() { static const Switches s; return s; }
@@ -84,6 +85,7 @@
     TOPO_HIP_TRY(hipSetDevice(device_));
     TOPO_HIP_TRY(hipStreamCreate(&own_stream_.h));
     stream_ = own_stream_;
+    tile_prefilter_ = switches().tile_prefilter;
     for (auto& e : load_ev_) TOPO_HIP_TRY(hipEventCreate(&e.h));
     return init_ctx(ctx_[0], false);
 }
@@ -240,11 +242,12 @@
     {
         std::vector<double> sph((size_t)bxc * byc * 4);
         TOPO_HIP_TRY(hipMemcpy(sph.data(), nt.dev.block_bounds, sph.size() * sizeof(double), hipMemcpyDeviceToHost));
-        double c[3] = {0.0, 0.0, 0.0}, r2 = 0.0;
+        double c[3] = {0.0, 0.0, 0.0}, r2 = 0.0, rmax = 0.0;
         bool finite = true;
         for (size_t i = 0; i < sph.size(); i += 4) {
             finite = finite && std::isfinite(sph[i]) && std::isfinite(sph[i + 1]) && std::isfinite(sph[i + 2]) && std::isfinite(sph[i + 3]);
             for (int k = 0; k < 3; ++k) c[k] += sph[i + k];
+            rmax = std::max(rmax, sph[i + 3]);
         }
         for (int k = 0; k < 3; ++k) c[k] /= (double)(sph.size() / 4);
         for (size_t i = 0; i < sph.size() && finite; i += 4) {
@@ -253,6 +256,7 @@
         }
         nt.centres[0] = c[0]; nt.centres[1] = c[1]; nt.centres[2] = c[2];
         nt.centres[3] = finite ? std::sqrt(r2) : -1.0;
+        nt.block_radius = finite ? rmax : -1.0;
     }
     TOPO_HIP_TRY(hipGetLastError());
     return TOPO_OK;
@@ -459,10 +463,32 @@
     fill_params(c, p);
     last_blocks_tested_ = p.work_cap;
     last_far_phase_ = p.split_m > 0.0f && !(switches().far_skip && far_phase_empty(views, n, tiles_, &p.split_m));
-    if (int rc = queue_frame(c, stream, p, pack_in_cull ? &pack : nullptr, last_far_phase_, out, slots, n_slots, after_slot)) return rc;
+    const CullList cull = cull_pairs(views, p);
+    if (int rc = queue_frame(c, stream, p, pack_in_cull ? &pack : nullptr, cull, last_far_phase_, out, slots, n_slots, after_slot)) return rc;
     record_submission(c, p);
     TOPO_HIP_TRY(hipGetLastError());
     return TOPO_OK;
+}
+
+TerrainRenderer::CullList TerrainRenderer::cull_pairs(const topo_uniforms* views, const FrameParams& p) {
+    const size_t all = (size_t)p.n_views * p.n_tiles;
+    last_cull_pairs_[0] = last_cull_pairs_[1] = (uint32_t)all;
+    CullList list{nullptr, 0};
+    if (!tile_prefilter_ || all == 0 || all > 65536) return list;
+    if (tile_spheres_gen_ != tile_gen_) {
+        tile_spheres_.clear();
+        for (const auto& kv : tiles_) {
+            tile_spheres_.insert(tile_spheres_.end(), kv.second.centres, kv.second.centres + 4);
+            tile_spheres_.push_back(kv.second.block_radius);
+        }
+        tile_spheres_gen_ = tile_gen_;
+    }
+    const uint32_t kept = tile_prefilter(views, p.n_views, tile_spheres_.data(), p.n_tiles, cull_codes_, kMaxCullPairs);
+    if (kept > kMaxCullPairs) return list;
+    last_cull_pairs_[0] = kept;
+    list.codes = cull_codes_;
+    list.n = kept;
+    return list;
 }
 
 int TerrainRenderer::grow_frame_buffers(FrameCtx& c, hipStream_t stream, uint32_t n, uint32_t w, uint32_t h, FrameParams& p) {
@@ -490,7 +516,7 @@
     const size_t near_cap = (size_t)((kBCY + p.near_strip - 1) / p.near_strip) * work_cap;
     if (int rc = ensure(stream, c.d_work, (near_cap ? near_cap : 1) * sizeof(WorkItem))) return rc;
     if (int rc = ensure(stream, c.d_work2, (near_cap ? near_cap : 1) * sizeof(WorkItem))) return rc;
-    const size_t far_sub_cap = ((work_cap + 255) / 256 + kFarLists - 1) / kFarLists * 256;
+    const size_t far_sub_cap = (cull_workgroups_max(n, p.n_tiles, p.bx_count * p.by_count) + kFarLists - 1) / kFarLists * 256;
     if (int rc = ensure(stream, c.d_far, (far_sub_cap ? far_sub_cap * kFarLists : 1) * sizeof(FarItem))) return rc;
     if (int rc = ensure(stream, c.d_big, p.big_cap * sizeof(BigItem))) return rc;
     if (int rc = ensure(stream, c.d_rare, p.rare_cap * sizeof(RareItem))) return rc;
@@ -582,7 +608,7 @@
                (to_unorm8(1.0f) << 24);
 }
 
-int TerrainRenderer::queue_frame(FrameCtx& c, hipStream_t stream, FrameParams& p, const ViewPack* pack_in_cull, bool far_phase, const OutputParams& out,
+int TerrainRenderer::queue_frame(FrameCtx& c, hipStream_t stream, FrameParams& p, const ViewPack* pack_in_cull, const CullList& cull, bool far_phase, const OutputParams& out,
                                  const ResolveSlot* slots, uint32_t n_slots, const std::function<int(uint32_t, hipStream_t)>* after_slot) {
     const uint32_t n = p.n_views, w = (uint32_t)p.W, h = (uint32_t)p.H;
     uint32_t* const counters_next = c.d_counters.as<uint32_t>() + ((c.frames & 1u) ^ 1u) * kCounterWords;
@@ -601,10 +627,10 @@
     TOPO_HIP_TRY(mark(kStClear, true));
     const hipEvent_t ev_first = own(kStClear);
     const bool fuse = fused_clear_cull(p);
-    if (fuse) launch_clear_cull(p, counters_next, stream, ev_first, pack_in_cull, n);
+    if (fuse) launch_clear_cull(p, counters_next, stream, ev_first, pack_in_cull, n, cull.codes, cull.n);
     else launch_clear(p, counters_next, stream, ev_first);
     TOPO_HIP_TRY(mark(kStCull));
-    if (!fuse) launch_cull(p, stream);
+    if (!fuse) launch_cull(p, stream, cull.codes, cull.n);
     TOPO_HIP_TRY(mark(kStRasterNear));
     launch_raster(p, 0, stream);
     TOPO_HIP_TRY(mark(kStRareBigNear));
diff --git a/topo-renderer_amd/csrc/terrain_renderer.hpp b/topo-renderer_amd/csrc/terrain_renderer.hpp
--- a/topo-renderer_amd/csrc/terrain_renderer.hpp
+++ b/topo-renderer_amd/csrc/terrain_renderer.hpp
@@ -70,6 +70,7 @@
     uint32_t* d_normals = nullptr;
     float* d_minmax = nullptr;
     double centres[4] = {0.0, 0.0, 0.0, -1.0};
+    double block_radius = -1.0;
     TileDev dev{};
     DeviceBuffer mask;
 };
@@ -85,6 +86,8 @@
                     const float rp[2], const float mp[2], const float ps[2]);
     int unload_terrain(int32_t lat, int32_t lon);
     bool last_far_phase() const { return last_far_phase_; }
+    void set_tile_prefilter(bool on) { tile_prefilter_ = on; }
+    void last_cull_pairs(uint32_t out[2]) const { out[0] = last_cull_pairs_[0]; out[1] = last_cull_pairs_[1]; }
     int update(uint32_t w, uint32_t h, const topo_uniforms* u, const topo_post_uniforms* pu);
     int render(uint8_t* rgba, size_t rgba_pitch, float* depth, size_t depth_pitch);
     int render_views_device(uint32_t n, const topo_uniforms* views, uint32_t w, uint32_t h, const OutputParams& out);
@@ -230,8 +233,10 @@
     int grow_frame_buffers(FrameCtx& c, hipStream_t s, uint32_t n, uint32_t w, uint32_t h, FrameParams& p);
     int stage_views(FrameCtx& c, hipStream_t s, const topo_uniforms* views, FrameParams& p, ViewPack& pack, bool* pack_in_cull);
     void fill_params(FrameCtx& c, FrameParams& p);
-    int queue_frame(FrameCtx& c, hipStream_t s, FrameParams& p, const ViewPack* pack_in_cull, bool far_phase, const OutputParams& out, const ResolveSlot* slots,
-                    uint32_t n_slots, const std::function<int(uint32_t, hipStream_t)>* after_slot);
+    struct CullList { const uint16_t* codes; uint32_t n; };
+    CullList cull_pairs(const topo_uniforms* views, const FrameParams& p);
+    int queue_frame(FrameCtx& c, hipStream_t s, FrameParams& p, const ViewPack* pack_in_cull, const CullList& cull, bool far_phase, const OutputParams& out,
+                    const ResolveSlot* slots, uint32_t n_slots, const std::function<int(uint32_t, hipStream_t)>* after_slot);
     void record_submission(FrameCtx& c, const FrameParams& p);
     int frame_durations(const FrameCtx::TimedFrame& f, float out[7]);
 
@@ -254,6 +259,11 @@
     uint32_t depth_w_ = 0, depth_h_ = 0;
     uint32_t last_blocks_tested_ = 0;
     bool last_far_phase_ = true;
+    bool tile_prefilter_ = true;
+    std::vector<double> tile_spheres_;
+    uint64_t tile_spheres_gen_ = ~0ull;
+    uint16_t cull_codes_[kMaxCullPairs] = {};
+    uint32_t last_cull_pairs_[2] = {0, 0};
     bool vs_on_ = false, vs_ever_ = false;
     DeviceBuffer d_vs_table_;
     DeviceBuffer d_vs_stats_;
diff --git a/topo-renderer_amd/csrc/topo_capi.cpp b/topo-renderer_amd/csrc/topo_capi.cpp
--- a/topo-renderer_amd/csrc/topo_capi.cpp
+++ b/topo-renderer_amd/csrc/topo_capi.cpp
@@ -133,6 +133,19 @@
     return TOPO_OK;
 }
 
+int topo_debug_set_tile_prefilter(topo_ctx* ctx, int32_t on) {
+    TOPO_GUARD(ctx);
+    ctx->r->set_tile_prefilter(on != 0);
+    return TOPO_OK;
+}
+
+int topo_debug_cull_pairs(topo_ctx* ctx, uint32_t out[2]) {
+    TOPO_GUARD(ctx);
+    if (!out) return TOPO_ERR_INVALID;
+    ctx->r->last_cull_pairs(out);
+    return TOPO_OK;
+}
+
 int topo_get_timings(topo_ctx* ctx, float out_ms[TOPO_TIMING_SLOTS]) {
     TOPO_GUARD(ctx);
     TOPO_CALL(ctx->r->get_timings(out_ms));
diff --git a/topo-renderer_amd/csrc/topo_kernels.h b/topo-renderer_amd/csrc/topo_kernels.h
--- a/topo-renderer_amd/csrc/topo_kernels.h
+++ b/topo-renderer_amd/csrc/topo_kernels.h
@@ -115,9 +115,12 @@
 constexpr uint32_t kPackViews = 8;
 struct ViewPack { ViewDev v[kPackViews]; };
 void launch_put_views(const ViewPack& pack, uint32_t n, ViewDev* dst, hipStream_t s);
+constexpr uint32_t kMaxCullPairs = 1024;
 void launch_clear(const FrameParams& p, uint32_t* zero, hipStream_t s, hipEvent_t start = nullptr);
-void launch_clear_cull(const FrameParams& p, uint32_t* zero, hipStream_t s, hipEvent_t start = nullptr, const ViewPack* pack = nullptr, uint32_t n_pack_views = 0);
-void launch_cull(const FrameParams& p, hipStream_t s);
+void launch_clear_cull(const FrameParams& p, uint32_t* zero, hipStream_t s, hipEvent_t start = nullptr, const ViewPack* pack = nullptr, uint32_t n_pack_views = 0,
+                       const uint16_t* pairs = nullptr, uint32_t n_pairs = 0);
+void launch_cull(const FrameParams& p, hipStream_t s, const uint16_t* pairs = nullptr, uint32_t n_pairs = 0);
+size_t cull_workgroups_max(uint32_t n_views, uint32_t n_tiles, uint32_t blocks_per_tile);
 void launch_raster(const FrameParams& p, int phase, hipStream_t s);
 void launch_occlusion(const FrameParams& p, hipStream_t s);
 void launch_raster_rare(const FrameParams& p, hipStream_t s);
diff --git a/topo-renderer_amd/csrc/topo_kernels.hip b/topo-renderer_amd/csrc/topo_kernels.hip
--- a/topo-renderer_amd/csrc/topo_kernels.hip
+++ b/topo-renderer_amd/csrc/topo_kernels.hip
@@ -1,4 +1,6 @@
+#include <algorithm>
 #include <atomic>
+#include <cstring>
 
 #include "kernels_common.h"
 #include "kernels_load.h"
@@ -117,19 +119,43 @@
     hipLaunchKernelGGL(k_put_views, dim3(1), dim3(256), 0, s, pack, n * (uint32_t)(sizeof(ViewDev) / 4), (uint32_t*)dst);
 }
 
-void launch_clear_cull(const FrameParams& p, uint32_t* zero, hipStream_t s, hipEvent_t start, const ViewPack* pack, uint32_t n_pack_views) {
-    const size_t total = (size_t)p.n_views * p.n_tiles * p.bx_count * p.by_count;
-    const unsigned n_cull = (unsigned)((total + 255) / 256), n_clear = 2048;
+namespace {
+struct CullGrid {
+    unsigned n_blocks;
+    uint32_t wgs_per_pair;
+    CullPairs list{};
+    CullGrid(const FrameParams& p, const uint16_t* pairs, uint32_t n_pairs) {
+        const uint32_t blocks_per_tile = p.bx_count * p.by_count;
+        if (pairs && n_pairs <= kMaxCullPairs && blocks_per_tile) {
+            wgs_per_pair = (blocks_per_tile + 255) / 256;
+            n_blocks = n_pairs * wgs_per_pair;
+            memcpy(list.code, pairs, n_pairs * sizeof(uint16_t));
+        } else {
+            wgs_per_pair = 0;
+            n_blocks = (unsigned)(((size_t)p.n_views * p.n_tiles * blocks_per_tile + 255) / 256);
+        }
+    }
+};
+}
+size_t cull_workgroups_max(uint32_t n_views, uint32_t n_tiles, uint32_t blocks_per_tile) {
+    const size_t pairs = (size_t)n_views * n_tiles;
+    return std::max((pairs * blocks_per_tile + 255) / 256, pairs * ((blocks_per_tile + 255) / 256));
+}
+
+void launch_clear_cull(const FrameParams& p, uint32_t* zero, hipStream_t s, hipEvent_t start, const ViewPack* pack, uint32_t n_pack_views, const uint16_t* pairs,
+                       uint32_t n_pairs) {
+    const CullGrid g(p, pairs, n_pairs);
+    const unsigned n_clear = 2048;
     static const ViewPack none{};
     const ViewPack& pk = pack ? *pack : none;
     const uint32_t words = pack ? n_pack_views * (uint32_t)(sizeof(ViewDev) / 4) : 0u;
-    launch_timed(k_clear_cull, dim3(n_cull + n_clear), dim3(256), s, start, nullptr, p, n_cull, n_clear, zero, pk, words);
-}
-
-void launch_cull(const FrameParams& p, hipStream_t s) {
-    const size_t total = (size_t)p.n_views * p.n_tiles * p.bx_count * p.by_count;
-    if (total == 0) return;
-    hipLaunchKernelGGL(k_cull, dim3((unsigned)((total + 255) / 256)), dim3(256), 0, s, p);
+    launch_timed(k_clear_cull, dim3(g.n_blocks + n_clear), dim3(256), s, start, nullptr, p, g.n_blocks, n_clear, zero, pk, words, g.wgs_per_pair, g.list);
+}
+
+void launch_cull(const FrameParams& p, hipStream_t s, const uint16_t* pairs, uint32_t n_pairs) {
+    const CullGrid g(p, pairs, n_pairs);
+    if (g.n_blocks == 0) return;
+    hipLaunchKernelGGL(k_cull, dim3(g.n_blocks), dim3(256), 0, s, p, g.wgs_per_pair, g.list);
 }
 
 void launch_raster(const FrameParams& p, int phase, hipStream_t s) {
```

Result: faster. 89450 Mpix/s (median of 6 runs) (+1.5%).
